# GameTechDev/Intel-Texture-Works-Plugin

Measured on AMD Instinct MI355X. Metric: Mpixels/s encode (BC1/BC3/BC7/BC6H) at 4k x 4k; bit-exact vs the oracle under the pinned ISPC sse/avx-target arithmetic model (no ispc binary exists here; sensitivity of that model: profiles/arith_sensitivity.txt), higher is better.
Workload: dtype f32; 1 GPU; bc7_slow: BC7 GetProfile_slow on ONE synthetic 4096x4096 RGBA8 surface, weak-sharded over 1 GPU(s) by block-row bands (4096 texel rows per rank), texels resident in HBM, device-pointer C ABI call; blocks_per_gpu=1048576, ranks_seen_by_rccl=1, device=gfx950:sramecc+:xnack- / AMD Radeon Graphics / 256 CUs / 2400 MHz, lib=itw-amd 0.1 gfx950 arith=x86-lut-nr contract=off

## Files before the change

include/itw_test_hooks.h:

```cpp
#ifndef ITW_TEST_HOOKS_H
#define ITW_TEST_HOOKS_H

#include "ispc_texcomp.h"

#ifdef __cplusplus
extern "C" {
#endif
#pragma GCC visibility push(default)

void itwTestRcp  (const float* d_in, float* d_out, int64_t n);
void itwTestRsqrt(const float* d_in, float* d_out, int64_t n);
void itwTestF2I  (const float* d_in, int32_t* d_out, int64_t n);

void itwTestBc7TwoSubsetBounds(const rgba_surface* d_src, float* d_out);

int itwTestBc45IndexTable(uint32_t* host_out);

int itwTestBc45ClosestS(uint8_t* host_out);

void itwMultiGpuTestInjectFailure(int rank, int stage, int stall_ms);

void itwTestCombinerHold(int requests, int timeout_ms);
void itwTestCombinerCounters(int64_t out[5]);

#pragma GCC visibility pop
#ifdef __cplusplus
}
#endif
#endif
```

intel-texture-works-plugin_amd/csrc/abi.hip:

```cpp
#include <hip/hip_runtime.h>
#include <cstdio>
#include <cstdlib>
#include <cstring>
#include "../../include/itw_amd.h"
#include "../../include/itw_bc45.h"
#include "../../include/itw_dispatch.h"
#ifdef ITW_TEST_HOOKS
#include "../../include/itw_test_hooks.h"
#endif
#include <algorithm>
#include <atomic>
#include <chrono>
#include <condition_variable>
#include <mutex>
#include <thread>
#include <vector>
#include "bcn_format.hpp"
#include "host_rt.hpp"
#include "kernels.hpp"
#include "x86_math.hpp"

namespace itw {

namespace {
// ... 1194 lines not shown
void CompressBlocksBC4(const rgba_surface* src, uint8_t* dst)
{
    itw::guarded([&] { Job j; j.kind = itw::BCN_BC4; compress(j, src, dst); });
}
void CompressBlocksBC5(const rgba_surface* src, uint8_t* dst)
{
    itw::guarded([&] { Job j; j.kind = itw::BCN_BC5; compress(j, src, dst); });
}
void CompressBlocksBC4S(const rgba_surface* src, uint8_t* dst)
{
    itw::guarded([&] { Job j; j.kind = itw::BCN_BC4S; compress(j, src, dst); });
}
void CompressBlocksBC5S(const rgba_surface* src, uint8_t* dst)
{
    itw::guarded([&] { Job j; j.kind = itw::BCN_BC5S; compress(j, src, dst); });
}

bool itwCompressImageSlicedEx(const rgba_surface* source, uint8_t* target, int64_t block_row_pitch, int dxgi_format, const void* settings,
                              int64_t slice_pixels, ItwProgressFunc* progress, void* user)
{
    bool done = false;
    itw::clear_failure();
    const bool ok = itw::guarded([&] {
        if (!source) itw::fail_msg("null surface");
        const Job j = job_of(dxgi_format, settings);
        const itw::SurfaceGeometry geo = itw::surface_geometry(j.kind, source->width, source->height);
        const int64_t tight = (int64_t)geo.bx * geo.bpb;
        if (block_row_pitch != tight) itw::fail_msg("itwCompressImageSlicedEx: block_row_pitch %lld != %lld (tight)", (long long)block_row_pitch, (long long)tight);
        done = compress_sliced(j, source, target, slices_of(source, slice_pixels), progress, user);
    });
    return ok && done;
}

bool itwCompressImageChainEx(const rgba_surface* images, int count, uint8_t* target, int dxgi_format, const void* settings,
                             ItwProgressFunc* progress, void* user)
{
    bool done = false;
    itw::clear_failure();
    const bool ok = itw::guarded([&] {
        const Job j = chain_job(images, count, target, dxgi_format, settings);
        done = compress_chain(j, images, count, target, progress, user);
    });
    return ok && done;
}

void itwSetSliceWindow(int slices) { g_slice_window.store(slices < 0 ? -1 : slices, std::memory_order_relaxed); }

int itwSliceWindow(int dxgi_format, int width, int height, int64_t slice_pixels) { return itwSliceWindowFor(dxgi_format, nullptr, width, height, slice_pixels); }

int itwSliceWindowFor(int dxgi_format, const void* settings, int width, int height, int64_t slice_pixels)
{
    if (slice_window_setting() < 0) return 0;
    const int kind = itw::format_kind(dxgi_format);
    const int64_t slices = std::min(itw::slice_count(width, height, slice_pixels), itw::kMaxSlices);
    const bool heavy = kind == itw::BCN_BC7 && settings && itw::bc7_scans_every_shape(*static_cast<const bc7_enc_settings*>(settings));
    return slice_window(kind, itw::surface_geometry(kind, width, height).blocks() / slices, (int)slices, heavy);
}

void  itwSetStream(void* s) { tls.user_stream = (hipStream_t)s; }
void* itwGetStream(void)    { return (void*)tls.user_stream; }

int itwAvailable(void)
{
    int n = 0;
    if (hipGetDeviceCount(&n) != hipSuccess || n < 1) { (void)hipGetLastError(); return 0; }
    int dev = 0;
    hipDeviceProp_t p;
    if (hipGetDevice(&dev) != hipSuccess || hipGetDeviceProperties(&p, dev) != hipSuccess) { (void)hipGetLastError(); return 0; }
    return std::strncmp(p.gcnArchName, "gfx950", 6) == 0 ? 1 : 0;
}

void itwSetErrorMode(int mode) { itw::g_error_mode.store(mode == ITW_ON_ERROR_RETURN ? 1 : 0); }
const char* itwLastError(void) { return itw::t_has_error ? itw::t_last_error : nullptr; }
void itwClearError(void) { itw::clear_failure(); }

const char* itwDeviceInfo(void)
{
    tls.info[0] = 0;
    itw::guarded([&] {
        int dev = 0;
        ITW_CHECK(hipGetDevice(&dev));
        hipDeviceProp_t p;
        ITW_CHECK(hipGetDeviceProperties(&p, dev));
        std::snprintf(tls.info, sizeof(tls.info), "%s / %s / %d CUs / %.0f MHz", p.gcnArchName, p.name,
                      p.multiProcessorCount, p.clockRate / 1000.0);
    });
    return tls.info;
}

void itwSetBc7Path(int path) { itw::set_bc7_path(path); itw::set_bc6h_path(path); }
void itwSetBc7Pilot(int percent) { itw::set_bc7_pilot(percent); }

const char* itwVersion(void) { return "itw-amd 0.1 gfx950 arith=x86-lut-nr contract=off"; }

int64_t itwBandForPart(int32_t width, int32_t height, int32_t bytes_per_block,
                       int32_t part, int32_t parts, int32_t* first_row, int32_t* row_count)
{
    const int64_t R = height / 4, bx = width / 4;
    if (parts <= 0 || part < 0 || part >= parts) { if (first_row) *first_row = 0; if (row_count) *row_count = 0; return -1; }
    const int64_t r0 = R * part / parts, r1 = R * (part + 1) / parts;
    if (first_row) *first_row = (int32_t)(r0 * 4);
    if (row_count) *row_count = (int32_t)((r1 - r0) * 4);
    return r0 * bx * bytes_per_block;
}

int64_t itwBandForPartEx(int32_t width, int32_t height, int32_t bytes_per_block, int32_t part, int32_t parts, int32_t keep_partial_blocks,
                         int32_t* first_row, int32_t* row_count)
{
    if (!keep_partial_blocks) return itwBandForPart(width, height, bytes_per_block, part, parts, first_row, row_count);
    const int64_t R = ((int64_t)height + 3) / 4, bx = ((int64_t)width + 3) / 4;
    if (parts <= 0 || part < 0 || part >= parts || height < 1 || width < 1) { if (first_row) *first_row = 0; if (row_count) *row_count = 0; return -1; }
    const int64_t r0 = R * part / parts, r1 = R * (part + 1) / parts;
    const int64_t y0 = r0 * 4, y1 = (r1 * 4 < height) ? r1 * 4 : height;
    if (first_row) *first_row = (int32_t)y0;
    if (row_count) *row_count = (int32_t)(y1 > y0 ? y1 - y0 : 0);
    return r0 * bx * bytes_per_block;
}

void itwWarmupBC45(void)
{
    itwClearError();
    itw::guarded([&] { bind_thread_to_current_device(); itw::warmup_bc45(); });
}

void itwWarmupBC45S(void)
{
    itwClearError();
    itw::guarded([&] { bind_thread_to_current_device(); itw::warmup_bc45s(); });
}

#ifdef ITW_TEST_HOOKS
int itwTestBc45IndexTable(uint32_t* host_out)
{
    itwClearError();
    return itw::guarded([&] { if (!host_out) itw::fail_msg("null pointer"); itw::copy_bc45_index_table(host_out, tls.user_stream); }) ? 0 : -1;
}

int itwTestBc45ClosestS(uint8_t* host_out)
{
    itwClearError();
    return itw::guarded([&] { if (!host_out) itw::fail_msg("null pointer"); itw::copy_bc45_closest_snorm(host_out, tls.user_stream); }) ? 0 : -1;
}

void itwTestBc7TwoSubsetBounds(const rgba_surface* d_src, float* d_out)
{
    itwClearError();
    itw::guarded([&] {
        if (!d_src || !d_src->ptr || !d_out) itw::fail_msg("null pointer");
        itw::launch_bc7_test_bounds(d_src->ptr, d_src->stride, d_src->width, d_src->height, d_out, tls.user_stream);
        ITW_CHECK(hipGetLastError());
    });
}

void itwTestRcp(const float* in, float* out, int64_t n)
{
    if (n <= 0) return;
    hipLaunchKernelGGL(k_test_rcp, dim3((unsigned)((n + 255) / 256)), dim3(256), 0, tls.user_stream, in, out, n);
    itw::guarded([&] { ITW_CHECK(hipGetLastError()); });
}
void itwTestRsqrt(const float* in, float* out, int64_t n)
{
    if (n <= 0) return;
    hipLaunchKernelGGL(k_test_rsqrt, dim3((unsigned)((n + 255) / 256)), dim3(256), 0, tls.user_stream, in, out, n);
    itw::guarded([&] { ITW_CHECK(hipGetLastError()); });
}
void itwTestF2I(const float* in, int32_t* out, int64_t n)
{
    if (n <= 0) return;
    hipLaunchKernelGGL(k_test_f2i, dim3((unsigned)((n + 255) / 256)), dim3(256), 0, tls.user_stream, in, out, n);
    itw::guarded([&] { ITW_CHECK(hipGetLastError()); });
}

void itwTestCombinerHold(int requests, int timeout_ms)
{
    int dev = 0;
    if (hipGetDevice(&dev) != hipSuccess) { (void)hipGetLastError(); return; }
    if (dev < 0 || dev >= kMaxDevices) return;
    Combiner& c = g_combiner[dev];
    std::lock_guard<std::mutex> lk(c.m);
    c.hold_requests = requests > 0 ? requests : 0;
    c.hold_timeout_ms = timeout_ms > 0 ? timeout_ms : 0;
}

void itwTestCombinerCounters(int64_t out[5])
{
    if (!out) return;
    out[0] = g_cstats.bursts.load(); out[1] = g_cstats.batches.load(); out[2] = g_cstats.requests.load(); out[3] = g_cstats.calls.load();
    out[4] = g_hold_timeouts.load();
}
#endif

}
```

intel-texture-works-plugin_amd/csrc/bc7.hip:

```cpp
#include <atomic>
#include <cstdlib>
#include <cstring>
#include <type_traits>
#include "bc7_exact.hpp"
#include "kernels.hpp"
#include "host_rt.hpp"

namespace itw {

#define BCN_TABLE_QUAL __device__ const
#include "bc7_f02_schedule.h"
#undef BCN_TABLE_QUAL

#ifndef ITW_BC7_LANE_PAL
#define ITW_BC7_LANE_PAL 1
#endif
constexpr int LANE_PAL_LEVELS = 24;
constexpr int TPB = 256;
constexpr float INV255 = 1.0f / 255.0f;
constexpr int32_t ERR_MAX = 0x7fffffff;
enum Family { F_MODES02 = 0, F_MODES13 = 1, F_MODE7 = 2, F_MODES456 = 3 };

struct ModeTraits { int pairs, bits, ch; };
__device__ __forceinline__ constexpr ModeTraits traits(int mode)
// ... 1007 lines not shown

template <int FAMILY, int RANKED, bool VEC16>
__global__ void __launch_bounds__(TPB) __attribute__((amdgpu_waves_per_eu(search_waves(FAMILY, RANKED), search_waves(FAMILY, RANKED))))
bc7_search_kernel(const uint8_t* __restrict__ src, int64_t stride, int32_t blocks_x, int32_t nblocks,
                  uint4* __restrict__ wins, const bc7_enc_settings S)
{
    __shared__ unsigned short s_seed16[2048];
    __shared__ uint32_t s_seed32[2048];
    extern __shared__ int32_t s_keys[];
    __shared__ uint2 s_pal[RANKED == 0 ? 12 * TPB : (RANKED == 2 && ITW_BC7_LANE_PAL) ? 16 * TPB : 1];
    Lane ln;
    ln.T = stage_seed_tables_fast(s_seed16, s_seed32, threadIdx.x, TPB);
    __syncthreads();
    const int32_t gid = blockIdx.x * TPB + threadIdx.x;
    const bool live = gid < nblocks;
    const int32_t b = live ? gid : nblocks - 1;
    ln.keys = s_keys + threadIdx.x;
    ln.pal = s_pal + ((RANKED == 0 || (RANKED == 2 && ITW_BC7_LANE_PAL)) ? threadIdx.x : 0);
    load_block<VEC16>(ln.tx, src, stride, blocks_x, b);

    Win wa, wb;
    if (FAMILY == F_MODES02) search_02(ln, S, wa, wb);
    if (FAMILY == F_MODES13) search_two_subset<false, 3, RANKED>(ln, S, wa, wb);
    if (FAMILY == F_MODE7) {
        if (S.channels == 4) search_two_subset<true, 4, RANKED>(ln, S, wa, wb); else search_two_subset<true, 3, RANKED>(ln, S, wa, wb);
    }
    if (live) {
        store_win(wins, nblocks, 0, b, wa);
        if (FAMILY != F_MODE7) store_win(wins, nblocks, 1, b, wb);
    }
}

template <int FAMILY, bool VEC16>
__global__ void __launch_bounds__(TPB) __attribute__((amdgpu_waves_per_eu(finish_waves(FAMILY), finish_waves(FAMILY))))
bc7_finish_kernel(const uint8_t* __restrict__ src, int64_t stride, int32_t blocks_x, int32_t nblocks,
                  uint8_t* __restrict__ dst, int32_t* __restrict__ err_ws, const uint4* __restrict__ wins,
                  const bc7_enc_settings S, const int first)
{
    __shared__ unsigned short s_seed16[2048];
    __shared__ uint32_t s_seed32[2048];
    __shared__ uint2 s_pal[FAMILY == F_MODES456 ? (ITW_BC7_LANE_PAL ? 16 : 8) * TPB : (ITW_BC7_LANE_PAL ? (FAMILY == F_MODES02 ? 24 : 16) * TPB : 1)];
    Lane ln;
    ln.T = stage_seed_tables_fast(s_seed16, s_seed32, threadIdx.x, TPB);
    __syncthreads();
    const int32_t gid = blockIdx.x * TPB + threadIdx.x;
    const bool live = gid < nblocks;
    const int32_t b = live ? gid : nblocks - 1;
    ln.keys = nullptr;
    ln.pal = s_pal + ((FAMILY == F_MODES456 || ITW_BC7_LANE_PAL) ? threadIdx.x : 0);
    load_block<VEC16>(ln.tx, src, stride, blocks_x, b);

    ln.best_err = first ? ERR_MAX : err_ws[b];
    ln.best[0] = ln.best[1] = ln.best[2] = ln.best[3] = 0u;
    ln.improved = (first != 0);
    ln.opaque_err = 0;
    if (S.channels == 4) {
        uint32_t e = 0;
#pragma unroll
        for (int d = 0; d < 4; d++) { const uint32_t x = ~ln.tx.pl[3][d]; e = udot4(x, x, e); }
        ln.opaque_err = (int32_t)e;
    }

    if (FAMILY == F_MODES02) {
        Win w;
        load_win(w, wins, nblocks, 0, b);
        refine_and_commit<0>(ln, w, S.refineIterations[0], S.channels);
        if (!S.skip_mode2) { load_win(w, wins, nblocks, 1, b); refine_and_commit<2>(ln, w, S.refineIterations[2], S.channels); }
    }
    if (FAMILY == F_MODES13) {
        Win w;
        if (S.fastSkipTreshold_mode1 > 0) { load_win(w, wins, nblocks, 0, b); refine_and_commit<1>(ln, w, S.refineIterations[1], S.channels); }
        if (S.fastSkipTreshold_mode3 > 0) { load_win(w, wins, nblocks, 1, b); refine_and_commit<3>(ln, w, S.refineIterations[3], S.channels); }
    }
    if (FAMILY == F_MODE7) {
        Win w;
        load_win(w, wins, nblocks, 0, b);
        refine_and_commit<7>(ln, w, S.refineIterations[7], S.channels);
    }
    if (FAMILY == F_MODES456) {
        if (S.mode_selection[2]) modes_45(ln, S);
        if (S.mode_selection[3]) { if (S.channels == 4) mode_6<4>(ln, S); else mode_6<3>(ln, S); }
    }

    if (live && ln.improved) {
        uint32_t* d = reinterpret_cast<uint32_t*>(dst + (int64_t)b * 16);
        if (VEC16) *reinterpret_cast<uint4*>(d) = make_uint4(ln.best[0], ln.best[1], ln.best[2], ln.best[3]);
        else { d[0] = ln.best[0]; d[1] = ln.best[1]; d[2] = ln.best[2]; d[3] = ln.best[3]; }
        err_ws[b] = ln.best_err;
    }
}

enum WideKind { WK_SCAN02 = 0, WK_SCAN13 = 1, WK_SCAN7 = 2 };
__host__ __device__ constexpr int wide_win_slot(int mode) { return mode == 0 ? 0 : mode == 2 ? 1 : mode == 1 ? 2 : mode == 3 ? 3 : 4; }

template <int FIT_CH, int RANK_CH>
__device__ __forceinline__ void whole_block_rank_stats(Stats<RANK_CH>& rfull, const Tex& tx)
{
    IStats<FIT_CH> full;
    stats_int<FIT_CH>(full, tx.pl, whole_block());
    IStats<RANK_CH> t;
    #pragma unroll
    for (int i = 0; i < 10; i++) t.m[i] = full.m[i];
    #pragma unroll
    for (int i = 0; i < 4; i++) t.s[i] = full.s[i];
    t.n = 16;
    stats_float<RANK_CH>(rfull, t);
}

template <int FIT_CH, int RANK_CH>
__device__ __forceinline__ int32_t merge_key(const Win& w, const Tex& tx, const SeedTables& T)
{
    if (w.key >= 0) return w.key;
    Stats<RANK_CH> rfull;
    whole_block_rank_stats<FIT_CH, RANK_CH>(rfull, tx);
    return rank_key<RANK_CH>(w.shape, tx, rfull, T);
}

__device__ __forceinline__ uint32_t pack_win(const Win& w) { return w.err == ERR_MAX ? 0xffffffffu : (((uint32_t)w.err << 7) | ((uint32_t)w.shape & 127u)); }
__device__ __forceinline__ void unpack_win(Win& w, uint32_t v)
{
    if (v == 0xffffffffu) { w.err = ERR_MAX; w.shape = 0; } else { w.err = (int32_t)(v >> 7); w.shape = (int32_t)(v & 127u); }
    w.key = -1;
}

#ifndef LIST_SCAN_MAX_PARTS
#define LIST_SCAN_MAX_PARTS 8
#endif
__device__ __forceinline__ int32_t list_scan_parts(int32_t count, int32_t nblocks)
{
    const int32_t chunks = ((count + TPB - 1) / TPB + 7) & ~7;
    if (chunks <= 0) return 1;
    const int32_t p = nblocks / (chunks * TPB);
    return p < 1 ? 1 : (p > LIST_SCAN_MAX_PARTS ? LIST_SCAN_MAX_PARTS : p);
}
template <int FIT_CH, int RANK_CH>
__device__ __forceinline__ void merge_packed_parts(Win& w, Lane& ln, const uint32_t* __restrict__ row, int32_t count, int parts, int32_t slot)
{
    unpack_win(w, row[slot]);
    for (int p = 1; p < parts; p++) {
        Win x;
        unpack_win(x, row[(int64_t)p * count + slot]);
        if (x.err < w.err) { w = x; continue; }
        if (x.err != w.err || x.err == ERR_MAX) continue;
        w.key = merge_key<FIT_CH, RANK_CH>(w, ln.tx, ln.T); x.key = merge_key<FIT_CH, RANK_CH>(x, ln.tx, ln.T);
        if (x.key < w.key) w = x;
    }
}

struct PairRegion { uint64_t* words; int32_t* buckets; int32_t* ctr; int32_t cap; };
constexpr int PAIR_CTR_OVERFLOW = 64, PAIR_CTR_REDO = 65, PAIR_CTR_LIST = 66, PAIR_CTR_TARGET = 68, PAIR_CTR_WORDS = 80;
struct PairTarget { PairRegion P; int32_t* redo; };
static_assert(sizeof(PairTarget) <= (PAIR_CTR_WORDS - PAIR_CTR_TARGET) * sizeof(int32_t) && PAIR_CTR_TARGET % 2 == 0 && PAIR_CTR_WORDS % 4 == 0, "PairTarget behind the counters");
constexpr int PAIR_MAX_PER_BLOCK = 32;
constexpr unsigned long long PAIR_WORD_HEAVY = ~0ull - 1ull;

struct ScanTasks { int n; int kind[3]; };

struct ChunkSel { int32_t kind, stripe, band; const int32_t* gate; int32_t want; };
__device__ __forceinline__ int32_t sel_chunk(const ChunkSel& s, int32_t i)
{
    if (s.kind == 0) return i;
    if (s.kind == 2) return i * 8 + 3;
    const int32_t q = i / s.stripe;
    return (2 * q + s.band) * s.stripe + (i - q * s.stripe);
}

__host__ __device__ constexpr int scan_all_waves(bool ranked, bool fam7) { return fam7 ? (ranked ? SWR27 : SW7) : (ranked ? SWR2 : SWALL); }
template <bool VEC16, bool RANKED_LISTS, bool FAM7>
__global__ void __launch_bounds__(TPB) __attribute__((amdgpu_waves_per_eu(scan_all_waves(RANKED_LISTS, FAM7), scan_all_waves(RANKED_LISTS, FAM7))))
bc7_scan_all(const uint8_t* __restrict__ src, int64_t stride, int32_t blocks_x, int32_t nblocks, uint32_t* __restrict__ wins4,
             const bc7_enc_settings S, const ScanTasks tasks, const int ranked13, const int ranked7, const int32_t nchunks, const int32_t grain,
             const int32_t* __restrict__ rgb_list, const int32_t* __restrict__ rgb_count, const int32_t split, const ChunkSel sel,
             const uint4* __restrict__ compact)
{
    __shared__ unsigned short s_seed16[2048];
    __shared__ uint32_t s_seed32[2048];
    __shared__ uint2 s_pal[((RANKED_LISTS && ITW_BC7_LANE_PAL) ? 16 : 12) * TPB];
    if (sel.gate && *sel.gate != sel.want) return;
    if (!RANKED_LISTS && split) {
        const int32_t count = *rgb_count;
        const int32_t parts = list_scan_parts(count, nblocks);
        const uint32_t wg = blockIdx.x;
        const int32_t chunk = (int32_t)((wg / (8u * (uint32_t)parts)) * 8u + (wg & 7u)), part = (int32_t)((wg >> 3) % (uint32_t)parts);
        if (chunk * TPB >= count) return;
        Lane ln;
        ln.T = stage_seed_tables_fast(s_seed16, s_seed32, threadIdx.x, TPB);
        __syncthreads();
        const int32_t gid = chunk * TPB + threadIdx.x;
        const bool live = gid < count;
        const int32_t slot = live ? gid : count - 1;
        ln.keys = nullptr;
        ln.pal = s_pal + threadIdx.x;
        if (compact) load_block_compact(ln.tx, compact, slot); else load_block<VEC16>(ln.tx, src, stride, blocks_x, rgb_list[slot]);
        Win wa, wb;
        if (FAM7) {
            search_two_subset<true, 4, 0>(ln, S, wa, wb, part, parts);
            if (live) wins4[(int64_t)wide_win_slot(7) * nblocks + (int64_t)part * count + slot] = pack_win(wa);
        } else {
            search_two_subset<false, 3, 0>(ln, S, wa, wb, part, parts);
            if (live) {
                wins4[(int64_t)wide_win_slot(1) * nblocks + (int64_t)part * count + slot] = pack_win(wa);
                wins4[(int64_t)wide_win_slot(3) * nblocks + (int64_t)part * count + slot] = pack_win(wb);
            }
        }
        return;
    }
    const uint32_t w = blockIdx.x, per = (uint32_t)grain * (uint32_t)tasks.n, group = w / per, r = w % per;
    const int t = (int)(r / (uint32_t)grain);
    const int32_t chunk_i = (int32_t)(group * (uint32_t)grain + r % (uint32_t)grain);
    if (chunk_i >= nchunks) return;
    const int32_t chunk = sel_chunk(sel, chunk_i);
    const int32_t nact = (!FAM7 && rgb_list) ? *rgb_count : nblocks;
    if (chunk * TPB >= nact) return;
    Lane ln;
    ln.T = stage_seed_tables_fast(s_seed16, s_seed32, threadIdx.x, TPB);
    __syncthreads();
    const int32_t gid = chunk * TPB + threadIdx.x;
    const bool live = gid < nact;
    const int32_t slot = live ? gid : nact - 1;
    const int32_t b = (!FAM7 && rgb_list) ? rgb_list[slot] : slot;
    ln.keys = nullptr;
    ln.pal = s_pal + threadIdx.x;
    load_block<VEC16>(ln.tx, src, stride, blocks_x, b);
    const int kind = tasks.kind[t];
    Win wa, wb;
    if (!FAM7 && kind == WK_SCAN02) {
        search_02(ln, S, wa, wb);
        if (live) { wins4[(int64_t)wide_win_slot(0) * nblocks + b] = pack_win(wa); if (!S.skip_mode2) wins4[(int64_t)wide_win_slot(2) * nblocks + b] = pack_win(wb); }
    } else if (!FAM7) {
        if (RANKED_LISTS && ranked13) search_two_subset<false, 3, 2>(ln, S, wa, wb); else search_two_subset<false, 3, 0>(ln, S, wa, wb);
        if (live) { wins4[(int64_t)wide_win_slot(1) * nblocks + b] = pack_win(wa); wins4[(int64_t)wide_win_slot(3) * nblocks + b] = pack_win(wb); }
    } else {
        if (S.channels == 4) { if (RANKED_LISTS && ranked7) search_two_subset<true, 4, 2>(ln, S, wa, wb); else search_two_subset<true, 4, 0>(ln, S, wa, wb); }
        else                 { if (RANKED_LISTS && ranked7) search_two_subset<true, 3, 2>(ln, S, wa, wb); else search_two_subset<true, 3, 0>(ln, S, wa, wb); }
        if (live) wins4[(int64_t)wide_win_slot(7) * nblocks + b] = pack_win(wa);
    }
}

__device__ __forceinline__ int32_t append_to_list(int32_t* __restrict__ list, int32_t* __restrict__ count, bool need, int32_t b)
{
    const unsigned long long m = __ballot(need);
    int32_t pos = -1;
    if (m) {
        const int lane = (int)(threadIdx.x & 63u);
        int32_t base = 0;
        if (lane == 0) base = atomicAdd(count, (int32_t)__popcll(m));
        base = __shfl(base, 0);
        if (need) { pos = base + (int32_t)__popcll(m & ((1ull << lane) - 1ull)); list[pos] = b; }
    }
    return pos;
}

__device__ __forceinline__ bool mode6_cannot_win(Lane& ln)
{
    if (__all(ln.best_err == 0)) return true;
    IStats<3> full;
    stats_int<3>(full, ln.tx.pl, whole_block());
    const float d = __builtin_amdgcn_sqrtf(subset_residual_bound(full) * rcp_of_count(16)) * 0.999999f - BOUND_SLACK3[16];
    const float e = fmaxf(d, 0.0f);
    const float lb = e * e * 0.999999f;
    return __all(lb >= (float)ln.best_err);
}

#ifndef FINISH_ALL_WAVES
#define FINISH_ALL_WAVES 2
#endif
#ifndef BOUND_BAIL_AFTER
#define BOUND_BAIL_AFTER 4
#endif
#ifndef BOUND_BAIL_LANES
#define BOUND_BAIL_LANES 40
#endif
template <bool VEC16, int PHASE>
__global__ void __launch_bounds__(TPB) __attribute__((amdgpu_waves_per_eu(FINISH_ALL_WAVES, FINISH_ALL_WAVES)))
bc7_finish_all(const uint8_t* __restrict__ src, int64_t stride, int32_t blocks_x, int32_t nblocks, uint8_t* __restrict__ dst,
               const uint32_t* __restrict__ wins4, const bc7_enc_settings S, int32_t* __restrict__ inc_err,
               const int32_t* __restrict__ in_list, const int32_t* __restrict__ in_count, int32_t* __restrict__ out_list, int32_t* __restrict__ out_count,
               int32_t* __restrict__ out_list7, int32_t* __restrict__ out_count7, const ChunkSel sel,
               const uint4* __restrict__ in_compact, uint4* __restrict__ out_compact)
{
    constexpr bool LISTED = PHASE == 2 || PHASE == 4 || PHASE == 5 || PHASE == 7 || PHASE == 8;
    constexpr bool DO02 = PHASE == 0 || PHASE == 2 || PHASE == 3 || PHASE == 5;
    constexpr bool DO13 = PHASE == 0 || PHASE == 2 || PHASE == 4;
    constexpr bool DO7 = PHASE == 0 || PHASE == 1;
    constexpr bool DO456 = PHASE == 0 || PHASE == 1 || PHASE == 3 || PHASE == 6;
    __shared__ unsigned short s_seed16[2048];
    __shared__ uint32_t s_seed32[2048];
    __shared__ uint2 s_pal[(ITW_BC7_LANE_PAL ? LANE_PAL_LEVELS : 8) * TPB];
    __shared__ int32_t s_at[PHASE == 3 ? TPB / 64 : 1][64];
    if (sel.gate && *sel.gate != sel.want) return;
    const int32_t nact = LISTED ? *in_count : nblocks;
    const int32_t chunk = LISTED ? (int32_t)blockIdx.x : sel_chunk(sel, (int32_t)blockIdx.x);
    if (chunk * TPB >= nact) return;
    Lane ln;
    ln.T = stage_seed_tables_fast(s_seed16, s_seed32, threadIdx.x, TPB);
    __syncthreads();
    const int32_t gid = chunk * TPB + threadIdx.x;
    const bool live = gid < nact;
    const int32_t slot = live ? gid : nact - 1;
    const int32_t b = LISTED ? in_list[slot] : slot;
    ln.keys = nullptr;
    ln.pal = s_pal + threadIdx.x;
    if (LISTED && in_compact) load_block_compact(ln.tx, in_compact, slot); else load_block<VEC16>(ln.tx, src, stride, blocks_x, b);
    ln.best_err = ERR_MAX;
    ln.best[0] = ln.best[1] = ln.best[2] = ln.best[3] = 0u;
    ln.improved = false;
    ln.opaque_err = 0;
    if (S.channels == 4) {
        uint32_t e = 0;
#pragma unroll
        for (int d = 0; d < 4; d++) { const uint32_t x = ~ln.tx.pl[3][d]; e = udot4(x, x, e); }
        ln.opaque_err = (int32_t)e;
    }
    const bool on13 = S.mode_selection[1];
    int32_t e_alpha = ERR_MAX;
    if (PHASE == 2 || PHASE == 5) e_alpha = inc_err[b];
    if (PHASE == 4 || PHASE == 7 || PHASE == 8) ln.best_err = inc_err[b];
    Win w;
    if (DO02 && S.mode_selection[0]) {
        unpack_win(w, wins4[(int64_t)wide_win_slot(0) * nblocks + b]);
        refine_and_commit<0>(ln, w, S.refineIterations[0], S.channels);
        if (!S.skip_mode2) { ln.tx.fence(); unpack_win(w, wins4[(int64_t)wide_win_slot(2) * nblocks + b]); refine_and_commit<2>(ln, w, S.refineIterations[2], S.channels); }
    }
    const int32_t e02 = ln.best_err;
    if (DO13 && PHASE != 4) {
        if (on13 && S.fastSkipTreshold_mode1 > 0) { ln.tx.fence(); unpack_win(w, wins4[(int64_t)wide_win_slot(1) * nblocks + b]); refine_and_commit<1>(ln, w, S.refineIterations[1], S.channels); }
        if (on13 && S.fastSkipTreshold_mode3 > 0) { ln.tx.fence(); unpack_win(w, wins4[(int64_t)wide_win_slot(3) * nblocks + b]); refine_and_commit<3>(ln, w, S.refineIterations[3], S.channels); }
    }
    if (PHASE == 4) {
        const int parts = list_scan_parts(nact, nblocks);
        if (S.fastSkipTreshold_mode1 > 0) { ln.tx.fence(); merge_packed_parts<3, 3>(w, ln, wins4 + (int64_t)wide_win_slot(1) * nblocks, nact, parts, slot); refine_and_commit<1>(ln, w, S.refineIterations[1], S.channels); }
        if (S.fastSkipTreshold_mode3 > 0) { ln.tx.fence(); merge_packed_parts<3, 3>(w, ln, wins4 + (int64_t)wide_win_slot(3) * nblocks, nact, parts, slot); refine_and_commit<3>(ln, w, S.refineIterations[3], S.channels); }
    }
    bool redo = false;
    if (PHASE == 8) {
        const unsigned long long* pw = reinterpret_cast<const unsigned long long*>(wins4) + 2 * (int64_t)slot;
        const int32_t inc = ln.best_err;
        const bool heavy = pw[0] == PAIR_WORD_HEAVY;
        redo = !heavy && *out_count7 != 0;
        const bool use = !heavy && !redo;
        const unsigned long long v1 = (use && S.fastSkipTreshold_mode1 > 0) ? pw[0] : ~0ull, v3 = (use && S.fastSkipTreshold_mode3 > 0) ? pw[1] : ~0ull;
        if (v1 != ~0ull) {
            ln.tx.fence();
            w.err = (int32_t)(v1 >> 32); w.key = (int32_t)(uint32_t)v1; w.shape = w.key & 63;
            const bool open = w.err + ln.opaque_err >= inc;
            const int32_t before = ln.best_err;
            refine_and_commit<1>(ln, w, S.refineIterations[1], S.channels);
            redo = redo || (open && ln.best_err < before);
        }
        if (v3 != ~0ull) {
            ln.tx.fence();
            w.err = (int32_t)(v3 >> 32); w.key = (int32_t)(uint32_t)v3; w.shape = w.key & 63;
            const bool open = w.err + ln.opaque_err >= inc;
            const int32_t before = ln.best_err;
            refine_and_commit<3>(ln, w, S.refineIterations[3], S.channels);
            redo = redo || (open && ln.best_err < before);
        }
        append_to_list(out_list, out_count, live && redo, b);
    }
    if (PHASE == 7) {
        const int parts = list_scan_parts(nact, nblocks);
        ln.tx.fence();
        merge_packed_parts<4, 4>(w, ln, wins4 + (int64_t)wide_win_slot(7) * nblocks, nact, parts, slot);
        refine_and_commit<7>(ln, w, S.refineIterations[7], S.channels);
    }
    if (DO7 && on13 && S.fastSkipTreshold_mode7 > 0) { ln.tx.fence(); unpack_win(w, wins4[(int64_t)wide_win_slot(7) * nblocks + b]); refine_and_commit<7>(ln, w, S.refineIterations[7], S.channels); }
    if (DO456) {
        ln.tx.fence();
        if (S.mode_selection[2]) modes_45(ln, S);
        if (S.mode_selection[3]) {
            if (S.channels == 4) mode_6<4>(ln, S);
            else if (!mode6_cannot_win(ln)) mode_6<3>(ln, S);
        }
    }
    if (PHASE == 1) {
        if (live) inc_err[b] = ln.best_err;
        append_to_list(out_list, out_count, live && ln.opaque_err <= ln.best_err, b);
    }
    if (PHASE == 6) {
        const bool rgb = ln.opaque_err <= ln.best_err;
        if (live) inc_err[b] = rgb ? ln.best_err : ln.best_err + 1;
        append_to_list(out_list, out_count, live && rgb, b);
        append_to_list(out_list7, out_count7, live && !rgb, b);
    }
    if (PHASE == 3 || PHASE == 5) {
        int32_t inc;
        if (PHASE == 3) inc = ln.best_err + (ln.best_err < e02 ? 1 : 0);
        else            inc = (e02 <= e_alpha) ? e02 : e_alpha + 1;
        if (live) inc_err[b] = inc;
        ln.tx.fence();
        IStats<3> full;
        stats_int<3>(full, ln.tx.pl, whole_block());
        const float lim = (float)(inc - ln.opaque_err) - 0.5f;
        const float lim7 = (float)inc - 0.5f;
        const bool with7 = PHASE == 5 && out_list7 != nullptr;
        const PairTarget* target = nullptr;
        if (PHASE == 3) target = reinterpret_cast<const PairTarget*>(out_count + (PAIR_CTR_TARGET - PAIR_CTR_LIST));
        const bool pairs = PHASE == 3 && target->P.words != nullptr;
        bool need = !live, need7 = !live || !with7;
        unsigned long long mine = 0, any = 0;
#pragma unroll 1
        for (int shape = 0; shape < 64; shape++) {
            if (!pairs) {
                if (__all(need && need7)) break;
                if (shape == BOUND_BAIL_AFTER && __popcll(__ballot(need && need7)) >= BOUND_BAIL_LANES) { need = true; need7 = true; break; }
            }
            const float lb = two_subset_bound(shape, ln.tx.pl, full);
            const bool in = !(lb >= lim);
            need = need || in;
            need7 = need7 || !(lb >= lim7);
            if (pairs) {
                mine |= (live && in) ? (1ull << shape) : 0ull;
                any |= __ballot(live && in) ? (1ull << shape) : 0ull;
            }
        }
        const int32_t pos = append_to_list(out_list, out_count, live && need, b);
        if (out_compact && pos >= 0) {
            uint4* c = out_compact + (int64_t)pos * 4;
#pragma unroll
            for (int y = 0; y < 4; y++) c[y] = make_uint4(ln.tx.w[y * 4 + 0], ln.tx.w[y * 4 + 1], ln.tx.w[y * 4 + 2], ln.tx.w[y * 4 + 3]);
        }
        if (pairs) {
            const int lane = (int)__builtin_amdgcn_mbcnt_hi(~0u, __builtin_amdgcn_mbcnt_lo(~0u, 0u));
            const int wave = __builtin_amdgcn_readfirstlane((int)(threadIdx.x >> 6));
            const PairRegion P = target->P;
            int32_t* pair_redo = target->redo;
            const bool heavy = __popcll(mine) > PAIR_MAX_PER_BLOCK;
            if (pos >= 0) { P.words[2 * (int64_t)pos] = heavy ? PAIR_WORD_HEAVY : ~0ull; P.words[2 * (int64_t)pos + 1] = ~0ull; }
            if (heavy) mine = 0;
            append_to_list(pair_redo, P.ctr + PAIR_CTR_REDO, heavy, b);
            int32_t k = 0;
            for (unsigned long long rest = any; rest; rest &= rest - 1ull) {
                const int shape = __builtin_amdgcn_readfirstlane((int)__builtin_ctzll(rest));
                const int32_t c = (int32_t)__popcll(__ballot((mine >> shape) & 1ull));
                k = (lane == shape) ? c : k;
            }
            s_at[wave][lane] = k;
            __syncthreads();
            if (threadIdx.x < 64u) {
                int32_t t = 0;
#pragma unroll
                for (int w = 0; w < TPB / 64; w++) t += s_at[w][lane];
                int32_t base = t ? atomicAdd(P.ctr + lane, t) : 0;
                if (base + t > P.cap) { P.ctr[PAIR_CTR_OVERFLOW] = 1; base = -1; }
#pragma unroll
                for (int w = 0; w < TPB / 64; w++) { const int32_t c = s_at[w][lane]; s_at[w][lane] = base; base = base < 0 ? -1 : base + c; }
            }
            __syncthreads();
            const int32_t at = s_at[wave][lane];
            for (unsigned long long rest = any; rest; rest &= rest - 1ull) {
                const int shape = __builtin_amdgcn_readfirstlane((int)__builtin_ctzll(rest));
                const bool in = (mine >> shape) & 1ull;
                const unsigned long long m = __ballot(in);
                const int32_t base = __builtin_amdgcn_readlane(at, shape);
                if (in && base >= 0) P.buckets[(int64_t)shape * P.cap + base + (int32_t)__popcll(m & ((1ull << lane) - 1ull))] = pos;
            }
        }
        if (with7) append_to_list(out_list7, out_count7, live && need7, b);
    }
    bool store = live;
    if (PHASE == 2 || PHASE == 5) store = store && ln.best_err <= e_alpha;
    if (PHASE == 4 || PHASE == 7) store = store && ln.improved;
    if (PHASE == 8) store = store && ln.improved && !redo;
    if ((PHASE == 4 || PHASE == 8) && store) inc_err[b] = ln.best_err;
    if (store) {
        uint32_t* d = reinterpret_cast<uint32_t*>(dst + (int64_t)b * 16);
        if (VEC16) *reinterpret_cast<uint4*>(d) = make_uint4(ln.best[0], ln.best[1], ln.best[2], ln.best[3]);
        else { d[0] = ln.best[0]; d[1] = ln.best[1]; d[2] = ln.best[2]; d[3] = ln.best[3]; }
    }
}

template <bool VEC16>
__global__ void __launch_bounds__(TPB)
bc7_pilot_estimate(const uint8_t* __restrict__ src, int64_t stride, int32_t blocks_x, int32_t nblocks, const uint32_t* __restrict__ wins4,
                   const int skip_mode2, const ChunkSel sel, int32_t* __restrict__ counters , const int32_t thr256,
                   int32_t* __restrict__ flag, int32_t* __restrict__ host_counts )
{
    const int32_t chunk = sel_chunk(sel, (int32_t)blockIdx.x * 8 + 3);
    if (chunk * TPB < nblocks) {
        const int32_t gid = chunk * TPB + threadIdx.x;
        const bool live = gid < nblocks;
        const int32_t b = live ? gid : nblocks - 1;
        Tex tx;
        load_block<VEC16>(tx, src, stride, blocks_x, b);
        Win w0, w2;
        unpack_win(w0, wins4[(int64_t)wide_win_slot(0) * nblocks + b]);
        unpack_win(w2, skip_mode2 ? 0xffffffffu : wins4[(int64_t)wide_win_slot(2) * nblocks + b]);
        const int32_t e = min(w0.err, w2.err);
        IStats<3> full;
        stats_int<3>(full, tx.pl, whole_block());
        const float lim = (float)e - 0.5f;
        bool need = !live;
#pragma unroll 1
        for (int shape = 0; shape < 64; shape++) {
            if (__all(need)) break;
            if (shape == BOUND_BAIL_AFTER && __popcll(__ballot(need)) >= BOUND_BAIL_LANES) { need = true; break; }
            need = need || !(two_subset_bound(shape, tx.pl, full) >= lim);
        }
        const unsigned long long ml = __ballot(live && need), mt = __ballot(live);
        if ((threadIdx.x & 63u) == 0u) { atomicAdd(counters + 0, (int32_t)__popcll(ml)); atomicAdd(counters + 1, (int32_t)__popcll(mt)); }
    }
    __syncthreads();
    if (threadIdx.x == 0) {
        __threadfence();
        if (atomicAdd(counters + 2, 1) == (int32_t)gridDim.x - 1) {
            __threadfence();
            const int64_t listed = atomicAdd(counters + 0, 0), sampled = atomicAdd(counters + 1, 0);
            *flag = (listed * 256 <= (int64_t)thr256 * sampled) ? 1 : 0;
            if (host_counts) { host_counts[0] = (int32_t)listed; host_counts[1] = (int32_t)sampled; __threadfence_system(); }
        }
    }
}

__global__ void __launch_bounds__(TPB) bc7_bounded_setup(int32_t* __restrict__ counters, const PairTarget t0, const PairTarget t1)
{
    for (int i = (int)threadIdx.x; i < 16 + 2 * PAIR_CTR_WORDS; i += TPB) {
        const int j = i < 16 ? 0 : (i - 16) % PAIR_CTR_WORDS;
        if (i < 16 || j < PAIR_CTR_TARGET) counters[i] = 0;
    }
    if (threadIdx.x == 0) {
        *reinterpret_cast<PairTarget*>(counters + 16 + PAIR_CTR_TARGET) = t0;
        *reinterpret_cast<PairTarget*>(counters + 16 + PAIR_CTR_WORDS + PAIR_CTR_TARGET) = t1;
    }
}


__global__ void __launch_bounds__(TPB) __attribute__((amdgpu_waves_per_eu(4, 4)))
bc7_pair_scan(const uint8_t* __restrict__ src, int64_t stride, int32_t blocks_x, const int32_t* __restrict__ list, const uint4* __restrict__ compact,
              const bc7_enc_settings S, const PairRegion P)
{
    __shared__ unsigned short s_seed16[2048];
    __shared__ uint32_t s_seed32[2048];
    __shared__ uint2 s_pal[12 * TPB];
    __shared__ int32_t s_first[65];
    if (P.ctr[PAIR_CTR_OVERFLOW]) return;
    if (threadIdx.x == 0) {
        int32_t t = 0;
        for (int s = 0; s < 64; s++) { s_first[s] = t; t += (P.ctr[s] + 63) >> 6; }
        s_first[64] = t;
    }
    __syncthreads();
    const int32_t total = s_first[64];
    const int32_t wpb = TPB / 64;
    if ((int32_t)blockIdx.x * wpb >= total) return;
    Lane ln;
    ln.T = stage_seed_tables_fast(s_seed16, s_seed32, threadIdx.x, TPB);
    __syncthreads();
    ln.keys = nullptr;
    ln.pal = s_pal + threadIdx.x;
    const int lane = (int)(threadIdx.x & 63u);
    const bool on_a = S.fastSkipTreshold_mode1 > 0, on_b = S.fastSkipTreshold_mode3 > 0;
    int shape = 0;
#pragma unroll 1
    for (int32_t tile = (int32_t)blockIdx.x * wpb + (int32_t)(threadIdx.x >> 6); tile < total; tile += (int32_t)gridDim.x * wpb) {
        while (s_first[shape + 1] <= tile) shape++;
        shape = __builtin_amdgcn_readfirstlane(shape);
        const int32_t len = P.ctr[shape];
        const int32_t at = (tile - s_first[shape]) * 64 + lane;
        const bool live = at < len;
        const int32_t slot = P.buckets[(int64_t)shape * P.cap + (live ? at : len - 1)];
        if (compact) load_block_compact(ln.tx, compact, slot); else load_block<false>(ln.tx, src, stride, blocks_x, list[slot]);
        Win wa, wb;
        search_two_subset<false, 3, 0>(ln, S, wa, wb, shape, 64);
        const int32_t ea = wa.err, ec = wb.err;
        ln.tx.fence();
        Stats<3> rfull;
        whole_block_rank_stats<3, 3>(rfull, ln.tx);
        const uint32_t key = (uint32_t)rank_key<3>(shape, ln.tx, rfull, ln.T);
        if (live && on_a) atomicMin(reinterpret_cast<unsigned long long*>(P.words + 2 * (int64_t)slot),     ((unsigned long long)(uint32_t)ea << 32) | key);
        if (live && on_b) atomicMin(reinterpret_cast<unsigned long long*>(P.words + 2 * (int64_t)slot + 1), ((unsigned long long)(uint32_t)ec << 32) | key);
    }
}

constexpr int WIDE_SLOTS = 18;
constexpr int WIDE_SLOT_M4 = 5, WIDE_SLOT_M5 = 13, WIDE_SLOT_M6 = 17;
constexpr int WIDE_MAX_TASKS = 56;
constexpr int WIDE_MAX_PARTS = 16;
struct WideTasks { int n; uint8_t kind[WIDE_MAX_TASKS]; uint8_t part[WIDE_MAX_TASKS]; uint8_t parts[WIDE_MAX_TASKS]; };
struct WideModes { int n; uint8_t mode[20]; uint8_t parts[20]; };


struct WideDims { int32_t nblocks; int32_t pstride; };
__device__ __forceinline__ void store_win_wide(uint4* __restrict__ wins, WideDims d, int slot, int part, int32_t b, const Win& w)
{
    wins[((int64_t)slot * d.pstride + part) * d.nblocks + b] = make_uint4((uint32_t)w.err, (uint32_t)w.shape, (uint32_t)w.key, 0u);
}
__device__ __forceinline__ void load_win_wide(Win& w, const uint4* __restrict__ wins, WideDims d, int slot, int part, int32_t b)
{
    const uint4 v = wins[((int64_t)slot * d.pstride + part) * d.nblocks + b];
    w.err = (int32_t)v.x; w.shape = (int32_t)v.y; w.key = (int32_t)v.z;
}
__device__ __forceinline__ void store_candidate(int32_t* __restrict__ cerr, uint4* __restrict__ cblk, int32_t nblocks, int slot, int32_t b,
                                                int32_t err, const uint32_t (&blk)[4])
{
    cerr[(int64_t)slot * nblocks + b] = err;
    cblk[(int64_t)slot * nblocks + b] = make_uint4(blk[0], blk[1], blk[2], blk[3]);
}

template <int MODE>
__device__ __forceinline__ void merge_parts(Win& w, Lane& ln, const uint4* __restrict__ wins, WideDims dims, int parts, int32_t b, int channels)
{
    load_win_wide(w, wins, dims, wide_win_slot(MODE), 0, b);
    for (int p = 1; p < parts; p++) {
        Win x;
        load_win_wide(x, wins, dims, wide_win_slot(MODE), p, b);
        if (x.err < w.err) { w = x; continue; }
        if (x.err != w.err || x.err == ERR_MAX) continue;
        if (MODE == 0 || MODE == 2) {
            if (x.shape < w.shape) w = x;
        } else {
            if (MODE == 7) {
                if (channels == 4) { w.key = merge_key<4, 4>(w, ln.tx, ln.T); x.key = merge_key<4, 4>(x, ln.tx, ln.T); }
                else               { w.key = merge_key<4, 3>(w, ln.tx, ln.T); x.key = merge_key<4, 3>(x, ln.tx, ln.T); }
            } else { w.key = merge_key<3, 3>(w, ln.tx, ln.T); x.key = merge_key<3, 3>(x, ln.tx, ln.T); }
            if (x.key < w.key) w = x;
        }
    }
}

#ifndef WIDE_SCAN_WAVES
#define WIDE_SCAN_WAVES 4
#endif
#ifndef WIDE_FILL_DIVISOR
#define WIDE_FILL_DIVISOR 2
#endif
template <bool VEC16, bool RANKED_LISTS>
__global__ void __launch_bounds__(TPB) __attribute__((amdgpu_waves_per_eu(RANKED_LISTS ? 3 : WIDE_SCAN_WAVES, RANKED_LISTS ? 3 : WIDE_SCAN_WAVES)))
bc7_wide_phase1(const uint8_t* __restrict__ src, int64_t stride, int32_t blocks_x, int32_t nblocks, uint4* __restrict__ wins,
                int32_t* __restrict__ cerr, uint4* __restrict__ cblk, const bc7_enc_settings S, const WideTasks tasks, const int ranked13, const int ranked7,
                const int pstride)
{
    const WideDims dims{nblocks, pstride};
    __shared__ unsigned short s_seed16[2048];
    __shared__ uint32_t s_seed32[2048];
    __shared__ uint2 s_pal[((RANKED_LISTS && ITW_BC7_LANE_PAL) ? 16 : 12) * TPB];
    Lane ln;
    ln.T = stage_seed_tables_fast(s_seed16, s_seed32, threadIdx.x, TPB);
    __syncthreads();
    const int32_t gid = blockIdx.x * TPB + threadIdx.x;
    const bool live = gid < nblocks;
    const int32_t b = live ? gid : nblocks - 1;
    ln.keys = nullptr;
    ln.pal = s_pal + threadIdx.x;
    load_block<VEC16>(ln.tx, src, stride, blocks_x, b);
    ln.best_err = ERR_MAX; ln.opaque_err = 0; ln.improved = false;
    ln.best[0] = ln.best[1] = ln.best[2] = ln.best[3] = 0u;

    const int kind = tasks.kind[blockIdx.y], part = tasks.part[blockIdx.y], parts = tasks.parts[blockIdx.y];
    if (kind == WK_SCAN02) {
        Win w0, w2;
        search_02(ln, S, w0, w2, part, parts);
        if (live) { store_win_wide(wins, dims, wide_win_slot(0), part, b, w0); if (!S.skip_mode2) store_win_wide(wins, dims, wide_win_slot(2), part, b, w2); }
    } else if (kind == WK_SCAN13) {
        Win w1, w3;
        if (RANKED_LISTS && ranked13) search_two_subset<false, 3, 2>(ln, S, w1, w3, part, parts); else search_two_subset<false, 3, 0>(ln, S, w1, w3, part, parts);
        if (live) { store_win_wide(wins, dims, wide_win_slot(1), part, b, w1); store_win_wide(wins, dims, wide_win_slot(3), part, b, w3); }
    } else {
        Win w7, unused;
        if (S.channels == 4) { if (RANKED_LISTS && ranked7) search_two_subset<true, 4, 2>(ln, S, w7, unused, part, parts); else search_two_subset<true, 4, 0>(ln, S, w7, unused, part, parts); }
        else                 { if (RANKED_LISTS && ranked7) search_two_subset<true, 3, 2>(ln, S, w7, unused, part, parts); else search_two_subset<true, 3, 0>(ln, S, w7, unused, part, parts); }
        if (live) store_win_wide(wins, dims, wide_win_slot(7), part, b, w7);
    }
}

template <bool VEC16, bool SINGLES>
#ifndef WIDE_SINGLES_WAVES
#define WIDE_SINGLES_WAVES 3
#endif
__global__ void __launch_bounds__(TPB) __attribute__((amdgpu_waves_per_eu(SINGLES ? WIDE_SINGLES_WAVES : 2, SINGLES ? WIDE_SINGLES_WAVES : 2)))
bc7_wide_phase2(const uint8_t* __restrict__ src, int64_t stride, int32_t blocks_x, int32_t nblocks, const uint4* __restrict__ wins,
                int32_t* __restrict__ cerr, uint4* __restrict__ cblk, const bc7_enc_settings S, const WideModes modes, const int pstride)
{
    const WideDims dims{nblocks, pstride};
    __shared__ unsigned short s_seed16[2048];
    __shared__ uint32_t s_seed32[2048];
    __shared__ uint2 s_pal[SINGLES ? (ITW_BC7_LANE_PAL ? 16 : 8) * TPB : (ITW_BC7_LANE_PAL ? LANE_PAL_LEVELS * TPB : 1)];
    Lane ln;
    ln.T = stage_seed_tables_fast(s_seed16, s_seed32, threadIdx.x, TPB);
    __syncthreads();
    const int32_t gid = blockIdx.x * TPB + threadIdx.x;
    const bool live = gid < nblocks;
    const int32_t b = live ? gid : nblocks - 1;
    ln.keys = nullptr;
    ln.pal = s_pal + ((SINGLES || ITW_BC7_LANE_PAL) ? threadIdx.x : 0);
    load_block<VEC16>(ln.tx, src, stride, blocks_x, b);
    ln.best_err = ERR_MAX; ln.improved = false;
    ln.best[0] = ln.best[1] = ln.best[2] = ln.best[3] = 0u;
    ln.opaque_err = 0;
    if (S.channels == 4) {
        uint32_t e = 0;
#pragma unroll
        for (int d = 0; d < 4; d++) { const uint32_t x = ~ln.tx.pl[3][d]; e = udot4(x, x, e); }
        ln.opaque_err = (int32_t)e;
    }
    const int mode = modes.mode[blockIdx.y], parts = modes.parts[blockIdx.y];
    if (SINGLES && mode >= 100) {
        const int r = (mode - 100) >> 2, c = (mode - 100) & 3;
        Dual best4, best5;
        clear(best4); clear(best5);
        int32_t err4 = ERR_MAX, err5 = ERR_MAX;
        modes_45_scan(ln, S, r, r + 1, best4, err4, best5, err5, c == 3 ? 7 : 1 << c);
        uint32_t blk[4] = {0u, 0u, 0u, 0u};
        if (c != 2) {
            if (err4 < ERR_MAX) emit_dual<4>(blk, best4);
            if (live) store_candidate(cerr, cblk, nblocks, WIDE_SLOT_M4 + 2 * r + (c == 1 ? 1 : 0), b, err4, blk);
        }
        if (c >= 2) {
            blk[0] = blk[1] = blk[2] = blk[3] = 0u;
            if (err5 < ERR_MAX) emit_dual<5>(blk, best5);
            if (live) store_candidate(cerr, cblk, nblocks, WIDE_SLOT_M5 + r, b, err5, blk);
        }
        return;
    }
    if (SINGLES) {
        if (S.channels == 4) mode_6<4>(ln, S); else mode_6<3>(ln, S);
        if (live) store_candidate(cerr, cblk, nblocks, WIDE_SLOT_M6, b, ln.best_err, ln.best);
        return;
    }
    Win w;
    int slot = 0;
    if (mode == 0)      { merge_parts<0>(w, ln, wins, dims, parts, b, S.channels); refine_and_commit<0>(ln, w, S.refineIterations[0], S.channels); slot = 0; }
    else if (mode == 2) { merge_parts<2>(w, ln, wins, dims, parts, b, S.channels); refine_and_commit<2>(ln, w, S.refineIterations[2], S.channels); slot = 1; }
    else if (mode == 1) { merge_parts<1>(w, ln, wins, dims, parts, b, S.channels); refine_and_commit<1>(ln, w, S.refineIterations[1], S.channels); slot = 2; }
    else if (mode == 3) { merge_parts<3>(w, ln, wins, dims, parts, b, S.channels); refine_and_commit<3>(ln, w, S.refineIterations[3], S.channels); slot = 3; }
    else                { merge_parts<7>(w, ln, wins, dims, parts, b, S.channels); refine_and_commit<7>(ln, w, S.refineIterations[7], S.channels); slot = 4; }
    if (live) store_candidate(cerr, cblk, nblocks, slot, b, ln.best_err, ln.best);
}

__global__ void __launch_bounds__(TPB)
bc7_wide_commit(const int32_t* __restrict__ cerr, const uint4* __restrict__ cblk, int32_t nblocks, uint32_t active_slots, uint4* __restrict__ dst, int vec16)
{
    const int32_t b = blockIdx.x * TPB + threadIdx.x;
    if (b >= nblocks) return;
    int32_t best = ERR_MAX;
    uint4 blk = make_uint4(0u, 0u, 0u, 0u);
    for (int slot = 0; slot < WIDE_SLOTS; slot++) {
        if (!((active_slots >> slot) & 1u)) continue;
        const int32_t e = cerr[(int64_t)slot * nblocks + b];
        if (e < best) { best = e; blk = cblk[(int64_t)slot * nblocks + b]; }
    }
    if (vec16) dst[b] = blk;
    else { uint32_t* d = reinterpret_cast<uint32_t*>(dst) + (int64_t)b * 4; d[0] = blk.x; d[1] = blk.y; d[2] = blk.z; d[3] = blk.w; }
}

struct Bc7Launch {
    bool vec; dim3 grid; hipStream_t st; const uint8_t* src; int64_t stride; int bx; int32_t n;
    uint8_t* dst; int32_t* err; uint4* wins; bc7_enc_settings S; int first;
};

template <int FAMILY, int RANKED>
static void launch_search(const Bc7Launch& L)
{
    const size_t lds = RANKED == 1 ? (size_t)64 * TPB * sizeof(int32_t) : 0;
    if (L.vec) hipLaunchKernelGGL((bc7_search_kernel<FAMILY, RANKED, true>),  L.grid, dim3(TPB), lds, L.st, L.src, L.stride, L.bx, L.n, L.wins, L.S);
    else       hipLaunchKernelGGL((bc7_search_kernel<FAMILY, RANKED, false>), L.grid, dim3(TPB), lds, L.st, L.src, L.stride, L.bx, L.n, L.wins, L.S);
}
template <int FAMILY>
static void launch_finish(Bc7Launch& L)
{
    if (L.vec) hipLaunchKernelGGL((bc7_finish_kernel<FAMILY, true>),  L.grid, dim3(TPB), 0, L.st, L.src, L.stride, L.bx, L.n, L.dst, L.err, L.wins, L.S, L.first);
    else       hipLaunchKernelGGL((bc7_finish_kernel<FAMILY, false>), L.grid, dim3(TPB), 0, L.st, L.src, L.stride, L.bx, L.n, L.dst, L.err, L.wins, L.S, L.first);
    L.first = 0;
}

#ifndef ITW_BC7_WIDE_MAX_BLOCKS
#define ITW_BC7_WIDE_MAX_BLOCKS 262144
#endif

#ifdef ITW_TEST_HOOKS
template <bool VEC16>
__global__ void __launch_bounds__(TPB) bc7_test_bounds(const uint8_t* __restrict__ src, int64_t stride, int32_t blocks_x, int32_t nblocks, float* __restrict__ out)
{
    const int32_t gid = blockIdx.x * TPB + threadIdx.x;
    const int32_t b = gid < nblocks ? gid : nblocks - 1;
    Tex tx;
    load_block<VEC16>(tx, src, stride, blocks_x, b);
    IStats<3> full;
    stats_int<3>(full, tx.pl, whole_block());
#pragma unroll 1
    for (int shape = 0; shape < 64; shape++) {
        const float lb = two_subset_bound(shape, tx.pl, full);
        if (gid < nblocks) out[(int64_t)b * 64 + shape] = lb;
    }
}
void launch_bc7_test_bounds(const uint8_t* src, int64_t stride, int width, int height, float* out, hipStream_t st)
{
    const int bx = width / 4;
    const int64_t n = (int64_t)bx * (height / 4);
    if (n <= 0) return;
    const bool vec = ((reinterpret_cast<uintptr_t>(src) | (uintptr_t)stride) & 15) == 0;
    const dim3 grid((unsigned)((n + TPB - 1) / TPB));
    if (vec) hipLaunchKernelGGL((bc7_test_bounds<true>),  grid, dim3(TPB), 0, st, src, stride, bx, (int32_t)n, out);
    else     hipLaunchKernelGGL((bc7_test_bounds<false>), grid, dim3(TPB), 0, st, src, stride, bx, (int32_t)n, out);
}
#endif

static std::atomic<int> g_bc7_path{-1};
static int bc7_path_override()
{
    int v = g_bc7_path.load(std::memory_order_relaxed);
    if (v < 0) {
        const char* e = std::getenv("ITW_BC7_PATH");
        v = !e ? 0 : !std::strcmp(e, "deep") ? 1 : !std::strcmp(e, "wide") ? 2 : 0;
        g_bc7_path.store(v, std::memory_order_relaxed);
    }
    return v;
}
void set_bc7_path(int v) { g_bc7_path.store(v == 1 || v == 2 ? v : 0, std::memory_order_relaxed); }
bool bc7_staged_bands_ok()
{
    static const bool on = [] { const char* e = std::getenv("ITW_STAGED_BANDS"); return !(e && e[0] == '0'); }();
    return on && bc7_path_override() != 2;
}

static bool bc7_bounded_order()
{
    static const bool on = [] { const char* e = std::getenv("ITW_BC7_BOUND"); return !(e && e[0] == '0'); }();
    return on;
}
#ifndef ITW_BC7_PILOT_THR_DEFAULT
#define ITW_BC7_PILOT_THR_DEFAULT 90
#endif
static std::atomic<int> g_bc7_pilot{-2};
static int bc7_pilot_threshold()
{
    int pct = g_bc7_pilot.load(std::memory_order_relaxed);
    if (pct == -2) {
        const char* e = std::getenv("ITW_BC7_PILOT_THR");
        pct = e ? std::atoi(e) : ITW_BC7_PILOT_THR_DEFAULT;
        pct = pct < 0 ? -1 : (pct > 100 ? 100 : pct);
        g_bc7_pilot.store(pct, std::memory_order_relaxed);
    }
    return pct < 0 ? -1 : pct * 256 / 100;
}
void set_bc7_pilot(int percent) { g_bc7_pilot.store(percent < -1 ? -2 : (percent > 100 ? 100 : percent), std::memory_order_relaxed); }
static bool bc7_pilot_debug()
{
    static const bool on = [] { const char* e = std::getenv("ITW_BC7_PILOT_DEBUG"); return e && e[0] == '1'; }();
    return on;
}
static int bc7_bands()
{
    static const int k = [] { const char* e = std::getenv("ITW_BC7_BANDS"); const int v = e ? std::atoi(e) : 2; return v < 2 ? 1 : 2; }();
    return k;
}
static bool bc7_compact_lists()
{
    static const bool on = [] { const char* e = std::getenv("ITW_BC7_COMPACT"); return !(e && e[0] == '0'); }();
    return on;
}
static bool bc7_pairs_on()
{
    const char* e = std::getenv("ITW_BC7_PAIRS");
    return !(e && e[0] == '0');
}
static int32_t bc7_pair_cap(int32_t layout_cap)
{
    const char* e = std::getenv("ITW_BC7_PAIR_CAP");
    const long v = e ? std::atol(e) : 0;
    return (v > 0 && v < layout_cap) ? (int32_t)v : layout_cap;
}
static bool bc7_fused_on()
{
    static const bool on = [] { const char* e = std::getenv("ITW_BC7_FUSED"); return !(e && e[0] == '0'); }();
    return on;
}
static bool bc7_alpha_first(const bc7_enc_settings& S)
{
    static const bool on = [] { const char* e = std::getenv("ITW_BC7_ALPHA_PRUNE"); return !(e && e[0] == '0'); }();
    const bool on02 = S.mode_selection[0];
    const bool on13 = S.mode_selection[1] && (S.fastSkipTreshold_mode1 > 0 || S.fastSkipTreshold_mode3 > 0);
    const bool on7 = S.mode_selection[1] && S.fastSkipTreshold_mode7 > 0;
    return on && S.channels == 4 && (on02 || on13) && (on7 || S.mode_selection[2] || S.mode_selection[3]);
}
#define ITW_BC7_WIDE_MAX_BLOCKS_ALPHA_FIRST 131072

static bool bc7_use_wide(int64_t n, const bc7_enc_settings& S, int64_t wide_max)
{
    auto long_ranked = [](int t) { return t > 16 && t < 64; };
    if (S.mode_selection[1] && (long_ranked(S.fastSkipTreshold_mode1) || long_ranked(S.fastSkipTreshold_mode3) || long_ranked(S.fastSkipTreshold_mode7))) return false;
    auto ranked = [](int t) { return t > 0 && t < 64; };
    if (S.mode_selection[1]) {
        const int a = S.fastSkipTreshold_mode1, c = S.fastSkipTreshold_mode3;
        if ((ranked(a) || ranked(c)) && (a > 16 || c > 16)) return false;
    }
    if (S.mode45_channel0 < 0 || S.mode45_channel0 > 3) return false;
    const int o = bc7_path_override();
    if (o == 1) return false;
    const int64_t hard_cap = (int64_t)1 << 20;
    if (o == 2) return n <= hard_cap;
    if (n >= ITW_BC7_WIDE_MAX_BLOCKS_ALPHA_FIRST && bc7_alpha_first(S)) return false;
    return n <= (wide_max > 0 ? (wide_max < hard_cap ? wide_max : hard_cap) : ITW_BC7_WIDE_MAX_BLOCKS);
}

static size_t wide_win_entries(size_t n) { return n > 262144 ? n : 262144; }
static size_t wide_workspace_bytes(size_t n)
{
    return (size_t)5 * wide_win_entries(n) * sizeof(uint4) + (((size_t)WIDE_SLOTS * n * sizeof(int32_t) + 15) & ~(size_t)15) + (size_t)WIDE_SLOTS * n * sizeof(uint4);
}
struct ListRegion { size_t list, wins, compact, cap, pair_words, pair_redo, pair_buckets, pair_ctr, pair_cap; };
struct FusedLayout { size_t inc, list0, list1, list2, counts, words; ListRegion band[2]; };
struct FusedNeeds { bool lists, bands, compact, pairs; };
static FusedNeeds fused_needs(const bc7_enc_settings* s)
{
    if (!s) return FusedNeeds{true, true, true, true};
    bc7_enc_settings S = *s;
    S.channels = (s->channels == 4) ? 4 : 3;
    auto ranked = [](int t) { return t > 0 && t < 64; };
    const bool on02 = S.mode_selection[0];
    const bool on13 = S.mode_selection[1] && (S.fastSkipTreshold_mode1 > 0 || S.fastSkipTreshold_mode3 > 0);
    const bool r13 = on13 && (ranked(S.fastSkipTreshold_mode1) || ranked(S.fastSkipTreshold_mode3));
    const bool bounded = bc7_bounded_order() && on02 && on13 && !r13;
    const bool alpha = bc7_alpha_first(S);
    const bool on7 = S.mode_selection[1] && S.fastSkipTreshold_mode7 > 0;
    return FusedNeeds{alpha || bounded, bounded, bounded && !alpha && bc7_compact_lists(), bounded && !alpha && !on7};
}
static FusedLayout fused_layout(size_t n, const FusedNeeds& need)
{
    auto up4 = [](size_t w) { return (w + 3) & ~(size_t)3; };
    const size_t nchunks = (n + TPB - 1) / TPB;
    FusedLayout W;
    size_t o = up4(5 * n);
    W.inc = o;      o = up4(o + n);
    const size_t lcap = need.lists ? 2 * (nchunks / 2 + 65) * TPB : 0;
    W.list0 = o;    o = up4(o + lcap);
    W.list1 = o;    o = up4(o + lcap);
    W.list2 = o;    o = up4(o + lcap);
    W.counts = o;   o += 16;
    for (int k = 0; k < 2; k++) { W.band[k].pair_ctr = o; o += PAIR_CTR_WORDS; }
    for (int k = 0; k < 2; k++) {
        ListRegion& r = W.band[k];
        r.cap = (nchunks / 2 + 65) * TPB;
        r.list = o;    o = up4(o + (need.bands ? r.cap : 0));
        r.wins = o;    o = up4(o + (need.bands ? 5 * r.cap : 0));
    }
    W.band[0].compact = o; o += need.compact ? 16 * W.band[0].cap : 0;
    W.band[1].compact = o; o += need.compact ? 16 * W.band[1].cap : 0;
    for (int k = 0; k < 2; k++) { W.band[k].pair_words = o; o += need.pairs ? 4 * W.band[k].cap : 0; }
    for (int k = 0; k < 2; k++) { W.band[k].pair_redo = o; o += need.pairs ? W.band[k].cap : 0; }
    for (int k = 0; k < 2; k++) { W.band[k].pair_cap = W.band[k].cap / 8; W.band[k].pair_buckets = o; o += need.pairs ? 64 * W.band[k].pair_cap : 0; }
    W.words = o;
    return W;
}
bool bc7_scans_every_shape(const bc7_enc_settings& s) { return fused_needs(&s).bands; }

size_t bc7_workspace_bytes(int width, int height, int64_t wide_max_blocks, const bc7_enc_settings* settings)
{
    const size_t n = (size_t)(width / 4) * (size_t)(height / 4);
    size_t deep = ((n * sizeof(int32_t) + 15) & ~(size_t)15) + 2 * n * sizeof(uint4);
    const size_t fused = fused_layout(n, fused_needs(settings)).words * sizeof(uint32_t);
    if (fused > deep) deep = fused;
    const size_t limit = bc7_path_override() == 2 ? ((size_t)1 << 20) : (wide_max_blocks > 0 ? (size_t)wide_max_blocks : (size_t)ITW_BC7_WIDE_MAX_BLOCKS);
    const bool may_wide = bc7_path_override() != 1 && n <= limit && n <= ((size_t)1 << 20);
    const size_t wide = may_wide ? wide_workspace_bytes(n) : 0;
    return deep > wide ? deep : wide;
}

static void launch_bc7_wide(const uint8_t* src, int64_t stride, int bx, int64_t n, uint8_t* dst, const bc7_enc_settings& S, float* workspace,
                            hipStream_t st, const Bc7Aux* aux)
{
    uint4* wins = reinterpret_cast<uint4*>(workspace);
    int32_t* cerr = reinterpret_cast<int32_t*>(wins + (size_t)5 * wide_win_entries((size_t)n));
    uint4* cblk = reinterpret_cast<uint4*>(reinterpret_cast<uint8_t*>(cerr) + (((size_t)WIDE_SLOTS * n * sizeof(int32_t) + 15) & ~(size_t)15));
    const bool vec = ((reinterpret_cast<uintptr_t>(src) | (uintptr_t)stride | reinterpret_cast<uintptr_t>(dst)) & 15) == 0;
    auto ranked = [](int t) { return t > 0 && t < 64; };

    const bool on02 = S.mode_selection[0];
    const bool on13 = S.mode_selection[1] && (S.fastSkipTreshold_mode1 > 0 || S.fastSkipTreshold_mode3 > 0);
    const bool on7  = S.mode_selection[1] && S.fastSkipTreshold_mode7 > 0;
    const bool on45 = S.mode_selection[2], on6 = S.mode_selection[3];
    const int ranked13 = on13 && (ranked(S.fastSkipTreshold_mode1) || ranked(S.fastSkipTreshold_mode3));
    const int ranked7 = on7 && ranked(S.fastSkipTreshold_mode7);
    const bool any_ranked = ranked13 || ranked7;

    const int64_t waves = (n + 63) / 64;
    const int families = (on02 ? 1 : 0) + (on13 ? 1 : 0) + (on7 ? 1 : 0);
    const int resident = 1024 * (any_ranked ? 3 : WIDE_SCAN_WAVES);
    int want = 1;
    while (want < WIDE_MAX_PARTS && waves * families * want * WIDE_FILL_DIVISOR <= resident) want *= 2;
    auto cap = [&](int limit) { int p = want; while (p > limit) p /= 2; return p < 1 ? 1 : p; };
    const int p02 = cap(16);
    const int list13 = ranked13 ? (S.fastSkipTreshold_mode1 > S.fastSkipTreshold_mode3 ? S.fastSkipTreshold_mode1 : S.fastSkipTreshold_mode3) : 64;
    const int p13 = cap(ranked13 ? (list13 >= 8 ? 4 : list13 >= 2 ? 2 : 1) : 16);
    const int list7 = ranked7 ? S.fastSkipTreshold_mode7 : 64;
    const int p7 = cap(ranked7 ? (list7 >= 8 ? 4 : list7 >= 2 ? 2 : 1) : 16);
    int pstride = 1;
    if (on02 && p02 > pstride) pstride = p02;
    if (on13 && p13 > pstride) pstride = p13;
    if (on7 && p7 > pstride) pstride = p7;

    WideTasks T;
    std::memset(&T, 0, sizeof T);
    auto add = [&](int kind, int part, int parts) { T.kind[T.n] = (uint8_t)kind; T.part[T.n] = (uint8_t)part; T.parts[T.n] = (uint8_t)parts; T.n++; };
    WideModes R, G;
    std::memset(&R, 0, sizeof R);
    std::memset(&G, 0, sizeof G);
    uint32_t active = 0;
    auto add_refine = [&](int mode, int parts) { R.mode[R.n] = (uint8_t)mode; R.parts[R.n] = (uint8_t)parts; R.n++; active |= 1u << wide_win_slot(mode); };
    auto add_single = [&](int code) { G.mode[G.n] = (uint8_t)code; G.parts[G.n] = 1; G.n++; };
    if (on13) { for (int p = 0; p < p13; p++) add(WK_SCAN13, p, p13); if (S.fastSkipTreshold_mode1 > 0) add_refine(1, p13); if (S.fastSkipTreshold_mode3 > 0) add_refine(3, p13); }
    if (on02) { for (int p = 0; p < p02; p++) add(WK_SCAN02, p, p02); add_refine(0, p02); if (!S.skip_mode2) add_refine(2, p02); }
    if (on7)  { for (int p = 0; p < p7; p++) add(WK_SCAN7, p, p7); add_refine(7, p7); }
    if (on45) {
        const int rots = (S.channels == 4 ? 4 : 3) - S.mode45_channel0;
        const bool split = waves * (3 * rots + (on6 ? 1 : 0) + (aux ? 0 : R.n)) <= 2048;
        for (int r = S.mode45_channel0; r < (S.channels == 4 ? 4 : 3); r++) {
            if (split) { for (int c = 0; c < 3; c++) add_single(100 + 4 * r + c); active |= 3u << (WIDE_SLOT_M4 + 2 * r); }
            else       { add_single(100 + 4 * r + 3); active |= 1u << (WIDE_SLOT_M4 + 2 * r); }
            active |= 1u << (WIDE_SLOT_M5 + r);
        }
    }
    if (on6)  { add_single(6); active |= 1u << WIDE_SLOT_M6; }

    const unsigned gx = (unsigned)((n + TPB - 1) / TPB);
    const dim3 blk(TPB);
    hipStream_t gs = st;
    if (aux && G.n > 0 && T.n > 0) {
        (void)hipEventRecord(aux->fork, st);
        (void)hipStreamWaitEvent(aux->stream, aux->fork, 0);
        gs = aux->stream;
    }
    if (G.n > 0) {
        if (vec) hipLaunchKernelGGL((bc7_wide_phase2<true, true>),  dim3(gx, (unsigned)G.n), blk, 0, gs, src, stride, bx, (int32_t)n, wins, cerr, cblk, S, G, pstride);
        else     hipLaunchKernelGGL((bc7_wide_phase2<false, true>), dim3(gx, (unsigned)G.n), blk, 0, gs, src, stride, bx, (int32_t)n, wins, cerr, cblk, S, G, pstride);
        if (gs != st) (void)hipEventRecord(aux->join, gs);
    }
    if (T.n > 0) {
        const dim3 grid(gx, (unsigned)T.n);
        if (any_ranked) {
            if (vec) hipLaunchKernelGGL((bc7_wide_phase1<true, true>),  grid, blk, 0, st, src, stride, bx, (int32_t)n, wins, cerr, cblk, S, T, ranked13, ranked7, pstride);
            else     hipLaunchKernelGGL((bc7_wide_phase1<false, true>), grid, blk, 0, st, src, stride, bx, (int32_t)n, wins, cerr, cblk, S, T, ranked13, ranked7, pstride);
        } else {
            if (vec) hipLaunchKernelGGL((bc7_wide_phase1<true, false>),  grid, blk, 0, st, src, stride, bx, (int32_t)n, wins, cerr, cblk, S, T, ranked13, ranked7, pstride);
            else     hipLaunchKernelGGL((bc7_wide_phase1<false, false>), grid, blk, 0, st, src, stride, bx, (int32_t)n, wins, cerr, cblk, S, T, ranked13, ranked7, pstride);
        }
    }
    if (R.n > 0) {
        if (vec) hipLaunchKernelGGL((bc7_wide_phase2<true, false>),  dim3(gx, (unsigned)R.n), blk, 0, st, src, stride, bx, (int32_t)n, wins, cerr, cblk, S, R, pstride);
        else     hipLaunchKernelGGL((bc7_wide_phase2<false, false>), dim3(gx, (unsigned)R.n), blk, 0, st, src, stride, bx, (int32_t)n, wins, cerr, cblk, S, R, pstride);
    }
    if (gs != st) (void)hipStreamWaitEvent(st, aux->join, 0);
    hipLaunchKernelGGL(bc7_wide_commit, dim3(gx), blk, 0, st, cerr, cblk, (int32_t)n, active, reinterpret_cast<uint4*>(dst), vec ? 1 : 0);
}

bool bc7_has_order_verdict(const bc7_enc_settings& s)
{
    bc7_enc_settings S = s;
    S.channels = (s.channels == 4) ? 4 : 3;
    auto ranked = [](int t) { return t > 0 && t < 64; };
    const bool on13 = S.mode_selection[1] && (S.fastSkipTreshold_mode1 > 0 || S.fastSkipTreshold_mode3 > 0);
    return bc7_fused_on() && bc7_bounded_order() && S.mode_selection[0] && on13 && !ranked(S.fastSkipTreshold_mode1) && !ranked(S.fastSkipTreshold_mode3) &&
           !(S.mode_selection[1] && S.fastSkipTreshold_mode7 > 0) && !bc7_alpha_first(S);
}

void launch_bc7(const uint8_t* src, int64_t stride, int width, int height, uint8_t* dst,
                const bc7_enc_settings& s, float* workspace, hipStream_t st, const Bc7Aux* aux)
{
    const int bx = width / 4, by = height / 4;
    const int64_t n = (int64_t)bx * by;
    if (n <= 0) return;
    Bc7Launch L;
    L.S = s;
    L.S.channels = (s.channels == 4) ? 4 : 3;
    const bool single = aux && aux->single;
    if (aux && aux->probe && !bc7_has_order_verdict(L.S)) return;
    if (!single && bc7_use_wide(n, L.S, aux ? aux->wide_max_blocks : 0)) { launch_bc7_wide(src, stride, bx, n, dst, L.S, workspace, st, aux); return; }
    L.err = reinterpret_cast<int32_t*>(workspace);
    L.wins = reinterpret_cast<uint4*>(reinterpret_cast<uint8_t*>(workspace) + (((size_t)n * sizeof(int32_t) + 15) & ~(size_t)15));
    L.vec = ((reinterpret_cast<uintptr_t>(src) | (uintptr_t)stride | reinterpret_cast<uintptr_t>(dst)) & 15) == 0;
    L.grid = dim3((unsigned)((n + TPB - 1) / TPB));
    L.st = st; L.src = src; L.stride = stride; L.bx = bx; L.n = (int32_t)n; L.dst = dst; L.first = 1;
    const bc7_enc_settings& S = L.S;
    auto ranked = [](int t) { return t > 0 && t < 64; };
    auto small = [](int t) { return t <= 16; };
    {
        const bool fused_on = bc7_fused_on();
        const bool on02 = S.mode_selection[0];
        const bool on13 = S.mode_selection[1] && (S.fastSkipTreshold_mode1 > 0 || S.fastSkipTreshold_mode3 > 0);
        const bool on7 = S.mode_selection[1] && S.fastSkipTreshold_mode7 > 0;
        const bool r13 = on13 && (ranked(S.fastSkipTreshold_mode1) || ranked(S.fastSkipTreshold_mode3));
        const bool r7 = on7 && ranked(S.fastSkipTreshold_mode7);
        const bool long13 = r13 && !(small(S.fastSkipTreshold_mode1) && small(S.fastSkipTreshold_mode3));
        const bool long7 = r7 && !small(S.fastSkipTreshold_mode7);
        const bool any_mode = on02 || on13 || on7 || S.mode_selection[2] || S.mode_selection[3];
        if (fused_on && !long13 && !long7 && any_mode) {
            uint32_t* wins4 = reinterpret_cast<uint32_t*>(workspace);
            const int32_t nchunks = (int32_t)((n + TPB - 1) / TPB);
            const int a13 = r13 ? 1 : 0, a7 = r7 ? 1 : 0;
            const FusedLayout W = fused_layout((size_t)n, fused_needs(&S));
            int32_t* alpha_err = reinterpret_cast<int32_t*>(wins4 + W.inc);
            int32_t* rgb_list = reinterpret_cast<int32_t*>(wins4 + W.list0);
            int32_t* list13 = reinterpret_cast<int32_t*>(wins4 + W.list1);
            int32_t* list7 = reinterpret_cast<int32_t*>(wins4 + W.list2);
            int32_t* rgb_count = reinterpret_cast<int32_t*>(wins4 + W.counts);
            int32_t* count13 = rgb_count + 1;
            int32_t* pilot_flag = rgb_count + 6;
            int32_t* pilot_ctr = rgb_count + 8;
            const bool compact_on = bc7_compact_lists();
            const dim3 blk(TPB);
            const ChunkSel ALL{0, 1, 0, nullptr, 0};
            auto scan_rgb = [&](const int32_t* list, const int32_t* count, bool do13, bool do02, int32_t split = 0, ChunkSel sel = ChunkSel{0, 1, 0, nullptr, 0},
                                int32_t cnt = -1, hipStream_t s = nullptr, uint32_t* wins = nullptr, int32_t rows = 0, const uint4* compact = nullptr) {
                ScanTasks T;
                T.n = 0;
                if (on13 && do13) T.kind[T.n++] = WK_SCAN13;
                if (on02 && do02) T.kind[T.n++] = WK_SCAN02;
                if (T.n == 0) return;
                if (cnt < 0) cnt = nchunks;
                if (!s) s = st;
                if (!wins) { wins = wins4; rows = (int32_t)n; }
                const int32_t c8 = ((cnt + 7) / 8) * 8;
                int32_t grain = 256;
                if (grain > c8) grain = c8;
                const int32_t groups = (c8 + grain - 1) / grain;
                const dim3 grid((unsigned)(groups * grain * T.n));
                if (r13) {
                    if (L.vec) hipLaunchKernelGGL((bc7_scan_all<true, true, false>),  grid, blk, 0, s, src, stride, bx, rows, wins, S, T, a13, a7, cnt, grain, list, count, split, sel, compact);
                    else       hipLaunchKernelGGL((bc7_scan_all<false, true, false>), grid, blk, 0, s, src, stride, bx, rows, wins, S, T, a13, a7, cnt, grain, list, count, split, sel, compact);
                } else {
                    if (L.vec) hipLaunchKernelGGL((bc7_scan_all<true, false, false>),  grid, blk, 0, s, src, stride, bx, rows, wins, S, T, a13, a7, cnt, grain, list, count, split, sel, compact);
                    else       hipLaunchKernelGGL((bc7_scan_all<false, false, false>), grid, blk, 0, s, src, stride, bx, rows, wins, S, T, a13, a7, cnt, grain, list, count, split, sel, compact);
                }
            };
            auto scan_7 = [&](const int32_t* list = nullptr, const int32_t* count = nullptr, int32_t split = 0, int32_t cnt = -1, hipStream_t s = nullptr,
                              uint32_t* wins = nullptr, int32_t rows = 0) {
                if (!on7) return;
                ScanTasks T7;
                T7.n = 1; T7.kind[0] = WK_SCAN7;
                if (cnt < 0) cnt = nchunks;
                if (!s) s = st;
                if (!wins) { wins = wins4; rows = (int32_t)n; }
                const int32_t chunks8 = ((cnt + 7) / 8) * 8;
                const dim3 grid((unsigned)chunks8);
                if (r7) {
                    if (L.vec) hipLaunchKernelGGL((bc7_scan_all<true, true, true>),  grid, blk, 0, s, src, stride, bx, rows, wins, S, T7, a13, a7, cnt, chunks8, list, count, split, ALL, (const uint4*)nullptr);
                    else       hipLaunchKernelGGL((bc7_scan_all<false, true, true>), grid, blk, 0, s, src, stride, bx, rows, wins, S, T7, a13, a7, cnt, chunks8, list, count, split, ALL, (const uint4*)nullptr);
                } else {
                    if (L.vec) hipLaunchKernelGGL((bc7_scan_all<true, false, true>),  grid, blk, 0, s, src, stride, bx, rows, wins, S, T7, a13, a7, cnt, chunks8, list, count, split, ALL, (const uint4*)nullptr);
                    else       hipLaunchKernelGGL((bc7_scan_all<false, false, true>), grid, blk, 0, s, src, stride, bx, rows, wins, S, T7, a13, a7, cnt, chunks8, list, count, split, ALL, (const uint4*)nullptr);
                }
            };
            auto finish = [&](auto phase, const int32_t* in_list, const int32_t* in_count, int32_t* out_list, int32_t* out_count,
                              int32_t* out_list7 = nullptr, int32_t* out_count7 = nullptr, ChunkSel sel = ChunkSel{0, 1, 0, nullptr, 0}, int32_t cnt = -1,
                              hipStream_t s = nullptr, const uint32_t* wins = nullptr, int32_t rows = 0, const uint4* in_compact = nullptr, uint4* out_compact = nullptr) {
                constexpr int PH = decltype(phase)::value;
                if (PH == 3 && out_count != rgb_count + 16 + PAIR_CTR_LIST && out_count != rgb_count + 16 + PAIR_CTR_WORDS + PAIR_CTR_LIST)
                    fail_msg("bc7_finish_all<3>: the list length must be word %d of a band's counter block", PAIR_CTR_LIST);
                if (cnt < 0) cnt = nchunks;
                if (!s) s = st;
                if (!wins) { wins = wins4; rows = (int32_t)n; }
                const dim3 grid((unsigned)cnt);
                if (L.vec) hipLaunchKernelGGL((bc7_finish_all<true, PH>),  grid, blk, 0, s, src, stride, bx, rows, dst, wins, S, alpha_err, in_list, in_count, out_list, out_count, out_list7, out_count7, sel, in_compact, out_compact);
                else       hipLaunchKernelGGL((bc7_finish_all<false, PH>), grid, blk, 0, s, src, stride, bx, rows, dst, wins, S, alpha_err, in_list, in_count, out_list, out_count, out_list7, out_count7, sel, in_compact, out_compact);
            };
            const bool bounded = bc7_bounded_order() && on02 && on13 && !r13;
            if (bc7_alpha_first(S)) {
                ITW_CHECK(hipMemsetAsync(rgb_count, 0, 16 * sizeof(int32_t), st));
                if (bounded && on7 && !r7 && (S.mode_selection[2] || S.mode_selection[3])) {
                    const bool two = bc7_bands() > 1 && aux && !aux->single && aux->stream && nchunks >= 32;
                    int32_t stripe = nchunks / 16;
                    stripe = stripe < 1 ? 1 : (stripe > 64 ? 64 : stripe);
                    const int32_t stripes = (nchunks + stripe - 1) / stripe;
                    auto chain = [&](int k, hipStream_t s) {
                        const ChunkSel sel{two ? 1 : 0, stripe, k, nullptr, 0};
                        const int32_t cnt = two ? ((stripes + 1 - k) / 2) * stripe : nchunks;
                        const size_t cap = W.band[0].cap;
                        int32_t* lrgb = rgb_list + (two ? k * cap : 0); int32_t* l13 = list13 + (two ? k * cap : 0); int32_t* l7 = list7 + (two ? k * cap : 0);
                        int32_t* crgb = rgb_count + (k ? 11 : 0); int32_t* c13 = rgb_count + (k ? 12 : 1); int32_t* c7 = rgb_count + (k ? 13 : 2);
                        uint32_t* wins = two ? wins4 + W.band[k].wins : wins4;
                        const int32_t rows = two ? cnt * TPB : (int32_t)n;
                        finish(std::integral_constant<int, 6>{}, nullptr, nullptr, lrgb, crgb, l7, c7, sel, cnt, s);
                        scan_rgb(lrgb, crgb, false, true, 0, ALL, cnt, s);
                        finish(std::integral_constant<int, 5>{}, lrgb, crgb, l13, c13, l7, c7, ALL, cnt, s);
                        scan_rgb(l13, c13, true, false, 1, ALL, cnt, s, wins, rows);
                        finish(std::integral_constant<int, 4>{}, l13, c13, nullptr, nullptr, nullptr, nullptr, ALL, cnt, s, wins, rows);
                        scan_7(l7, c7, 1, cnt, s, wins, rows);
                        finish(std::integral_constant<int, 7>{}, l7, c7, nullptr, nullptr, nullptr, nullptr, ALL, cnt, s, wins, rows);
                    };
                    if (!two) chain(0, st);
                    else {
                        ITW_CHECK(hipEventRecord(aux->fork, st));
                        ITW_CHECK(hipStreamWaitEvent(aux->stream, aux->fork, 0));
                        chain(1, aux->stream);
                        chain(0, st);
                        ITW_CHECK(hipEventRecord(aux->join, aux->stream));
                        ITW_CHECK(hipStreamWaitEvent(st, aux->join, 0));
                    }
                } else {
                    scan_7();
                    finish(std::integral_constant<int, 1>{}, nullptr, nullptr, rgb_list, rgb_count);
                    if (bounded) {
                        scan_rgb(rgb_list, rgb_count, false, true);
                        finish(std::integral_constant<int, 5>{}, rgb_list, rgb_count, list13, count13);
                        scan_rgb(list13, count13, true, false, 1);
                        finish(std::integral_constant<int, 4>{}, list13, count13, nullptr, nullptr);
                    } else {
                        scan_rgb(rgb_list, rgb_count, true, true);
                        finish(std::integral_constant<int, 2>{}, rgb_list, rgb_count, nullptr, nullptr);
                    }
                }
            } else if (bounded && !on7) {
                const bool two = bc7_bands() > 1 && aux && !aux->single && aux->stream && nchunks >= 32;
                const bool pairs = bc7_pairs_on();
                const bool pilot = two && bc7_pilot_threshold() >= 0 && aux->mid;
                int32_t stripe = nchunks / 16;
                stripe = stripe < 1 ? 1 : (stripe > 64 ? 64 : stripe);
                const int32_t stripes = (nchunks + stripe - 1) / stripe;
                struct Band { ChunkSel sel; int32_t cnt; hipStream_t s; int32_t* list; int32_t* count; uint32_t* wins; int32_t rows; uint4* compact; PairRegion P; int32_t* redo; };
                auto band = [&](int k, hipStream_t s) {
                    const ListRegion& r = W.band[k];
                    Band B{ChunkSel{two ? 1 : 0, stripe, k, nullptr, 0}, two ? ((stripes + 1 - k) / 2) * stripe : nchunks, s,
                           reinterpret_cast<int32_t*>(wins4 + r.list), nullptr, wins4 + r.wins, 0, compact_on ? reinterpret_cast<uint4*>(wins4 + r.compact) : nullptr,
                           PairRegion{reinterpret_cast<uint64_t*>(wins4 + r.pair_words), reinterpret_cast<int32_t*>(wins4 + r.pair_buckets), reinterpret_cast<int32_t*>(wins4 + r.pair_ctr),
                                      bc7_pair_cap((int32_t)(two ? r.pair_cap : 2 * r.pair_cap))}, reinterpret_cast<int32_t*>(wins4 + r.pair_redo)};
                    B.count = B.P.ctr + PAIR_CTR_LIST;
                    B.rows = B.cnt * TPB;
                    if (!two) { B.list = list13; B.wins = wins4; B.rows = (int32_t)n; }
                    return B;
                };
                auto gated = [&](const Band& B, int32_t want) { ChunkSel g = B.sel; if (pilot) { g.gate = pilot_flag; g.want = want; } return g; };
                auto head = [&](const Band& B) { scan_rgb(nullptr, nullptr, false, true, 0, B.sel, B.cnt, B.s); };
                auto tail = [&](const Band& B) {
                    finish(std::integral_constant<int, 3>{}, nullptr, nullptr, B.list, B.count, nullptr, nullptr, gated(B, 1), B.cnt, B.s, nullptr, 0, nullptr, B.compact);
                    if (pairs) {
                        int32_t* redo_count = B.P.ctr + PAIR_CTR_REDO;
                        hipLaunchKernelGGL(bc7_pair_scan, dim3((unsigned)((B.cnt + 1) / 2)), blk, 0, B.s, src, stride, bx, B.list, B.compact, S, B.P);
                        finish(std::integral_constant<int, 8>{}, B.list, B.count, B.redo, redo_count, nullptr, B.P.ctr + PAIR_CTR_OVERFLOW, ALL, B.cnt, B.s,
                               reinterpret_cast<const uint32_t*>(B.P.words), B.rows, B.compact);
                        scan_rgb(B.redo, redo_count, true, false, 1, ALL, B.cnt, B.s, B.wins, B.rows);
                        finish(std::integral_constant<int, 4>{}, B.redo, redo_count, nullptr, nullptr, nullptr, nullptr, ALL, B.cnt, B.s, B.wins, B.rows);
                    } else {
                        scan_rgb(B.list, B.count, true, false, 1, ALL, B.cnt, B.s, B.wins, B.rows, B.compact);
                        finish(std::integral_constant<int, 4>{}, B.list, B.count, nullptr, nullptr, nullptr, nullptr, ALL, B.cnt, B.s, B.wins, B.rows, B.compact);
                    }
                    if (pilot) {
                        scan_rgb(nullptr, nullptr, true, false, 0, gated(B, 0), B.cnt, B.s);
                        finish(std::integral_constant<int, 0>{}, nullptr, nullptr, nullptr, nullptr, nullptr, nullptr, gated(B, 0), B.cnt, B.s);
                    }
                };
                auto setup = [&](const Band& A, const Band& Bb) {
                    const PairTarget off{PairRegion{nullptr, nullptr, nullptr, 0}, nullptr};
                    hipLaunchKernelGGL(bc7_bounded_setup, dim3(1), blk, 0, st, rgb_count, pairs ? PairTarget{A.P, A.redo} : off, pairs ? PairTarget{Bb.P, Bb.redo} : off);
                };
                if (!two) {
                    const Band B = band(0, st);
                    setup(B, B);
                    const bool probe = aux && aux->probe && aux->verdict && aux->verdict->event;
                    if (probe) scan_rgb(nullptr, nullptr, false, true, 0, ChunkSel{2, 1, 0, nullptr, 0}, (nchunks + 7) / 8, st);
                    else head(B);
                    if (aux && aux->verdict && aux->verdict->event) {
                        const dim3 grid((unsigned)((B.cnt + 7) / 8));
                        if (L.vec) hipLaunchKernelGGL((bc7_pilot_estimate<true>),  grid, blk, 0, st, src, stride, bx, (int32_t)n, wins4, S.skip_mode2 ? 1 : 0, B.sel, pilot_ctr, 256, pilot_flag, aux->verdict->host_counts_dev);
                        else       hipLaunchKernelGGL((bc7_pilot_estimate<false>), grid, blk, 0, st, src, stride, bx, (int32_t)n, wins4, S.skip_mode2 ? 1 : 0, B.sel, pilot_ctr, 256, pilot_flag, aux->verdict->host_counts_dev);
                        ITW_CHECK(hipEventRecord(aux->verdict->event, st));
                        aux->verdict->valid = true;
                    }
                    if (probe) return;
                    tail(B);
                } else {
                    hipStream_t s2 = aux->stream;
                    const Band A = band(0, st), Bb = band(1, s2);
                    setup(A, Bb);
                    ITW_CHECK(hipEventRecord(aux->fork, st));
                    ITW_CHECK(hipStreamWaitEvent(s2, aux->fork, 0));
                    head(Bb); head(A);
                    if (pilot) {
                        const dim3 grid((unsigned)((A.cnt + 7) / 8));
                        if (L.vec) hipLaunchKernelGGL((bc7_pilot_estimate<true>),  grid, blk, 0, st, src, stride, bx, (int32_t)n, wins4, S.skip_mode2 ? 1 : 0, A.sel, pilot_ctr, bc7_pilot_threshold(), pilot_flag, (int32_t*)nullptr);
                        else       hipLaunchKernelGGL((bc7_pilot_estimate<false>), grid, blk, 0, st, src, stride, bx, (int32_t)n, wins4, S.skip_mode2 ? 1 : 0, A.sel, pilot_ctr, bc7_pilot_threshold(), pilot_flag, (int32_t*)nullptr);
                        ITW_CHECK(hipEventRecord(aux->mid, st));
                        ITW_CHECK(hipStreamWaitEvent(s2, aux->mid, 0));
                    }
                    tail(Bb); tail(A);
                    ITW_CHECK(hipEventRecord(aux->join, s2));
                    ITW_CHECK(hipStreamWaitEvent(st, aux->join, 0));
                    if (bc7_pilot_debug()) {
                        int32_t h[16 + 2 * PAIR_CTR_WORDS];
                        ITW_CHECK(hipStreamSynchronize(st));
                        ITW_CHECK(hipMemcpy(h, rgb_count, sizeof h, hipMemcpyDeviceToHost));
                        std::fprintf(stderr, "bc7 pilot: estimate %d of %d sampled blocks listed -> %s; lists %d + %d of %lld blocks\n", h[8], h[9], h[6] ? "bounded" : "reference order",
                                     h[16 + PAIR_CTR_LIST], h[16 + PAIR_CTR_WORDS + PAIR_CTR_LIST], (long long)n);
                        for (int k = 0; k < 2 && pairs; k++) {
                            int32_t c[PAIR_CTR_WORDS];
                            ITW_CHECK(hipMemcpy(c, (k ? Bb : A).P.ctr, sizeof c, hipMemcpyDeviceToHost));
                            long long sum = 0; int32_t top = 0;
                            for (int i = 0; i < 64; i++) { sum += c[i]; top = c[i] > top ? c[i] : top; }
                            std::fprintf(stderr, "bc7 pairs: band %d: %lld pairs, fullest bucket %d of %d, overflow %d, deferred to the full scan %d\n", k, sum, top, (k ? Bb : A).P.cap,
                                         c[PAIR_CTR_OVERFLOW], c[PAIR_CTR_REDO]);
                        }
                    }
                }
            } else {
                scan_rgb(nullptr, nullptr, true, true);
                scan_7();
                finish(std::integral_constant<int, 0>{}, nullptr, nullptr, nullptr, nullptr);
            }
            return;
        }
    }
    if (S.mode_selection[0]) { launch_search<F_MODES02, 0>(L); launch_finish<F_MODES02>(L); }
    if (S.mode_selection[1] && (S.fastSkipTreshold_mode1 > 0 || S.fastSkipTreshold_mode3 > 0)) {
        if (ranked(S.fastSkipTreshold_mode1) || ranked(S.fastSkipTreshold_mode3)) {
            if (small(S.fastSkipTreshold_mode1) && small(S.fastSkipTreshold_mode3)) launch_search<F_MODES13, 2>(L);
            else launch_search<F_MODES13, 1>(L);
        } else launch_search<F_MODES13, 0>(L);
        launch_finish<F_MODES13>(L);
    }
    if (S.mode_selection[1] && S.fastSkipTreshold_mode7 > 0) {
        if (ranked(S.fastSkipTreshold_mode7)) {
            if (small(S.fastSkipTreshold_mode7)) launch_search<F_MODE7, 2>(L); else launch_search<F_MODE7, 1>(L);
        } else launch_search<F_MODE7, 0>(L);
        launch_finish<F_MODE7>(L);
    }
    if (S.mode_selection[2] || S.mode_selection[3]) launch_finish<F_MODES456>(L);
    if (L.first) ITW_CHECK(hipMemsetAsync(dst, 0, (size_t)n * 16, st));
}

}
```

intel-texture-works-plugin_amd/csrc/bc7_exact.hpp:

```cpp
#pragma once
#include "bcn_core.hpp"

namespace itw {

#define BCN_TABLE_QUAL __device__ const
#include "bc7_bytemasks.h"
#undef BCN_TABLE_QUAL

typedef short s16x2 __attribute__((ext_vector_type(2)));
__device__ __forceinline__ s16x2 as_s16x2(uint32_t v) { return __builtin_bit_cast(s16x2, v); }
__device__ __forceinline__ uint32_t as_u32(s16x2 v) { return __builtin_bit_cast(uint32_t, v); }
__device__ __forceinline__ uint32_t pk_sub(uint32_t a, uint32_t b) { return as_u32(as_s16x2(a) - as_s16x2(b)); }
__device__ __forceinline__ uint32_t pk_add(uint32_t a, uint32_t b) { return as_u32(as_s16x2(a) + as_s16x2(b)); }
__device__ __forceinline__ int32_t dot2(uint32_t a, uint32_t b, int32_t c)
{
    return __builtin_amdgcn_sdot2(as_s16x2(a), as_s16x2(b), c, false);
}
__device__ __forceinline__ uint32_t udot4(uint32_t a, uint32_t b, uint32_t c) { return __builtin_amdgcn_udot4(a, b, c, false); }
__device__ __forceinline__ uint32_t mul_lo_u16(uint32_t a, uint32_t b) { uint32_t d; asm("v_mul_lo_u16 %0, %1, %2" : "=v"(d) : "v"(a), "v"(b)); return d; }
__device__ __forceinline__ uint32_t add_u16(uint32_t a, uint32_t b) { uint32_t d; asm("v_add_u16 %0, %1, %2" : "=v"(d) : "v"(a), "v"(b)); return d; }
__device__ __forceinline__ uint32_t add32_u16(uint32_t a) { uint32_t d; asm("v_add_u16 %0, 32, %1" : "=v"(d) : "v"(a)); return d; }
__device__ __forceinline__ uint32_t ashr6_i16(uint32_t a) { uint32_t d; asm("v_ashrrev_i16 %0, 6, %1" : "=v"(d) : "v"(a)); return d; }
__device__ __forceinline__ uint32_t pack16(int32_t lo, int32_t hi) { return (uint32_t)lo | ((uint32_t)hi << 16); }
__device__ __forceinline__ int32_t imed3(int32_t v, int32_t lo, int32_t hi) { return min(max(v, lo), hi); }
// ... 6 lines not shown
struct Tex {
    uint32_t w[16];
    uint32_t pl[4][4];
    __device__ __forceinline__ float get(int p, int k) const { return (float)((w[k] >> (8 * p)) & 255u); }
    __device__ __forceinline__ uint32_t pair01(int k) const { return __builtin_amdgcn_perm(0u, w[k], 0x0c010c00u); }
    template <bool ALPHA>
    __device__ __forceinline__ uint32_t pair23(int k) const
    {
        return ALPHA ? __builtin_amdgcn_perm(0u, w[k], 0x0c030c02u) : ((w[k] >> 16) & 255u);
    }
    __device__ __forceinline__ void make_planar()
    {
        const int grp[4][4] = {{0, 2, 4, 6}, {1, 3, 5, 7}, {8, 10, 12, 14}, {9, 11, 13, 15}};
#pragma unroll
        for (int d = 0; d < 4; d++) {
            const uint32_t a = w[grp[d][0]], b = w[grp[d][1]], c = w[grp[d][2]], e = w[grp[d][3]];
            const uint32_t t0 = __builtin_amdgcn_perm(b, a, 0x05010400u);
            const uint32_t t1 = __builtin_amdgcn_perm(b, a, 0x07030602u);
            const uint32_t u0 = __builtin_amdgcn_perm(e, c, 0x05010400u);
            const uint32_t u1 = __builtin_amdgcn_perm(e, c, 0x07030602u);
            pl[0][d] = __builtin_amdgcn_perm(u0, t0, 0x05040100u);
            pl[1][d] = __builtin_amdgcn_perm(u0, t0, 0x07060302u);
            pl[2][d] = __builtin_amdgcn_perm(u1, t1, 0x05040100u);
            pl[3][d] = __builtin_amdgcn_perm(u1, t1, 0x07060302u);
        }
    }
    __device__ __forceinline__ void fence()
    {
#pragma unroll
        for (int k = 0; k < 16; k++) asm volatile("" : "+v"(w[k]));
#pragma unroll
        for (int c = 0; c < 4; c++)
#pragma unroll
            for (int d = 0; d < 4; d++) asm volatile("" : "+v"(pl[c][d]));
    }
};

struct SubsetMask {
    uint32_t bits;
    uint32_t bm[4];
    int32_t n;
};

__device__ __forceinline__ SubsetMask subset_of(int shape, int j)
{
    const uint32_t masks = BCN_SUBSET_MASKS[shape];
    const uint32_t m0 = masks & 0xffffu, m1 = masks >> 16;
    const uint32_t* t = BCN_BYTEMASK + shape * 8;
    SubsetMask s;
    if (j == 0)      { s.bits = m0; for (int d = 0; d < 4; d++) s.bm[d] = t[d]; }
    else if (j == 1) { s.bits = m1; for (int d = 0; d < 4; d++) s.bm[d] = t[4 + d]; }
    else             { s.bits = ~(m0 | m1) & 0xffffu; for (int d = 0; d < 4; d++) s.bm[d] = ~(t[d] | t[4 + d]); }
    s.n = __builtin_popcount(s.bits);
    return s;
}

__device__ __forceinline__ SubsetMask whole_block()
{
    return SubsetMask{0xffffu, {0xffffffffu, 0xffffffffu, 0xffffffffu, 0xffffffffu}, 16};
}

template <int CH>
struct IStats {
    int32_t m[10];
    int32_t s[4];
    int32_t n;
};

template <int CH>
__device__ __forceinline__ void stats_int(IStats<CH>& st, const uint32_t (&pl)[4][4], const SubsetMask& sm)
{
    uint32_t r[4], g[4], b[4], a[4];
#pragma unroll
    for (int d = 0; d < 4; d++) {
        r[d] = pl[0][d] & sm.bm[d]; g[d] = pl[1][d] & sm.bm[d]; b[d] = pl[2][d] & sm.bm[d];
        a[d] = (CH == 4) ? (pl[3][d] & sm.bm[d]) : 0u;
    }
    uint32_t m[10] = {0, 0, 0, 0, 0, 0, 0, 0, 0, 0}, s[4] = {0, 0, 0, 0};
#pragma unroll
    for (int d = 0; d < 4; d++) {
        m[0] = udot4(r[d], pl[0][d], m[0]); m[1] = udot4(r[d], pl[1][d], m[1]); m[2] = udot4(r[d], pl[2][d], m[2]);
        m[4] = udot4(g[d], pl[1][d], m[4]); m[5] = udot4(g[d], pl[2][d], m[5]);
        m[7] = udot4(b[d], pl[2][d], m[7]);
        s[0] = udot4(r[d], 0x01010101u, s[0]); s[1] = udot4(g[d], 0x01010101u, s[1]); s[2] = udot4(b[d], 0x01010101u, s[2]);
        if (CH == 4) {
            m[3] = udot4(r[d], pl[3][d], m[3]); m[6] = udot4(g[d], pl[3][d], m[6]); m[8] = udot4(b[d], pl[3][d], m[8]);
            m[9] = udot4(a[d], pl[3][d], m[9]);
            s[3] = udot4(a[d], 0x01010101u, s[3]);
        }
    }
#pragma unroll
    for (int i = 0; i < 10; i++) st.m[i] = (int32_t)m[i];
#pragma unroll
    for (int i = 0; i < 4; i++) st.s[i] = (int32_t)s[i];
    st.n = sm.n;
}

template <int CH>
__device__ __forceinline__ void stats_sub(IStats<CH>& a, const IStats<CH>& b)
{
#pragma unroll
    for (int i = 0; i < 10; i++) a.m[i] -= b.m[i];
#pragma unroll
    for (int i = 0; i < 4; i++) a.s[i] -= b.s[i];
    a.n -= b.n;
}

#ifndef ITW_BOUND_SQUARINGS
#define ITW_BOUND_SQUARINGS 1
#endif
__device__ const float BOUND_SLACK3[17] = {
    0.f, 0.866026282f, 1.22474611f, 1.50000155f, 1.73205256f, 1.93649364f, 2.12132239f, 2.29129004f, 2.44949222f, 2.59807873f,
    2.73861551f, 2.87228417f, 3.0000031f, 3.12250209f, 3.24037361f, 3.35410523f, 3.46410513f};

__device__ __forceinline__ float subset_residual_bound(const IStats<3>& st)
{
    const int32_t n = st.n;
    const int32_t c00 = n * st.m[0] - st.s[0] * st.s[0], c01 = n * st.m[1] - st.s[0] * st.s[1], c02 = n * st.m[2] - st.s[0] * st.s[2];
    const int32_t c11 = n * st.m[4] - st.s[1] * st.s[1], c12 = n * st.m[5] - st.s[1] * st.s[2], c22 = n * st.m[7] - st.s[2] * st.s[2];
    const float t = (float)(c00 + c11 + c22);
    const float inv = __builtin_amdgcn_rcpf(fmaxf(t, 1.0f));
    const float a = (float)c00 * inv, b = (float)c01 * inv, c = (float)c02 * inv, d = (float)c11 * inv, e = (float)c12 * inv, f = (float)c22 * inv;
    const float bb = b * b, cc = c * c, ee = e * e;
    const float A = a * a + bb + cc, B = a * b + b * d + c * e, C = a * c + b * e + c * f;
    const float D = bb + d * d + ee, E = b * c + d * e + e * f, F = cc + ee + f * f;
#if ITW_BOUND_SQUARINGS == 1
    const float off1 = B * B + C * C + E * E;
    const float fro1 = (A * A + D * D + F * F) + (off1 + off1);
    const float lam = __builtin_amdgcn_sqrtf(__builtin_amdgcn_sqrtf(fro1));
#else
    const float BB = B * B, CC = C * C, EE = E * E;
    const float A2 = A * A + BB + CC, B2 = A * B + B * D + C * E, C2 = A * C + B * E + C * F;
    const float D2 = BB + D * D + EE, E2 = B * C + D * E + E * F, F2 = CC + EE + F * F;
    const float off = B2 * B2 + C2 * C2 + E2 * E2;
    const float fro2 = (A2 * A2 + D2 * D2 + F2 * F2) + (off + off);
    const float lam = __builtin_amdgcn_sqrtf(__builtin_amdgcn_sqrtf(__builtin_amdgcn_sqrtf(fro2)));
#endif
    const float r = ((a + d + f) - lam) - 1e-5f;
    return fmaxf(r, 0.0f) * t;
}

__device__ __forceinline__ float two_subset_bound(int shape, const uint32_t (&pl)[4][4], const IStats<3>& full)
{
    const SubsetMask sm = subset_of(shape, 0);
    IStats<3> s0, s1 = full;
    stats_int<3>(s0, pl, sm);
    stats_sub<3>(s1, s0);
    const float d0 = __builtin_amdgcn_sqrtf(subset_residual_bound(s0) * rcp_of_count(s0.n)) * 0.999999f - BOUND_SLACK3[s0.n];
    const float d1 = __builtin_amdgcn_sqrtf(subset_residual_bound(s1) * rcp_of_count(s1.n)) * 0.999999f - BOUND_SLACK3[s1.n];
    const float e0 = fmaxf(d0, 0.0f), e1 = fmaxf(d1, 0.0f);
    return (e0 * e0 + e1 * e1) * 0.999999f;
}

template <int CH>
__device__ __forceinline__ void stats_float(Stats<CH>& f, const IStats<CH>& st)
{
#pragma unroll
    for (int i = 0; i < 10; i++) f.m[i] = (float)st.m[i];
#pragma unroll
    for (int i = 0; i < 4; i++) f.s[i] = (float)st.s[i];
    f.n = (float)st.n;
}

template <int CH>
__device__ __forceinline__ void fit_line(float (&ep)[2][4], const Tex& tx, uint32_t mask, const IStats<CH>& ist, float rn, const SeedTables& T)
{
    Stats<CH> st;
    stats_float<CH>(st, ist);
    float cv[10];
    covariance_of<CH>(cv, st, rn);
    float dc[4];
#pragma unroll
    for (int p = 0; p < CH; p++) dc[p] = st.s[p] * rn;

    const float inv_var = 1.0f / 65536.0f;
#pragma unroll
    for (int i = 0; i < 10; i++) cv[i] *= inv_var;
    const float eps = 0.001f * 0.001f;
    cv[0] += eps; cv[4] += eps; cv[7] += eps; cv[9] += eps;

    float axis[4];
    principal_axis<CH, 8, true>(axis, cv, T);

    float lo = __builtin_inff(), hi = -__builtin_inff();
    float probe = axis[0];
#pragma unroll
    for (int p = 1; p < CH; p++) probe += axis[p];
    probe *= 0.0f;
    if (__builtin_expect(probe != probe, 0)) {
#pragma unroll
        for (int k = 0; k < 16; k++) {
            if ((mask >> k) & 1u) {
                float dot = axis[0] * (tx.get(0, k) - dc[0]);
#pragma unroll
                for (int p = 1; p < CH; p++) dot += axis[p] * (tx.get(p, k) - dc[p]);
                lo = fmin_x86(lo, dot);
                hi = fmax_x86(hi, dot);
            }
        }
    } else {
#pragma unroll
        for (int k = 0; k < 16; k++) {
            if ((mask >> k) & 1u) {
                float dot = axis[0] * (tx.get(0, k) - dc[0]);
#pragma unroll
                for (int p = 1; p < CH; p++) dot += axis[p] * (tx.get(p, k) - dc[p]);
                lo = vmin_raw(lo, dot);
                hi = vmax_raw(hi, dot);
            }
        }
    }
    if (hi - lo < 1.0f) { lo -= 0.5f; hi += 0.5f; }
#pragma unroll
    for (int p = 0; p < CH; p++) {
        ep[0][p] = fclamp_num(lo * axis[p] + dc[p], 0.f, 255.f);
        ep[1][p] = fclamp_num(hi * axis[p] + dc[p], 0.f, 255.f);
    }
}

struct Segment {
    uint32_t a01, ba01;
    uint32_t a23, ba23;
    float k0, k1;
};

template <int BITS, int CH>
__device__ __forceinline__ Segment make_segment(const int32_t (&d)[2][4])
{
    Segment s;
    s.a01 = pack16(d[0][0], d[0][1]);
    s.ba01 = pk_sub(pack16(d[1][0], d[1][1]), s.a01);
    int32_t dd;
    if (CH == 4) {
        s.a23 = pack16(d[0][2], d[0][3]);
        s.ba23 = pk_sub(pack16(d[1][2], d[1][3]), s.a23);
        dd = dot2(s.ba01, s.ba01, dot2(s.ba23, s.ba23, 0));
    } else {
        const int32_t ba2 = d[1][2] - d[0][2];
        s.a23 = (uint32_t)d[0][2];
        s.ba23 = (uint32_t)ba2;
        dd = dot2(s.ba01, s.ba01, ba2 * ba2);
    }
    const float dn = -(float)dd;
    const float r = (dd == 0) ? 0.0f : 1.0f / dn;
    if (BITS <= 3) {
        s.k0 = (float)(1 << BITS) * r;
        s.k1 = 0.5f - 0.25f * r;
    } else {
        s.k0 = dn;
        s.k1 = r;
    }
    return s;
}

template <int BITS>
__device__ __forceinline__ uint32_t weight_selector(int32_t q) { return (uint32_t)q * 0x00010001u + 0x0c000c00u; }
template <int BITS>
__device__ __forceinline__ uint32_t weight_from_selector(uint32_t sel)
{
    if (BITS == 2) return __builtin_amdgcn_perm(0u, 0x402b1500u, sel);
    return __builtin_amdgcn_perm(0x40372e25u, 0x1b120900u, sel);
}
__device__ __forceinline__ uint32_t weight_pair4(int32_t q) { return (((uint32_t)q * 68u + 8u) >> 4) * 0x00010001u; }

template <int BITS, int CH>
__device__ __forceinline__ void select_texel(int32_t& q_out, int32_t& e_out, const Segment& sg, uint32_t t01, uint32_t t23)
{
    constexpr int LEVELS = 1 << BITS;
    const uint32_t at01 = pk_sub(sg.a01, t01);
    uint32_t at23;
    int32_t m;
    if (CH == 4) {
        at23 = pk_sub(sg.a23, t23);
        m = dot2(at01, sg.ba01, dot2(at23, sg.ba23, 0));
    } else {
        at23 = sg.a23 - t23;
        m = dot2(at01, sg.ba01, (int32_t)at23 * (int32_t)sg.ba23);
    }
    const float mf = (float)m;
    float x;
    if (BITS <= 3) {
        x = __builtin_fmaf(mf, sg.k0, sg.k1);
    } else {
        float q = mf * sg.k1;
        const float rem = __builtin_fmaf(-q, sg.k0, mf);
        q = __builtin_fmaf(rem, sg.k1, q);
        x = __builtin_fmaf(q, (float)LEVELS, 0.5f);
    }
    const int32_t q1 = imed3((int32_t)x, 1, LEVELS - 1);

    uint32_t w0, w1;
    if (BITS <= 3) {
        const uint32_t sel = weight_selector<BITS>(q1);
        w1 = weight_from_selector<BITS>(sel);
        w0 = weight_from_selector<BITS>(sel - 0x00010001u);
    } else {
        w1 = weight_pair4(q1); w0 = weight_pair4(q1 - 1);
    }
    const s16x2 k32 = {32, 32}, six = {6, 6};
    const uint32_t x0_01 = pk_add(as_u32((as_s16x2(w0) * as_s16x2(sg.ba01) + k32) >> six), at01);
    const uint32_t x1_01 = pk_add(as_u32((as_s16x2(w1) * as_s16x2(sg.ba01) + k32) >> six), at01);
    int32_t e0, e1;
    if (CH == 4) {
        const uint32_t x0_23 = pk_add(as_u32((as_s16x2(w0) * as_s16x2(sg.ba23) + k32) >> six), at23);
        const uint32_t x1_23 = pk_add(as_u32((as_s16x2(w1) * as_s16x2(sg.ba23) + k32) >> six), at23);
        e0 = dot2(x0_01, x0_01, dot2(x0_23, x0_23, 0));
// ... 337 lines not shown
```

intel-texture-works-plugin_amd/csrc/kernels.hpp:

```cpp
#pragma once
#include <hip/hip_runtime.h>
#include <stdint.h>
#include "../../include/ispc_texcomp.h"

namespace itw {

void launch_bc1 (const uint8_t* src, int64_t stride, int width, int height, uint8_t* dst, hipStream_t st);
void launch_bc3 (const uint8_t* src, int64_t stride, int width, int height, uint8_t* dst, hipStream_t st);
void launch_etc1(const uint8_t* src, int64_t stride, int width, int height, uint8_t* dst, int threshold, hipStream_t st);
void launch_bc4 (const uint8_t* src, int64_t stride, int width, int height, uint8_t* dst, hipStream_t st);
void launch_bc5 (const uint8_t* src, int64_t stride, int width, int height, uint8_t* dst, hipStream_t st);
void launch_bc4s(const uint8_t* src, int64_t stride, int width, int height, uint8_t* dst, hipStream_t st);
void launch_bc5s(const uint8_t* src, int64_t stride, int width, int height, uint8_t* dst, hipStream_t st);
void warmup_bc45s();
void copy_bc45_closest_snorm(uint8_t* host_out, hipStream_t st);
void warmup_bc45();
void copy_bc45_index_table(uint32_t* host_out, hipStream_t st);
size_t bc7_workspace_bytes(int width, int height, int64_t wide_max_blocks = 0, const bc7_enc_settings* settings = nullptr);
void set_bc7_path(int path);
bool bc7_scans_every_shape(const bc7_enc_settings& s);
bool bc7_has_order_verdict(const bc7_enc_settings& s);
bool bc7_staged_bands_ok();
void set_bc7_pilot(int percent);
struct Bc7Verdict { hipEvent_t event; volatile int32_t* host_counts; bool valid; int32_t* host_counts_dev; };
struct Bc7Aux { hipStream_t stream; hipEvent_t fork, join; int64_t wide_max_blocks; hipEvent_t mid; bool single; Bc7Verdict* verdict; bool probe; };
void launch_bc7 (const uint8_t* src, int64_t stride, int width, int height, uint8_t* dst,
                 const bc7_enc_settings& s, float* workspace, hipStream_t st, const Bc7Aux* aux = nullptr);
void launch_bc7_test_bounds(const uint8_t* src, int64_t stride, int width, int height, float* out, hipStream_t st);
size_t bc6h_workspace_bytes(int width, int height, const bc6h_enc_settings& s);
void launch_bc6h(const uint8_t* src, int64_t stride, int width, int height, uint8_t* dst,
                 const bc6h_enc_settings& s, hipStream_t st, void* workspace = nullptr);
void set_bc6h_path(int path);

__device__ __forceinline__ int bc45_fill_index(int i, int valid)
{
    const int s = i < valid ? i : (i == 3 ? 1 : 0);
    return s < valid ? s : 0;
}

struct ChainImage { const uint8_t* ptr; int64_t stride; int32_t width, height; int64_t first_block; };
void launch_chain_gather(const ChainImage* images, int nimg, int64_t nblocks, int packed_bx, int packed_by, int texel_bytes, bool fill45,
                         uint8_t* dst, int64_t dst_pitch, hipStream_t st, uint8_t* extents = nullptr);

}
```

intel-texture-works-plugin_amd/itw_amd/__init__.py:

```python
from .abi import (
    lib, test_lib, TEST_HOOK_SYMBOLS, lib_path, RgbaSurface, Bc7Settings, Bc6hSettings, EtcSettings, BC7_PROFILES, BC6H_PROFILES,
    bc7_profile, bc6h_profile, etc_profile, compress, compress_numpy, band_for_part, version, device_info,
    BYTES_PER_BLOCK, EXPORTED_SYMBOLS, DXGI_FORMAT, DdsDesc, image_func, compress_image, PROGRESS_FUNC, pad_to_multiple_of_4, dds_file, decode, block_count, KEEPS_PARTIAL_BLOCKS, SIGNED_FORMATS,
    available, set_error_mode, last_error, ON_ERROR_ABORT, ON_ERROR_RETURN, set_bc7_path, set_bc7_pilot, compress_image_multigpu, multigpu_sub_bands, MultiGpuStats, source_sha256, bc7_two_subset_bounds,
    chain_bytes, compress_chain, mip_chain, decode_chain, decode_image, load_dds, dds_images,
    KtxDesc, ktx_file, ktx_images, load_ktx,
    ErrorStats, OWN_CHANNELS, measure, measure_async, measure_chain, stats_from_tensor,
    RefineStats, compress_refined, RefinePolicy, RefineTargetStats, compress_refined_to, psnr_to_total_sse,
    compress_chain_refined, compress_chain_refined_to, chain_psnr_to_total_sse,
)
```

intel-texture-works-plugin_amd/itw_amd/abi.py:

```python
import ctypes as C
import os

_PKG = os.path.dirname(os.path.abspath(__file__))
_LIB = os.path.normpath(os.path.join(_PKG, "..", "lib", "libispc_texcomp.so"))
_TEST_LIB = os.path.normpath(os.path.join(_PKG, "..", "lib", "libispc_texcomp_test.so"))

BYTES_PER_BLOCK = {"bc1": 8, "bc3": 16, "bc7": 16, "bc6h": 16, "bc4": 8, "bc5": 16, "bc4_snorm": 8, "bc5_snorm": 16, "etc1": 8}
KEEPS_PARTIAL_BLOCKS = ("bc4", "bc5", "bc4_snorm", "bc5_snorm")
SIGNED_FORMATS = ("bc4_snorm", "bc5_snorm")
BC7_PROFILES = ("ultrafast", "veryfast", "fast", "basic", "slow",
                "alpha_ultrafast", "alpha_veryfast", "alpha_fast", "alpha_basic", "alpha_slow")
BC6H_PROFILES = ("veryfast", "fast", "basic", "slow", "veryslow")

EXPORTED_SYMBOLS = tuple(
    ["CompressBlocksBC1", "CompressBlocksBC3", "CompressBlocksBC6H", "CompressBlocksBC7"]
    + ["GetProfile_" + p for p in BC7_PROFILES] + ["GetProfile_bc6h_" + p for p in BC6H_PROFILES]
    + ["itwSetStream", "itwGetStream", "itwAvailable", "itwSetErrorMode", "itwLastError", "itwClearError", "itwSetBc7Path", "itwSetBc7Pilot",
       "itwDeviceInfo", "itwVersion", "itwBandForPart", "itwBandForPartEx", "itwGetProfile_etc_slow", "itwCompressBlocksETC1"]
    + ["GetProcessorCount", "InitWin32Threads", "DestroyThreads", "GetBytesPerBlock", "CompressImageMT", "CompressImageST",
       "CompressImageBC1", "CompressImageBC3", "CompressImageBC4", "CompressImageBC5", "CompressImageBC4S", "CompressImageBC5S"]
    + ["CompressImageBC7_" + p for p in BC7_PROFILES] + ["CompressImageBC6H_" + p for p in BC6H_PROFILES]
    + ["itwCompressImageSliced", "itwCompressImageSlicedEx", "itwChainBytes", "itwCompressImageChain", "itwCompressImageChainEx", "itwCompressImageRefined", "itwCompressImageRefinedTo", "itwPsnrToTotalSse", "itwCompressImageChainRefined", "itwCompressImageChainRefinedTo", "itwChainPsnrToTotalSse", "itwSetSliceWindow", "itwSliceWindow", "itwSliceWindowFor", "itwPadToMultipleOf4", "itwFreeSurface", "itwPadToMultipleOf4Device",
       "itwConvertToRGBA8Device", "itwConvertToRGBA16FDevice"]
    + ["itwMultiGpuRanks", "itwMultiGpuTransport", "itwMultiGpuPeerLinks", "itwCompressImageMultiGPU", "itwCompressImageMultiGPUEx", "itwCompressImageMultiGPUBands",
       "itwMultiGpuSetInterleave", "itwMultiGpuPieces"]
    + ["CompressBlocksBC4", "CompressBlocksBC5", "itwWarmupBC45", "CompressBlocksBC4S", "CompressBlocksBC5S", "itwWarmupBC45S"]
    + ["itwDecodeBlocks", "itwDecodeChain", "itwDecodeImage", "itwMeasureBlocks", "itwMeasureChain", "itwStatsPsnr"]
    + ["itwDdsLevelBytes", "itwDdsHeaderBytes", "itwDdsFileBytes", "itwDdsWriteHeader", "itwDdsReadHeader", "itwDdsWriteFile", "itwDdsImage"]
    + ["itwKtxHeaderBytes", "itwKtxFileBytes", "itwKtxWriteHeader", "itwKtxReadHeader", "itwKtxWriteFile", "itwKtxImage"])
TEST_HOOK_SYMBOLS = ("itwTestRcp", "itwTestRsqrt", "itwTestF2I", "itwTestBc7TwoSubsetBounds", "itwTestBc45IndexTable", "itwTestBc45ClosestS",
                     "itwMultiGpuTestInjectFailure", "itwTestCombinerHold", "itwTestCombinerCounters")




class RgbaSurface(C.Structure):
    _fields_ = [("ptr", C.c_void_p), ("width", C.c_int32), ("height", C.c_int32), ("stride", C.c_int32)]


class Bc7Settings(C.Structure):
    _fields_ = [("mode_selection", C.c_bool * 4), ("refineIterations", C.c_int * 8),
                ("skip_mode2", C.c_bool), ("fastSkipTreshold_mode1", C.c_int),
                ("fastSkipTreshold_mode3", C.c_int), ("fastSkipTreshold_mode7", C.c_int),
                ("mode45_channel0", C.c_int), ("refineIterations_channel", C.c_int),
                ("channels", C.c_int)]


class Bc6hSettings(C.Structure):
    _fields_ = [("slow_mode", C.c_bool), ("fast_mode", C.c_bool), ("refineIterations_1p", C.c_int),
                ("refineIterations_2p", C.c_int), ("fastSkipTreshold", C.c_int)]


class EtcSettings(C.Structure):
    _fields_ = [("fastSkipTreshold", C.c_int)]


assert C.sizeof(RgbaSurface) == 24 and C.sizeof(Bc7Settings) == 64 and C.sizeof(Bc6hSettings) == 16 and C.sizeof(EtcSettings) == 4

DXGI_FORMAT = {"etc1": 0x8D64, "bc1": 71, "bc1_srgb": 72, "bc3": 77, "bc3_srgb": 78, "bc4": 80, "bc4_snorm": 81, "bc5": 83, "bc5_snorm": 84, "bc6h": 95, "bc6h_sf16": 96, "bc7": 98, "bc7_srgb": 99}


class DdsDesc(C.Structure):
    _fields_ = [("width", C.c_uint32), ("height", C.c_uint32), ("mip_levels", C.c_uint32), ("dxgi_format", C.c_uint32),
                ("is_cubemap", C.c_uint32), ("array_size", C.c_uint32)]


class KtxDesc(C.Structure):
    _fields_ = [("width", C.c_uint32), ("height", C.c_uint32), ("mip_levels", C.c_uint32), ("gl_internal_format", C.c_uint32),
                ("is_cubemap", C.c_uint32), ("key_value_bytes", C.c_uint32)]


class MultiGpuRankStats(C.Structure):
    _fields_ = [("rank", C.c_int32), ("device", C.c_int32), ("block_row0", C.c_int32), ("block_rows", C.c_int32),
                ("upload_ms", C.c_float), ("encode_ms", C.c_float), ("gather_ms", C.c_float), ("span_ms", C.c_float)]


class MultiGpuStats(C.Structure):
    _fields_ = [("ranks", C.c_int32), ("devices", C.c_int32), ("peer_links", C.c_int32), ("rccl_ranks", C.c_int32),
                ("watchdog_fired", C.c_int32), ("resident_bands", C.c_int32), ("wall_ms", C.c_float), ("posted_ms", C.c_float),
                ("transport", C.c_char * 8), ("transport_note", C.c_char * 96), ("rank", MultiGpuRankStats * 64),
                ("interleave", C.c_int32)]

    def as_dict(self):
        n = max(0, min(int(self.ranks), 64))
        return {"ranks": int(self.ranks), "devices": int(self.devices), "peer_links": int(self.peer_links), "rccl_ranks": int(self.rccl_ranks),
                "watchdog_fired": bool(self.watchdog_fired), "resident_bands": bool(self.resident_bands), "interleave": int(self.interleave),
                "wall_ms": round(float(self.wall_ms), 4), "posted_ms": round(float(self.posted_ms), 4),
                "transport": self.transport.decode(), "transport_note": self.transport_note.decode(),
                "per_rank": [{"rank": int(r.rank), "device": int(r.device), "block_row0": int(r.block_row0), "block_rows": int(r.block_rows),
                              "upload_ms": round(float(r.upload_ms), 4), "encode_ms": round(float(r.encode_ms), 4),
                              "gather_ms": round(float(r.gather_ms), 4), "span_ms": round(float(r.span_ms), 4)} for r in self.rank[:n]]}


OWN_CHANNELS = {"bc1": "rgb", "bc3": "rgba", "bc4": "r", "bc5": "rg", "bc4_snorm": "r", "bc5_snorm": "rg", "bc6h": "rgb", "bc7": "rgba", "etc1": "rgb"}
_DXGI_BASE = {71: "bc1", 72: "bc1", 77: "bc3", 78: "bc3", 80: "bc4", 81: "bc4_snorm", 83: "bc5", 84: "bc5_snorm", 95: "bc6h", 96: "bc6h",
              98: "bc7", 99: "bc7", 0x8D64: "etc1"}


def _base(fmt):
    return fmt if fmt in SIGNED_FORMATS else fmt.split("_")[0]


def _check_texel_type(fmt, img):
    if fmt in SIGNED_FORMATS and not str(img.dtype).endswith(".int8") and str(img.dtype) != "int8":
        raise TypeError(f"{fmt} encodes RGBA8_SNORM: pass an int8 array / tensor, not {img.dtype} "
                        "(view uint8 bytes as int8 if they are two's complement codes)")


def _channel_mask(channels):
    mask = 0
    for c in channels:
        mask |= 1 << ("rgba".index(c.lower()) if isinstance(c, str) else int(c))
    assert 0 <= mask < 16
    return mask


class ErrorStats(C.Structure):
    _fields_ = [("dxgi_format", C.c_int32), ("width", C.c_int32), ("height", C.c_int32), ("reserved_blocks", C.c_uint32),
                ("blocks", C.c_uint64), ("sse", C.c_uint64 * 4), ("max_abs", C.c_uint32 * 4), ("worst_block_sse", C.c_uint64),
                ("worst_block", C.c_uint32), ("_pad", C.c_uint32), ("mode_hist", C.c_uint64 * 16)]

    def _mask(self, channels):
        return _channel_mask(OWN_CHANNELS[_DXGI_BASE[int(self.dxgi_format)]] if channels is None else channels)

    def mse(self, channels=None):
        mask = self._mask(channels)
        picked = [c for c in range(4) if mask >> c & 1]
        return sum(int(self.sse[c]) for c in picked) / float(int(self.width) * int(self.height) * len(picked))

    def psnr(self, channels=None):
        if _DXGI_BASE.get(int(self.dxgi_format)) == "bc6h":
            raise ValueError("PSNR is not defined for BC6H code differences; use sse / max_abs")
        return float(lib().itwStatsPsnr(C.byref(self), self._mask(channels)))

    def as_dict(self):
        return {"dxgi_format": int(self.dxgi_format), "width": int(self.width), "height": int(self.height),
                "reserved_blocks": int(self.reserved_blocks), "blocks": int(self.blocks), "sse": [int(v) for v in self.sse],
                "max_abs": [int(v) for v in self.max_abs], "worst_block_sse": int(self.worst_block_sse), "worst_block": int(self.worst_block),
                "mode_hist": [int(v) for v in self.mode_hist]}

    def __eq__(self, other):
        return isinstance(other, ErrorStats) and bytes(self) == bytes(other)

    __hash__ = None


assert C.sizeof(ErrorStats) == 216


class RefineStats(C.Structure):
    _fields_ = [("blocks", C.c_uint64), ("listed", C.c_uint64), ("replaced", C.c_uint64), ("sse_first", C.c_uint64), ("sse_final", C.c_uint64),
                ("worst_first", C.c_uint64), ("worst_final", C.c_uint64)]

    def as_dict(self):
        return {name: int(getattr(self, name)) for name, _ in self._fields_}


assert C.sizeof(RefineStats) == 56


class RefinePolicy(C.Structure):
    _fields_ = [("max_listed", C.c_uint64), ("target_total_sse", C.c_uint64)]


class RefineTargetStats(C.Structure):
    _fields_ = [("total", RefineStats), ("rounds", C.c_uint32), ("target_met", C.c_uint32), ("budget", C.c_uint64 * 5), ("listed", C.c_uint64 * 5)]

    def as_dict(self):
        d = self.total.as_dict()
        d.update(rounds=int(self.rounds), target_met=int(self.target_met), budget=[int(v) for v in self.budget],
                 listed_per_round=[int(v) for v in self.listed])
        return d


assert C.sizeof(RefinePolicy) == 16 and C.sizeof(RefineTargetStats) == 144
UINT64_MAX = 2 ** 64 - 1

COMPRESSION_FUNC = C.CFUNCTYPE(None, C.POINTER(RgbaSurface), C.c_void_p)
PROGRESS_FUNC = C.CFUNCTYPE(C.c_bool, C.c_int, C.c_int, C.c_void_p)

_lib = None
_test_lib = None


def lib_path():
    return _LIB


def lib():
    global _lib
    if _lib is None:
        _lib = _load(_LIB, hooks=False)
    return _lib


def test_lib():
    global _test_lib
    if _test_lib is None:
        _test_lib = _load(_TEST_LIB, hooks=True)
    return _test_lib


def _load(path, hooks):
    if True:
        if not os.path.exists(path):
            raise RuntimeError(
                f"{path} is missing: build it with `python -c 'import __graft_entry__ as g; g.build()'` "
                "or `make -C intel-texture-works-plugin_amd/csrc`.  There is no CPU fallback.")
        L = C.CDLL(path, mode=C.RTLD_LOCAL if hooks else C.RTLD_GLOBAL)
        L.CompressBlocksBC1.argtypes = [C.POINTER(RgbaSurface), C.c_void_p]
        L.CompressBlocksBC4.argtypes = [C.POINTER(RgbaSurface), C.c_void_p]
        L.CompressBlocksBC5.argtypes = [C.POINTER(RgbaSurface), C.c_void_p]
        L.CompressBlocksBC4.restype = None
        L.itwWarmupBC45.restype = None
        for n in ("CompressBlocksBC4S", "CompressBlocksBC5S", "CompressImageBC4S", "CompressImageBC5S"):
            getattr(L, n).argtypes = [C.POINTER(RgbaSurface), C.c_void_p]
            getattr(L, n).restype = None
        L.itwWarmupBC45S.restype = None
        L.CompressBlocksBC5.restype = None
        L.CompressBlocksBC3.argtypes = [C.POINTER(RgbaSurface), C.c_void_p]
        L.CompressBlocksBC7.argtypes = [C.POINTER(RgbaSurface), C.c_void_p, C.POINTER(Bc7Settings)]
        L.CompressBlocksBC6H.argtypes = [C.POINTER(RgbaSurface), C.c_void_p, C.POINTER(Bc6hSettings)]
        for n in ("CompressBlocksBC1", "CompressBlocksBC3", "CompressBlocksBC7", "CompressBlocksBC6H"):
            getattr(L, n).restype = None
        L.itwGetProfile_etc_slow.argtypes = [C.POINTER(EtcSettings)]
        L.itwGetProfile_etc_slow.restype = None
        L.itwCompressBlocksETC1.argtypes = [C.POINTER(RgbaSurface), C.c_void_p, C.POINTER(EtcSettings)]
        L.itwCompressBlocksETC1.restype = None
        L.itwSetStream.argtypes = [C.c_void_p]
        L.itwSetStream.restype = None
        L.itwGetStream.restype = C.c_void_p
        L.itwDeviceInfo.restype = C.c_char_p
        L.itwAvailable.restype = C.c_int
        L.itwSetErrorMode.argtypes = [C.c_int]
        L.itwSetErrorMode.restype = None
        L.itwLastError.restype = C.c_char_p
        L.itwClearError.restype = None
        L.itwSetBc7Path.argtypes = [C.c_int]
        L.itwSetBc7Path.restype = None
        L.itwSetBc7Pilot.argtypes = [C.c_int]
        L.itwSetBc7Pilot.restype = None
        L.itwVersion.restype = C.c_char_p
        L.itwBandForPart.argtypes = [C.c_int32] * 5 + [C.POINTER(C.c_int32)] * 2
        L.itwBandForPart.restype = C.c_int64
        L.itwBandForPartEx.argtypes = [C.c_int32] * 6 + [C.POINTER(C.c_int32)] * 2
        L.itwBandForPartEx.restype = C.c_int64
        if hooks:
            for n in ("itwTestRcp", "itwTestRsqrt", "itwTestF2I"):
                getattr(L, n).argtypes = [C.c_void_p, C.c_void_p, C.c_int64]
                getattr(L, n).restype = None
            L.itwTestBc7TwoSubsetBounds.argtypes = [C.POINTER(RgbaSurface), C.c_void_p]
            L.itwTestBc7TwoSubsetBounds.restype = None
            L.itwTestBc45IndexTable.argtypes = [C.c_void_p]
            L.itwTestBc45IndexTable.restype = C.c_int
            L.itwTestBc45ClosestS.argtypes = [C.c_void_p]
            L.itwTestBc45ClosestS.restype = C.c_int
            L.itwMultiGpuTestInjectFailure.argtypes = [C.c_int, C.c_int, C.c_int]
            L.itwMultiGpuTestInjectFailure.restype = None
            L.itwTestCombinerHold.argtypes = [C.c_int, C.c_int]
            L.itwTestCombinerHold.restype = None
            L.itwTestCombinerCounters.argtypes = [C.POINTER(C.c_int64)]
            L.itwTestCombinerCounters.restype = None
        L.GetProcessorCount.restype = C.c_int
        L.GetBytesPerBlock.argtypes = [C.c_int]
        L.GetBytesPerBlock.restype = C.c_int
        for n in ("CompressImageMT", "CompressImageST"):
            getattr(L, n).argtypes = [C.POINTER(RgbaSurface), C.c_void_p, C.c_void_p, C.c_int]
            getattr(L, n).restype = C.c_bool
        for n in ["CompressImageBC1", "CompressImageBC3"] + ["CompressImageBC7_" + p for p in BC7_PROFILES] \
                + ["CompressImageBC6H_" + p for p in BC6H_PROFILES]:
            getattr(L, n).argtypes = [C.POINTER(RgbaSurface), C.c_void_p]
            getattr(L, n).restype = None
        L.itwCompressImageSliced.argtypes = [C.POINTER(RgbaSurface), C.c_void_p, C.c_int64, C.c_void_p, C.c_int, C.c_bool,
                                             C.c_int64, C.c_void_p, C.c_void_p]
        L.itwCompressImageSliced.restype = C.c_bool
        L.itwCompressImageSlicedEx.argtypes = [C.POINTER(RgbaSurface), C.c_void_p, C.c_int64, C.c_int, C.c_void_p, C.c_int64, C.c_void_p, C.c_void_p]
        L.itwCompressImageSlicedEx.restype = C.c_bool
        L.itwChainBytes.argtypes = [C.c_void_p, C.c_int, C.c_int]
        L.itwChainBytes.restype = C.c_int64
        L.itwCompressImageChain.argtypes = [C.c_void_p, C.c_int, C.c_void_p, C.c_void_p, C.c_int, C.c_void_p, C.c_void_p]
        L.itwCompressImageChain.restype = C.c_bool
        L.itwCompressImageChainEx.argtypes = [C.c_void_p, C.c_int, C.c_void_p, C.c_int, C.c_void_p, C.c_void_p, C.c_void_p]
        L.itwCompressImageChainEx.restype = C.c_bool
        L.itwCompressImageRefined.argtypes = [C.POINTER(RgbaSurface), C.c_void_p, C.c_int, C.c_void_p, C.c_void_p, C.c_uint32, C.c_uint64,
                                              C.c_void_p, C.c_size_t, C.c_void_p, C.c_void_p]
        L.itwCompressImageRefined.restype = C.c_bool
        L.itwCompressImageRefinedTo.argtypes = [C.POINTER(RgbaSurface), C.c_void_p, C.c_int, C.c_void_p, C.c_void_p, C.c_uint32, C.c_void_p, C.c_size_t,
                                                C.c_void_p, C.c_size_t, C.c_void_p, C.c_void_p]
        L.itwCompressImageRefinedTo.restype = C.c_bool
        L.itwPsnrToTotalSse.argtypes = [C.c_int, C.c_int, C.c_int, C.c_uint32, C.c_double]
        L.itwPsnrToTotalSse.restype = C.c_uint64
        L.itwCompressImageChainRefined.argtypes = [C.c_void_p, C.c_int, C.c_void_p, C.c_int, C.c_void_p, C.c_void_p, C.c_uint32, C.c_uint64,
                                                   C.c_void_p, C.c_size_t, C.c_void_p, C.c_void_p, C.c_void_p]
        L.itwCompressImageChainRefined.restype = C.c_bool
        L.itwCompressImageChainRefinedTo.argtypes = [C.c_void_p, C.c_int, C.c_void_p, C.c_int, C.c_void_p, C.c_void_p, C.c_uint32, C.c_void_p, C.c_size_t,
                                                     C.c_void_p, C.c_size_t, C.c_void_p, C.c_void_p, C.c_void_p]
        L.itwCompressImageChainRefinedTo.restype = C.c_bool
        L.itwChainPsnrToTotalSse.argtypes = [C.c_void_p, C.c_int, C.c_int, C.c_uint32, C.c_double]
        L.itwChainPsnrToTotalSse.restype = C.c_uint64
        L.itwSetSliceWindow.argtypes = [C.c_int]
        L.itwSetSliceWindow.restype = None
        L.itwSliceWindow.argtypes = [C.c_int, C.c_int, C.c_int, C.c_int64]
        L.itwSliceWindow.restype = C.c_int
        L.itwSliceWindowFor.argtypes = [C.c_int, C.c_void_p, C.c_int, C.c_int, C.c_int64]
        L.itwSliceWindowFor.restype = C.c_int
        L.itwMultiGpuRanks.restype = C.c_int
        L.itwMultiGpuSetInterleave.argtypes = [C.c_int]
        L.itwMultiGpuSetInterleave.restype = None
        L.itwMultiGpuPieces.argtypes = [C.c_int32, C.c_int, C.c_int]
        L.itwMultiGpuPieces.restype = C.c_int
        L.itwMultiGpuTransport.restype = C.c_char_p
        L.itwMultiGpuPeerLinks.restype = C.c_int
        L.itwCompressImageMultiGPU.argtypes = [C.POINTER(RgbaSurface), C.c_void_p, C.c_void_p, C.c_int, C.c_int]
        L.itwCompressImageMultiGPU.restype = C.c_bool
        L.itwCompressImageMultiGPUEx.argtypes = [C.POINTER(RgbaSurface), C.c_void_p, C.c_void_p, C.c_int, C.c_int, C.POINTER(RgbaSurface),
                                                 C.POINTER(MultiGpuStats)]
        L.itwCompressImageMultiGPUEx.restype = C.c_bool
        L.itwCompressImageMultiGPUBands.argtypes = [C.POINTER(RgbaSurface), C.c_void_p, C.c_void_p, C.c_int, C.c_int, C.POINTER(RgbaSurface), C.c_int,
                                                    C.POINTER(MultiGpuStats)]
        L.itwCompressImageMultiGPUBands.restype = C.c_bool
        L.itwPadToMultipleOf4.argtypes = [C.POINTER(RgbaSurface), C.c_int]
        L.itwPadToMultipleOf4.restype = RgbaSurface
        L.itwFreeSurface.argtypes = [C.POINTER(RgbaSurface)]
        L.itwFreeSurface.restype = None
        L.itwPadToMultipleOf4Device.argtypes = [C.POINTER(RgbaSurface), C.c_int, C.c_void_p]
        L.itwPadToMultipleOf4Device.restype = None
        L.itwConvertToRGBA8Device.argtypes = [C.c_void_p, C.c_int, C.c_int, C.c_int, C.c_int, C.c_int, C.c_int, C.c_void_p]
        L.itwConvertToRGBA8Device.restype = C.c_int
        L.itwConvertToRGBA16FDevice.argtypes = [C.c_void_p, C.c_int, C.c_int, C.c_int, C.c_int, C.c_int, C.c_void_p]
        L.itwConvertToRGBA16FDevice.restype = C.c_int
        L.itwDecodeBlocks.argtypes = [C.c_int, C.c_void_p, C.c_int, C.c_int, C.c_void_p, C.c_int64, C.c_void_p]
        L.itwDecodeBlocks.restype = C.c_int
        L.itwDecodeChain.argtypes = [C.c_int, C.c_void_p, C.c_void_p, C.c_int, C.c_void_p, C.c_void_p]
        L.itwDecodeChain.restype = C.c_int
        L.itwDecodeImage.argtypes = [C.c_int, C.c_void_p, C.c_void_p, C.c_void_p, C.c_void_p]
        L.itwDecodeImage.restype = C.c_int
        L.itwMeasureBlocks.argtypes = [C.c_int, C.c_void_p, C.POINTER(RgbaSurface), C.c_void_p, C.c_size_t, C.c_void_p]
        L.itwMeasureBlocks.restype = C.c_int
        L.itwMeasureChain.argtypes = [C.c_void_p, C.c_int, C.c_void_p, C.c_int, C.c_void_p, C.c_size_t]
        L.itwMeasureChain.restype = C.c_int
        L.itwStatsPsnr.argtypes = [C.POINTER(ErrorStats), C.c_uint32]
        L.itwStatsPsnr.restype = C.c_double
        L.itwDdsLevelBytes.argtypes = [C.c_uint32, C.c_uint32, C.c_uint32]
        L.itwDdsLevelBytes.restype = C.c_size_t
        for n in ("itwDdsHeaderBytes", "itwDdsFileBytes"):
            getattr(L, n).argtypes = [C.POINTER(DdsDesc)]
            getattr(L, n).restype = C.c_size_t
        L.itwDdsWriteHeader.argtypes = [C.POINTER(DdsDesc), C.c_void_p, C.c_size_t]
        L.itwDdsWriteHeader.restype = C.c_size_t
        L.itwDdsReadHeader.argtypes = [C.c_void_p, C.c_size_t, C.POINTER(DdsDesc)]
        L.itwDdsReadHeader.restype = C.c_size_t
        L.itwDdsWriteFile.argtypes = [C.POINTER(DdsDesc), C.POINTER(C.c_void_p), C.c_size_t, C.c_void_p, C.c_size_t]
        L.itwDdsWriteFile.restype = C.c_size_t
        L.itwDdsImage.argtypes = [C.POINTER(DdsDesc), C.c_uint32, C.POINTER(C.c_uint32), C.POINTER(C.c_uint32), C.POINTER(C.c_size_t)]
        L.itwDdsImage.restype = C.c_size_t
        for n in ("itwKtxHeaderBytes", "itwKtxFileBytes"):
            getattr(L, n).argtypes = [C.POINTER(KtxDesc)]
            getattr(L, n).restype = C.c_size_t
        L.itwKtxWriteHeader.argtypes = [C.POINTER(KtxDesc), C.c_void_p, C.c_size_t]
        L.itwKtxWriteHeader.restype = C.c_size_t
        L.itwKtxReadHeader.argtypes = [C.c_void_p, C.c_size_t, C.POINTER(KtxDesc)]
        L.itwKtxReadHeader.restype = C.c_size_t
        L.itwKtxWriteFile.argtypes = [C.POINTER(KtxDesc), C.POINTER(C.c_void_p), C.c_size_t, C.c_void_p, C.c_size_t]
        L.itwKtxWriteFile.restype = C.c_size_t
        L.itwKtxImage.argtypes = [C.POINTER(KtxDesc), C.c_uint32, C.POINTER(C.c_uint32), C.POINTER(C.c_uint32), C.POINTER(C.c_size_t)]
        L.itwKtxImage.restype = C.c_size_t
    return L


def version():
    return lib().itwVersion().decode()


def source_sha256():
    import hashlib
    d = os.path.normpath(os.path.join(_PKG, "..", "csrc"))
    h = hashlib.sha256()
    for name in sorted(os.listdir(d)):
        if name.endswith((".hip", ".hpp", ".h")) or name == "Makefile":
            h.update(name.encode() + b"\0")
            with open(os.path.join(d, name), "rb") as f:
                h.update(f.read())
    return h.hexdigest()


ON_ERROR_ABORT, ON_ERROR_RETURN = 0, 1
BC7_PATH = {"auto": 0, "deep": 1, "wide": 2}


def set_bc7_pilot(percent):
    lib().itwSetBc7Pilot(-2 if percent is None else int(percent))


def set_bc7_path(name):
    lib().itwSetBc7Path(BC7_PATH[name])


def available():
    return bool(lib().itwAvailable())


def set_error_mode(mode):
    lib().itwSetErrorMode(mode)


def last_error():
    e = lib().itwLastError()
    return e.decode() if e else None


def device_info():
    return lib().itwDeviceInfo().decode()


def bc7_profile(name):
    if name not in BC7_PROFILES:
        raise KeyError(name)
    s = Bc7Settings()
    getattr(lib(), "GetProfile_" + name)(C.byref(s))
    return s


def bc6h_profile(name):
    if name not in BC6H_PROFILES:
        raise KeyError(name)
    s = Bc6hSettings()
    getattr(lib(), "GetProfile_bc6h_" + name)(C.byref(s))
    return s


def etc_profile(name="slow"):
    if name != "slow":
        raise KeyError(name)
    s = EtcSettings()
    lib().itwGetProfile_etc_slow(C.byref(s))
    return s


def band_for_part(width, height, fmt, part, parts):
    y0, n = C.c_int32(), C.c_int32()
    off = lib().itwBandForPartEx(width, height, BYTES_PER_BLOCK[fmt], part, parts, 1 if fmt in KEEPS_PARTIAL_BLOCKS else 0, C.byref(y0), C.byref(n))
    if off < 0:
        raise ValueError((part, parts))
    return y0.value, n.value, off


def _call(fmt, surf, dst_ptr, settings):
    L = lib()
    if fmt == "bc1":
        L.CompressBlocksBC1(C.byref(surf), dst_ptr)
    elif fmt == "bc3":
        L.CompressBlocksBC3(C.byref(surf), dst_ptr)
    elif fmt == "bc4":
        L.CompressBlocksBC4(C.byref(surf), dst_ptr)
    elif fmt == "bc5":
        L.CompressBlocksBC5(C.byref(surf), dst_ptr)
    elif fmt == "bc4_snorm":
        L.CompressBlocksBC4S(C.byref(surf), dst_ptr)
    elif fmt == "bc5_snorm":
        L.CompressBlocksBC5S(C.byref(surf), dst_ptr)
    elif fmt == "bc7":
        st = settings if isinstance(settings, Bc7Settings) else bc7_profile(settings or "slow")
        L.CompressBlocksBC7(C.byref(surf), dst_ptr, C.byref(st))
    elif fmt == "bc6h":
        st = settings if isinstance(settings, Bc6hSettings) else bc6h_profile(settings or "slow")
        L.CompressBlocksBC6H(C.byref(surf), dst_ptr, C.byref(st))
    elif fmt == "etc1":
        st = settings if isinstance(settings, EtcSettings) else etc_profile(settings or "slow")
        L.itwCompressBlocksETC1(C.byref(surf), dst_ptr, C.byref(st))
    else:
        raise ValueError(fmt)


def block_count(fmt, width, height):
    if fmt in KEEPS_PARTIAL_BLOCKS:
        return ((width + 3) // 4) * ((height + 3) // 4)
    return (width // 4) * (height // 4)


def compress_numpy(fmt, img, settings=None):
    import numpy as np
    _check_texel_type(fmt, img)
    assert img.ndim == 3 and img.shape[2] == 4 and img.strides[2] == img.itemsize and img.strides[1] == 4 * img.itemsize
    assert img.dtype == (np.uint16 if fmt == "bc6h" else np.int8 if fmt in SIGNED_FORMATS else np.uint8)
    h, w = img.shape[:2]
    out = np.empty(block_count(fmt, w, h) * BYTES_PER_BLOCK[fmt], dtype=np.uint8)
    surf = RgbaSurface(img.ctypes.data, w, h, img.strides[0])
    _call(fmt, surf, out.ctypes.data, settings)
    return out


def compress(fmt, img, settings=None, out=None):
    import torch
    _check_texel_type(fmt, img)
    assert img.is_cuda and img.dim() == 3 and img.shape[2] == 4
    es = img.element_size()
    assert es == (2 if fmt == "bc6h" else 1), "texel type does not match the format"
    assert img.stride(2) == 1 and img.stride(1) == 4
    h, w = img.shape[:2]
    nbytes = block_count(fmt, w, h) * BYTES_PER_BLOCK[fmt]
    if out is None:
        out = torch.empty(nbytes, dtype=torch.uint8, device=img.device)
    assert out.is_cuda and out.numel() >= nbytes and out.is_contiguous()
    L = lib()
    with torch.cuda.device(img.device):
        L.itwSetStream(torch.cuda.current_stream(img.device).cuda_stream)
        surf = RgbaSurface(img.data_ptr(), w, h, img.stride(0) * es)
        _call(fmt, surf, out.data_ptr(), settings)
    return out


def bc7_two_subset_bounds(img):
    import torch
    assert img.is_cuda and img.dim() == 3 and img.shape[2] == 4 and img.element_size() == 1
    assert img.stride(2) == 1 and img.stride(1) == 4
    h, w = img.shape[:2]
    out = torch.empty(((h // 4) * (w // 4), 64), dtype=torch.float32, device=img.device)
    L = test_lib()
    with torch.cuda.device(img.device):
        L.itwSetStream(torch.cuda.current_stream(img.device).cuda_stream)
        surf = RgbaSurface(img.data_ptr(), w, h, img.stride(0))
        L.itwTestBc7TwoSubsetBounds(C.byref(surf), out.data_ptr())
    e = L.itwLastError()
    if e:
        raise RuntimeError(e.decode())
    return out


def image_func(fmt, profile=None, L=None):
    name = {"bc1": "CompressImageBC1", "bc3": "CompressImageBC3", "bc4": "CompressImageBC4", "bc5": "CompressImageBC5",
            "bc4_snorm": "CompressImageBC4S", "bc5_snorm": "CompressImageBC5S"}.get(fmt) or \
        ("CompressImageBC7_" if fmt == "bc7" else "CompressImageBC6H_") + (profile or "slow")
    return C.cast(getattr(L or lib(), name), C.c_void_p)


def compress_image(fmt, img, profile=None, multithreaded=True, slice_pixels=0, progress=None, out=None, settings=None):
    import numpy as np
    _check_texel_type(fmt, img)
    h, w = img.shape[:2]
    nbytes = block_count(fmt, w, h) * BYTES_PER_BLOCK[fmt]
    on_device = hasattr(img, "data_ptr")
    if on_device:
        import torch
        if out is None:
            out = torch.zeros(nbytes, dtype=torch.uint8, device=img.device)
        surf = RgbaSurface(img.data_ptr(), w, h, img.stride(0) * img.element_size())
        lib().itwSetStream(torch.cuda.current_stream(img.device).cuda_stream)
    else:
        if out is None:
            out = np.zeros(nbytes, dtype=np.uint8)
        surf = RgbaSurface(img.ctypes.data, w, h, img.strides[0])
    dst = out.data_ptr() if hasattr(out, "data_ptr") else out.ctypes.data
    cb = PROGRESS_FUNC(progress) if progress else None
    pitch = block_count(fmt, w, 4) * BYTES_PER_BLOCK[fmt]
    if fmt == "etc1" and settings is None:
        settings = etc_profile(profile or "slow")
    if settings is not None:
        ok = lib().itwCompressImageSlicedEx(C.byref(surf), dst, pitch, DXGI_FORMAT[fmt], C.cast(C.byref(settings), C.c_void_p), slice_pixels,
                                            C.cast(cb, C.c_void_p) if cb else None, None)
    else:
        ok = lib().itwCompressImageSliced(C.byref(surf), dst, pitch, image_func(fmt, profile),
                                          DXGI_FORMAT[fmt], multithreaded, slice_pixels, C.cast(cb, C.c_void_p) if cb else None, None)
    return bool(ok), out


def _surfaces(images):
    surfs = []
    for img in images:
        if hasattr(img, "data_ptr"):
            assert img.dim() == 3 and img.shape[2] == 4 and img.stride(2) == 1 and img.stride(1) == 4
            surfs.append(RgbaSurface(img.data_ptr(), img.shape[1], img.shape[0], img.stride(0) * img.element_size()))
        else:
            assert img.ndim == 3 and img.shape[2] == 4 and img.strides[2] == img.itemsize and img.strides[1] == 4 * img.itemsize
            surfs.append(RgbaSurface(img.ctypes.data, img.shape[1], img.shape[0], img.strides[0]))
    return (RgbaSurface * max(1, len(surfs)))(*surfs)


def chain_bytes(fmt, images):
    arr = (RgbaSurface * max(1, len(images)))(*[RgbaSurface(None, s[1], s[0], 0) if isinstance(s, tuple) else _surfaces([s])[0] for s in images])
    return int(lib().itwChainBytes(C.cast(arr, C.c_void_p), len(images), DXGI_FORMAT[fmt]))


def compress_chain(fmt, images, profile=None, settings=None, progress=None, out=None, cmp_func=None):
    import numpy as np
    fmt_key = fmt
    base = _base(fmt)
    for img in images:
        _check_texel_type(fmt, img)
    nbytes = sum(((img.shape[1] + 3) // 4) * ((img.shape[0] + 3) // 4) for img in images) * BYTES_PER_BLOCK[base]
    on_device = bool(images) and hasattr(images[0], "data_ptr")
    if out is None:
        if on_device:
            import torch
            out = torch.zeros(nbytes, dtype=torch.uint8, device=images[0].device)
        else:
            out = np.zeros(nbytes, dtype=np.uint8)
    if on_device or hasattr(out, "data_ptr"):
        import torch
        dev = images[0].device if on_device else out.device
        lib().itwSetStream(torch.cuda.current_stream(dev).cuda_stream)
    dst = out.data_ptr() if hasattr(out, "data_ptr") else out.ctypes.data
    arr = _surfaces(images)
    cb = PROGRESS_FUNC(progress) if progress else None
    cbp = C.cast(cb, C.c_void_p) if cb else None
    if cmp_func is not None:
        ok = lib().itwCompressImageChain(C.cast(arr, C.c_void_p), len(images), dst, cmp_func, DXGI_FORMAT[fmt_key], cbp, None)
    else:
        if settings is None and base == "bc7":
            settings = bc7_profile(profile or "slow")
        elif settings is None and base == "bc6h":
            settings = bc6h_profile(profile or "slow")
        elif settings is None and base == "etc1":
            settings = etc_profile(profile or "slow")
        sp = C.cast(C.byref(settings), C.c_void_p) if settings is not None else None
        ok = lib().itwCompressImageChainEx(C.cast(arr, C.c_void_p), len(images), dst, DXGI_FORMAT[fmt_key], sp, cbp, None)
    return bool(ok), out


def mip_chain(img):
    import numpy as np
    levels = [np.ascontiguousarray(img)]
    half = img.dtype == np.uint16
    while levels[-1].shape[0] > 1 or levels[-1].shape[1] > 1:
        a = levels[-1]
        f = a.view(np.float16).astype(np.float32) if half else a.astype(np.float32)
        h, w = a.shape[:2]
        nh, nw = max(1, h >> 1), max(1, w >> 1)
        f = np.pad(f, ((0, 2 * nh - h if 2 * nh > h else 0), (0, 2 * nw - w if 2 * nw > w else 0), (0, 0)), mode="edge")[:2 * nh, :2 * nw]
        m = 0.25 * (f[0::2, 0::2] + f[1::2, 0::2] + f[0::2, 1::2] + f[1::2, 1::2])
        levels.append(np.ascontiguousarray(m.astype(np.float16).view(np.uint16) if half else np.floor(m + 0.5).astype(np.uint8)))
    return levels


def multigpu_sub_bands(fmt, width, height, ranks, L=None):
    k = (L or lib()).itwMultiGpuPieces(height, ranks, 1 if fmt in KEEPS_PARTIAL_BLOCKS else 0)
    out = []
    for j in range(k * ranks):
        y0, rows, off = band_for_part(width, height, fmt, j, k * ranks)
        out.append((j, j % ranks, y0, rows, off))
    return out


def compress_image_multigpu(fmt, img, profile=None, ranks=0, out=None, bands=None, stats=None, L=None, interleave=None):
    import numpy as np
    L = L or lib()
    if interleave is not None:
        L.itwMultiGpuSetInterleave(int(interleave))
    if bands is not None:
        import torch
        h, w = (img if isinstance(img, tuple) else img.shape[:2])
        if not ranks:
            ranks = len(bands)
        assert len(bands) % ranks == 0, f"{len(bands)} resident surfaces for {ranks} ranks"
        for b in bands:
            assert b.is_cuda and b.dim() == 3 and b.shape[2] == 4 and b.stride(2) == 1 and b.stride(1) == 4 and b.shape[1] == w
            torch.cuda.synchronize(b.device)
        arr = (RgbaSurface * len(bands))(*[RgbaSurface(b.data_ptr(), w, b.shape[0], b.stride(0) * b.element_size()) for b in bands])
        on_gpu, src_ptr, stride = True, None, w * 4 * bands[0].element_size()
        first_dev = bands[0].device
    else:
        h, w = img.shape[:2]
        arr = None
        on_gpu = not isinstance(img, np.ndarray)
        src_ptr, stride = (img.data_ptr(), img.stride(0) * img.element_size()) if on_gpu else (img.ctypes.data, img.strides[0])
        first_dev = img.device if on_gpu else None
    nbytes = block_count(fmt, w, h) * BYTES_PER_BLOCK[fmt]
    if out is None:
        if on_gpu:
            import torch
            out = torch.empty(nbytes, dtype=torch.uint8, device=first_dev)
        else:
            out = np.empty(nbytes, dtype=np.uint8)
    dst_ptr = out.ctypes.data if isinstance(out, np.ndarray) else out.data_ptr()
    if on_gpu and bands is None:
        import torch
        torch.cuda.synchronize(img.device)
    surf = RgbaSurface(src_ptr, w, h, stride)
    if bands is None and stats is None:
        ok = L.itwCompressImageMultiGPU(C.byref(surf), dst_ptr, image_func(fmt, profile, L), DXGI_FORMAT[fmt], ranks)
    elif bands is not None and len(bands) != ranks:
        ok = L.itwCompressImageMultiGPUBands(C.byref(surf), dst_ptr, image_func(fmt, profile, L), DXGI_FORMAT[fmt], ranks, arr, len(bands),
# ... 499 lines not shown
```

Baseline: 3855 Mpixels/s.

## Split BC7 modes 4/5 rotation search into bounded per-rotation task lists

The single tail phase that ran modes 4/5/6 per block is split into three steps. First, a new phase computes a lower bound on the error for each rotation from the block's covariance and lists only the rotations that could beat the current best. Second, a dense task kernel runs the mode 4/5 scan on those lists and resolves the winner per block with an atomicMin on a packed word. Third, a final phase applies the winner and runs mode 6. The goal is to skip rotations that cannot win and to avoid wave divergence from mixed per-block work. In exchange it adds two kernel launches, extra workspace and atomics, and it relies on the bound being conservative to stay bit-exact.

```diff
diff --git a/include/itw_test_hooks.h b/include/itw_test_hooks.h
--- a/include/itw_test_hooks.h
+++ b/include/itw_test_hooks.h
@@ -14,6 +14,8 @@
 
 void itwTestBc7TwoSubsetBounds(const rgba_surface* d_src, float* d_out);
 
+void itwTestBc7RotationBounds(const rgba_surface* d_src, float* d_out);
+
 int itwTestBc45IndexTable(uint32_t* host_out);
 
 int itwTestBc45ClosestS(uint8_t* host_out);
diff --git a/intel-texture-works-plugin_amd/csrc/abi.hip b/intel-texture-works-plugin_amd/csrc/abi.hip
--- a/intel-texture-works-plugin_amd/csrc/abi.hip
+++ b/intel-texture-works-plugin_amd/csrc/abi.hip
@@ -1370,6 +1370,16 @@
     });
 }
 
+void itwTestBc7RotationBounds(const rgba_surface* d_src, float* d_out)
+{
+    itwClearError();
+    itw::guarded([&] {
+        if (!d_src || !d_src->ptr || !d_out) itw::fail_msg("null pointer");
+        itw::launch_bc7_test_rot_bounds(d_src->ptr, d_src->stride, d_src->width, d_src->height, d_out, tls.user_stream);
+        ITW_CHECK(hipGetLastError());
+    });
+}
+
 void itwTestRcp(const float* in, float* out, int64_t n)
 {
     if (n <= 0) return;
diff --git a/intel-texture-works-plugin_amd/csrc/bc7.hip b/intel-texture-works-plugin_amd/csrc/bc7.hip
--- a/intel-texture-works-plugin_amd/csrc/bc7.hip
+++ b/intel-texture-works-plugin_amd/csrc/bc7.hip
@@ -1183,6 +1183,9 @@
 struct PairTarget { PairRegion P; int32_t* redo; };
 static_assert(sizeof(PairTarget) <= (PAIR_CTR_WORDS - PAIR_CTR_TARGET) * sizeof(int32_t) && PAIR_CTR_TARGET % 2 == 0 && PAIR_CTR_WORDS % 4 == 0, "PairTarget behind the counters");
 constexpr int PAIR_MAX_PER_BLOCK = 32;
+struct RotRegion { int32_t* lists; int32_t* counts; unsigned long long* words; uint4* payload; int32_t cap; };
+constexpr int ROT_WORD_ROT_SHIFT = 29, ROT_WORD_MODE5_SHIFT = 31;
+constexpr unsigned long long ROT_WORD_POS_MASK = (1ull << ROT_WORD_ROT_SHIFT) - 1ull;
 constexpr unsigned long long PAIR_WORD_HEAVY = ~0ull - 1ull;
 
 struct ScanTasks { int n; int kind[3]; };
@@ -1308,17 +1311,18 @@
                const uint32_t* __restrict__ wins4, const bc7_enc_settings S, int32_t* __restrict__ inc_err,
                const int32_t* __restrict__ in_list, const int32_t* __restrict__ in_count, int32_t* __restrict__ out_list, int32_t* __restrict__ out_count,
                int32_t* __restrict__ out_list7, int32_t* __restrict__ out_count7, const ChunkSel sel,
-               const uint4* __restrict__ in_compact, uint4* __restrict__ out_compact)
+               const uint4* __restrict__ in_compact, uint4* __restrict__ out_compact, const RotRegion R)
 {
     constexpr bool LISTED = PHASE == 2 || PHASE == 4 || PHASE == 5 || PHASE == 7 || PHASE == 8;
-    constexpr bool DO02 = PHASE == 0 || PHASE == 2 || PHASE == 3 || PHASE == 5;
+    constexpr bool DO02 = PHASE == 0 || PHASE == 2 || PHASE == 3 || PHASE == 5 || PHASE == 9;
+    constexpr bool TAIL3 = PHASE == 3 || PHASE == 10;
     constexpr bool DO13 = PHASE == 0 || PHASE == 2 || PHASE == 4;
     constexpr bool DO7 = PHASE == 0 || PHASE == 1;
     constexpr bool DO456 = PHASE == 0 || PHASE == 1 || PHASE == 3 || PHASE == 6;
     __shared__ unsigned short s_seed16[2048];
     __shared__ uint32_t s_seed32[2048];
     __shared__ uint2 s_pal[(ITW_BC7_LANE_PAL ? LANE_PAL_LEVELS : 8) * TPB];
-    __shared__ int32_t s_at[PHASE == 3 ? TPB / 64 : 1][64];
+    __shared__ int32_t s_at[TAIL3 ? TPB / 64 : 1][64];
     if (sel.gate && *sel.gate != sel.want) return;
     const int32_t nact = LISTED ? *in_count : nblocks;
     const int32_t chunk = LISTED ? (int32_t)blockIdx.x : sel_chunk(sel, (int32_t)blockIdx.x);
@@ -1346,7 +1350,7 @@
     const bool on13 = S.mode_selection[1];
     int32_t e_alpha = ERR_MAX;
     if (PHASE == 2 || PHASE == 5) e_alpha = inc_err[b];
-    if (PHASE == 4 || PHASE == 7 || PHASE == 8) ln.best_err = inc_err[b];
+    if (PHASE == 4 || PHASE == 7 || PHASE == 8 || PHASE == 10) ln.best_err = inc_err[b];
     Win w;
     if (DO02 && S.mode_selection[0]) {
         unpack_win(w, wins4[(int64_t)wide_win_slot(0) * nblocks + b]);
@@ -1354,6 +1358,30 @@
         if (!S.skip_mode2) { ln.tx.fence(); unpack_win(w, wins4[(int64_t)wide_win_slot(2) * nblocks + b]); refine_and_commit<2>(ln, w, S.refineIterations[2], S.channels); }
     }
     const int32_t e02 = ln.best_err;
+    if (PHASE == 9) {
+        if (live) { inc_err[b] = e02; R.words[b] = ~0ull; }
+        ln.tx.fence();
+        IStats<3> full;
+        stats_int<3>(full, ln.tx.pl, whole_block());
+        const float lim = (float)e02 - 0.5f;
+        const bool on45 = live && S.mode_selection[2];
+#pragma unroll
+        for (int r = 0; r < 3; r++) {
+            const bool need = on45 && r >= S.mode45_channel0 && !(rotation_bound(r, full) >= lim);
+            append_to_list(R.lists + (int64_t)r * R.cap, R.counts + r, need, b);
+        }
+    }
+    if (PHASE == 10) {
+        const unsigned long long v = R.words[b];
+        const int32_t e = (int32_t)(v >> 32);
+        if (v != ~0ull && e < ln.best_err) {
+            const uint4 p = R.payload[(int64_t)((v >> ROT_WORD_ROT_SHIFT) & 3ull) * R.cap + (int64_t)(v & ROT_WORD_POS_MASK)];
+            ln.best_err = e; ln.improved = true;
+            ln.best[0] = p.x; ln.best[1] = p.y; ln.best[2] = p.z; ln.best[3] = p.w;
+        }
+        ln.tx.fence();
+        if (S.mode_selection[3] && !mode6_cannot_win(ln)) mode_6<3>(ln, S);
+    }
     if (DO13 && PHASE != 4) {
         if (on13 && S.fastSkipTreshold_mode1 > 0) { ln.tx.fence(); unpack_win(w, wins4[(int64_t)wide_win_slot(1) * nblocks + b]); refine_and_commit<1>(ln, w, S.refineIterations[1], S.channels); }
         if (on13 && S.fastSkipTreshold_mode3 > 0) { ln.tx.fence(); unpack_win(w, wins4[(int64_t)wide_win_slot(3) * nblocks + b]); refine_and_commit<3>(ln, w, S.refineIterations[3], S.channels); }
@@ -1414,9 +1442,9 @@
         append_to_list(out_list, out_count, live && rgb, b);
         append_to_list(out_list7, out_count7, live && !rgb, b);
     }
-    if (PHASE == 3 || PHASE == 5) {
+    if (TAIL3 || PHASE == 5) {
         int32_t inc;
-        if (PHASE == 3) inc = ln.best_err + (ln.best_err < e02 ? 1 : 0);
+        if (TAIL3) inc = ln.best_err + (ln.best_err < e02 ? 1 : 0);
         else            inc = (e02 <= e_alpha) ? e02 : e_alpha + 1;
         if (live) inc_err[b] = inc;
         ln.tx.fence();
@@ -1426,8 +1454,8 @@
         const float lim7 = (float)inc - 0.5f;
         const bool with7 = PHASE == 5 && out_list7 != nullptr;
         const PairTarget* target = nullptr;
-        if (PHASE == 3) target = reinterpret_cast<const PairTarget*>(out_count + (PAIR_CTR_TARGET - PAIR_CTR_LIST));
-        const bool pairs = PHASE == 3 && target->P.words != nullptr;
+        if (TAIL3) target = reinterpret_cast<const PairTarget*>(out_count + (PAIR_CTR_TARGET - PAIR_CTR_LIST));
+        const bool pairs = TAIL3 && target->P.words != nullptr;
         bool need = !live, need7 = !live || !with7;
         unsigned long long mine = 0, any = 0;
 #pragma unroll 1
@@ -1491,7 +1519,7 @@
     }
     bool store = live;
     if (PHASE == 2 || PHASE == 5) store = store && ln.best_err <= e_alpha;
-    if (PHASE == 4 || PHASE == 7) store = store && ln.improved;
+    if (PHASE == 4 || PHASE == 7 || PHASE == 10) store = store && ln.improved;
     if (PHASE == 8) store = store && ln.improved && !redo;
     if ((PHASE == 4 || PHASE == 8) && store) inc_err[b] = ln.best_err;
     if (store) {
@@ -1603,6 +1631,64 @@
     }
 }
 
+#ifndef ROT_TASK_WAVES
+#define ROT_TASK_WAVES 2
+#endif
+template <bool VEC16>
+__global__ void __launch_bounds__(TPB) __attribute__((amdgpu_waves_per_eu(ROT_TASK_WAVES, ROT_TASK_WAVES)))
+bc7_rot_tasks(const uint8_t* __restrict__ src, int64_t stride, int32_t blocks_x, const bc7_enc_settings S, const int32_t* __restrict__ inc_err, const RotRegion R)
+{
+    __shared__ unsigned short s_seed16[2048];
+    __shared__ uint32_t s_seed32[2048];
+    __shared__ uint2 s_pal[8 * TPB];
+    __shared__ int32_t s_first[4];
+    if (threadIdx.x == 0) {
+        int32_t t = 0;
+        for (int r = 0; r < 3; r++) { s_first[r] = t; t += (R.counts[r] + 63) >> 6; }
+        s_first[3] = t;
+    }
+    __syncthreads();
+    const int32_t total = s_first[3];
+    const int32_t wpb = TPB / 64;
+    if ((int32_t)blockIdx.x * wpb >= total) return;
+    Lane ln;
+    ln.T = stage_seed_tables_fast(s_seed16, s_seed32, threadIdx.x, TPB);
+    __syncthreads();
+    ln.keys = nullptr;
+    ln.pal = s_pal + threadIdx.x;
+    ln.best_err = ERR_MAX; ln.improved = false; ln.opaque_err = 0;
+    ln.best[0] = ln.best[1] = ln.best[2] = ln.best[3] = 0u;
+    const int lane = (int)(threadIdx.x & 63u);
+    const int32_t first1 = s_first[1], first2 = s_first[2];
+#pragma unroll 1
+    for (int32_t tile = (int32_t)blockIdx.x * wpb + (int32_t)(threadIdx.x >> 6); tile < total; tile += (int32_t)gridDim.x * wpb) {
+        const int r = __builtin_amdgcn_readfirstlane((tile >= first1 ? 1 : 0) + (tile >= first2 ? 1 : 0));
+        const int32_t len = R.counts[r];
+        const int32_t at = (tile - s_first[r]) * 64 + lane;
+        const bool live = at < len;
+        const int32_t pos = live ? at : len - 1;
+        const int32_t b = R.lists[(int64_t)r * R.cap + pos];
+        load_block<VEC16>(ln.tx, src, stride, blocks_x, b);
+        const int32_t inc = inc_err[b];
+        Dual best4, best5;
+        clear(best4); clear(best5);
+        int32_t err4 = inc, err5 = ERR_MAX;
+        modes_45_scan(ln, S, r, r + 1, best4, err4, best5, err5);
+        const bool five = err5 < err4;
+        if (five || err4 < inc) {
+            uint32_t blk[4] = {0u, 0u, 0u, 0u};
+            if (five) emit_dual<5>(blk, best5); else emit_dual<4>(blk, best4);
+            if (live) {
+                R.payload[(int64_t)r * R.cap + pos] = make_uint4(blk[0], blk[1], blk[2], blk[3]);
+                const unsigned long long word = ((unsigned long long)(uint32_t)(five ? err5 : err4) << 32) | ((five ? 1ull : 0ull) << ROT_WORD_MODE5_SHIFT) |
+                                                ((unsigned long long)r << ROT_WORD_ROT_SHIFT) | (unsigned long long)pos;
+                atomicMin(R.words + b, word);
+            }
+        }
+        ln.tx.fence();
+    }
+}
+
 constexpr int WIDE_SLOTS = 18;
 constexpr int WIDE_SLOT_M4 = 5, WIDE_SLOT_M5 = 13, WIDE_SLOT_M6 = 17;
 constexpr int WIDE_MAX_TASKS = 56;
@@ -1824,6 +1910,31 @@
     if (vec) hipLaunchKernelGGL((bc7_test_bounds<true>),  grid, dim3(TPB), 0, st, src, stride, bx, (int32_t)n, out);
     else     hipLaunchKernelGGL((bc7_test_bounds<false>), grid, dim3(TPB), 0, st, src, stride, bx, (int32_t)n, out);
 }
+template <bool VEC16>
+__global__ void __launch_bounds__(TPB) bc7_test_rot_bounds(const uint8_t* __restrict__ src, int64_t stride, int32_t blocks_x, int32_t nblocks, float* __restrict__ out)
+{
+    const int32_t gid = blockIdx.x * TPB + threadIdx.x;
+    const int32_t b = gid < nblocks ? gid : nblocks - 1;
+    Tex tx;
+    load_block<VEC16>(tx, src, stride, blocks_x, b);
+    IStats<3> full;
+    stats_int<3>(full, tx.pl, whole_block());
+#pragma unroll
+    for (int r = 0; r < 3; r++) {
+        const float lb = rotation_bound(r, full);
+        if (gid < nblocks) out[(int64_t)b * 3 + r] = lb;
+    }
+}
+void launch_bc7_test_rot_bounds(const uint8_t* src, int64_t stride, int width, int height, float* out, hipStream_t st)
+{
+    const int bx = width / 4;
+    const int64_t n = (int64_t)bx * (height / 4);
+    if (n <= 0) return;
+    const bool vec = ((reinterpret_cast<uintptr_t>(src) | (uintptr_t)stride) & 15) == 0;
+    const dim3 grid((unsigned)((n + TPB - 1) / TPB));
+    if (vec) hipLaunchKernelGGL((bc7_test_rot_bounds<true>),  grid, dim3(TPB), 0, st, src, stride, bx, (int32_t)n, out);
+    else     hipLaunchKernelGGL((bc7_test_rot_bounds<false>), grid, dim3(TPB), 0, st, src, stride, bx, (int32_t)n, out);
+}
 #endif
 
 static std::atomic<int> g_bc7_path{-1};
@@ -1883,6 +1994,11 @@
 static bool bc7_pairs_on()
 {
     const char* e = std::getenv("ITW_BC7_PAIRS");
+    return !(e && e[0] == '0');
+}
+static bool bc7_rot_tasks_on()
+{
+    const char* e = std::getenv("ITW_BC7_ROT_TASKS");
     return !(e && e[0] == '0');
 }
 static int32_t bc7_pair_cap(int32_t layout_cap)
@@ -1929,12 +2045,12 @@
 {
     return (size_t)5 * wide_win_entries(n) * sizeof(uint4) + (((size_t)WIDE_SLOTS * n * sizeof(int32_t) + 15) & ~(size_t)15) + (size_t)WIDE_SLOTS * n * sizeof(uint4);
 }
-struct ListRegion { size_t list, wins, compact, cap, pair_words, pair_redo, pair_buckets, pair_ctr, pair_cap; };
-struct FusedLayout { size_t inc, list0, list1, list2, counts, words; ListRegion band[2]; };
-struct FusedNeeds { bool lists, bands, compact, pairs; };
+struct ListRegion { size_t list, wins, compact, cap, pair_words, pair_redo, pair_buckets, pair_ctr, pair_cap, rot_lists, rot_payload; };
+struct FusedLayout { size_t inc, list0, list1, list2, counts, words, rot_words; ListRegion band[2]; };
+struct FusedNeeds { bool lists, bands, compact, pairs, rot; };
 static FusedNeeds fused_needs(const bc7_enc_settings* s)
 {
-    if (!s) return FusedNeeds{true, true, true, true};
+    if (!s) return FusedNeeds{true, true, true, true, true};
     bc7_enc_settings S = *s;
     S.channels = (s->channels == 4) ? 4 : 3;
     auto ranked = [](int t) { return t > 0 && t < 64; };
@@ -1944,7 +2060,7 @@
     const bool bounded = bc7_bounded_order() && on02 && on13 && !r13;
     const bool alpha = bc7_alpha_first(S);
     const bool on7 = S.mode_selection[1] && S.fastSkipTreshold_mode7 > 0;
-    return FusedNeeds{alpha || bounded, bounded, bounded && !alpha && bc7_compact_lists(), bounded && !alpha && !on7};
+    return FusedNeeds{alpha || bounded, bounded, bounded && !alpha && bc7_compact_lists(), bounded && !alpha && !on7, bounded && !alpha && !on7 && S.channels == 3};
 }
 static FusedLayout fused_layout(size_t n, const FusedNeeds& need)
 {
@@ -1970,6 +2086,9 @@
     for (int k = 0; k < 2; k++) { W.band[k].pair_words = o; o += need.pairs ? 4 * W.band[k].cap : 0; }
     for (int k = 0; k < 2; k++) { W.band[k].pair_redo = o; o += need.pairs ? W.band[k].cap : 0; }
     for (int k = 0; k < 2; k++) { W.band[k].pair_cap = W.band[k].cap / 8; W.band[k].pair_buckets = o; o += need.pairs ? 64 * W.band[k].pair_cap : 0; }
+    W.rot_words = o; o = up4(o + (need.rot ? 2 * n : 0));
+    for (int k = 0; k < 2; k++) { W.band[k].rot_lists = o; o += need.rot ? 3 * W.band[k].cap : 0; }
+    for (int k = 0; k < 2; k++) { W.band[k].rot_payload = o; o += need.rot ? 12 * W.band[k].cap : 0; }
     W.words = o;
     return W;
 }
@@ -2173,16 +2292,17 @@
             };
             auto finish = [&](auto phase, const int32_t* in_list, const int32_t* in_count, int32_t* out_list, int32_t* out_count,
                               int32_t* out_list7 = nullptr, int32_t* out_count7 = nullptr, ChunkSel sel = ChunkSel{0, 1, 0, nullptr, 0}, int32_t cnt = -1,
-                              hipStream_t s = nullptr, const uint32_t* wins = nullptr, int32_t rows = 0, const uint4* in_compact = nullptr, uint4* out_compact = nullptr) {
+                              hipStream_t s = nullptr, const uint32_t* wins = nullptr, int32_t rows = 0, const uint4* in_compact = nullptr, uint4* out_compact = nullptr,
+                              RotRegion rot = RotRegion{nullptr, nullptr, nullptr, nullptr, 0}) {
                 constexpr int PH = decltype(phase)::value;
-                if (PH == 3 && out_count != rgb_count + 16 + PAIR_CTR_LIST && out_count != rgb_count + 16 + PAIR_CTR_WORDS + PAIR_CTR_LIST)
+                if ((PH == 3 || PH == 10) && out_count != rgb_count + 16 + PAIR_CTR_LIST && out_count != rgb_count + 16 + PAIR_CTR_WORDS + PAIR_CTR_LIST)
                     fail_msg("bc7_finish_all<3>: the list length must be word %d of a band's counter block", PAIR_CTR_LIST);
                 if (cnt < 0) cnt = nchunks;
                 if (!s) s = st;
                 if (!wins) { wins = wins4; rows = (int32_t)n; }
                 const dim3 grid((unsigned)cnt);
-                if (L.vec) hipLaunchKernelGGL((bc7_finish_all<true, PH>),  grid, blk, 0, s, src, stride, bx, rows, dst, wins, S, alpha_err, in_list, in_count, out_list, out_count, out_list7, out_count7, sel, in_compact, out_compact);
-                else       hipLaunchKernelGGL((bc7_finish_all<false, PH>), grid, blk, 0, s, src, stride, bx, rows, dst, wins, S, alpha_err, in_list, in_count, out_list, out_count, out_list7, out_count7, sel, in_compact, out_compact);
+                if (L.vec) hipLaunchKernelGGL((bc7_finish_all<true, PH>),  grid, blk, 0, s, src, stride, bx, rows, dst, wins, S, alpha_err, in_list, in_count, out_list, out_count, out_list7, out_count7, sel, in_compact, out_compact, rot);
+                else       hipLaunchKernelGGL((bc7_finish_all<false, PH>), grid, blk, 0, s, src, stride, bx, rows, dst, wins, S, alpha_err, in_list, in_count, out_list, out_count, out_list7, out_count7, sel, in_compact, out_compact, rot);
             };
             const bool bounded = bc7_bounded_order() && on02 && on13 && !r13;
             if (bc7_alpha_first(S)) {
@@ -2233,17 +2353,20 @@
             } else if (bounded && !on7) {
                 const bool two = bc7_bands() > 1 && aux && !aux->single && aux->stream && nchunks >= 32;
                 const bool pairs = bc7_pairs_on();
+                const bool rot_tasks = bc7_rot_tasks_on() && S.channels == 3 && S.mode45_channel0 >= 0 && S.mode45_channel0 <= 3;
                 const bool pilot = two && bc7_pilot_threshold() >= 0 && aux->mid;
                 int32_t stripe = nchunks / 16;
                 stripe = stripe < 1 ? 1 : (stripe > 64 ? 64 : stripe);
                 const int32_t stripes = (nchunks + stripe - 1) / stripe;
-                struct Band { ChunkSel sel; int32_t cnt; hipStream_t s; int32_t* list; int32_t* count; uint32_t* wins; int32_t rows; uint4* compact; PairRegion P; int32_t* redo; };
+                struct Band { ChunkSel sel; int32_t cnt; hipStream_t s; int32_t* list; int32_t* count; uint32_t* wins; int32_t rows; uint4* compact; PairRegion P; int32_t* redo; RotRegion R; };
                 auto band = [&](int k, hipStream_t s) {
                     const ListRegion& r = W.band[k];
                     Band B{ChunkSel{two ? 1 : 0, stripe, k, nullptr, 0}, two ? ((stripes + 1 - k) / 2) * stripe : nchunks, s,
                            reinterpret_cast<int32_t*>(wins4 + r.list), nullptr, wins4 + r.wins, 0, compact_on ? reinterpret_cast<uint4*>(wins4 + r.compact) : nullptr,
                            PairRegion{reinterpret_cast<uint64_t*>(wins4 + r.pair_words), reinterpret_cast<int32_t*>(wins4 + r.pair_buckets), reinterpret_cast<int32_t*>(wins4 + r.pair_ctr),
-                                      bc7_pair_cap((int32_t)(two ? r.pair_cap : 2 * r.pair_cap))}, reinterpret_cast<int32_t*>(wins4 + r.pair_redo)};
+                                      bc7_pair_cap((int32_t)(two ? r.pair_cap : 2 * r.pair_cap))}, reinterpret_cast<int32_t*>(wins4 + r.pair_redo),
+                           RotRegion{reinterpret_cast<int32_t*>(wins4 + r.rot_lists), rgb_count + (k ? 11 : 3), reinterpret_cast<unsigned long long*>(wins4 + W.rot_words),
+                                     reinterpret_cast<uint4*>(wins4 + r.rot_payload), (int32_t)(two ? r.cap : 2 * r.cap)}};
                     B.count = B.P.ctr + PAIR_CTR_LIST;
                     B.rows = B.cnt * TPB;
                     if (!two) { B.list = list13; B.wins = wins4; B.rows = (int32_t)n; }
@@ -2252,7 +2375,13 @@
                 auto gated = [&](const Band& B, int32_t want) { ChunkSel g = B.sel; if (pilot) { g.gate = pilot_flag; g.want = want; } return g; };
                 auto head = [&](const Band& B) { scan_rgb(nullptr, nullptr, false, true, 0, B.sel, B.cnt, B.s); };
                 auto tail = [&](const Band& B) {
-                    finish(std::integral_constant<int, 3>{}, nullptr, nullptr, B.list, B.count, nullptr, nullptr, gated(B, 1), B.cnt, B.s, nullptr, 0, nullptr, B.compact);
+                    if (rot_tasks) {
+                        finish(std::integral_constant<int, 9>{}, nullptr, nullptr, nullptr, nullptr, nullptr, nullptr, gated(B, 1), B.cnt, B.s, nullptr, 0, nullptr, nullptr, B.R);
+                        if (L.vec) hipLaunchKernelGGL((bc7_rot_tasks<true>),  dim3((unsigned)B.cnt), blk, 0, B.s, src, stride, bx, S, alpha_err, B.R);
+                        else       hipLaunchKernelGGL((bc7_rot_tasks<false>), dim3((unsigned)B.cnt), blk, 0, B.s, src, stride, bx, S, alpha_err, B.R);
+                        finish(std::integral_constant<int, 10>{}, nullptr, nullptr, B.list, B.count, nullptr, nullptr, gated(B, 1), B.cnt, B.s, nullptr, 0, nullptr, B.compact, B.R);
+                    } else
+                        finish(std::integral_constant<int, 3>{}, nullptr, nullptr, B.list, B.count, nullptr, nullptr, gated(B, 1), B.cnt, B.s, nullptr, 0, nullptr, B.compact);
                     if (pairs) {
                         int32_t* redo_count = B.P.ctr + PAIR_CTR_REDO;
                         hipLaunchKernelGGL(bc7_pair_scan, dim3((unsigned)((B.cnt + 1) / 2)), blk, 0, B.s, src, stride, bx, B.list, B.compact, S, B.P);
@@ -2311,6 +2440,7 @@
                         ITW_CHECK(hipMemcpy(h, rgb_count, sizeof h, hipMemcpyDeviceToHost));
                         std::fprintf(stderr, "bc7 pilot: estimate %d of %d sampled blocks listed -> %s; lists %d + %d of %lld blocks\n", h[8], h[9], h[6] ? "bounded" : "reference order",
                                      h[16 + PAIR_CTR_LIST], h[16 + PAIR_CTR_WORDS + PAIR_CTR_LIST], (long long)n);
+                        if (rot_tasks) std::fprintf(stderr, "bc7 rot tasks: rotation lists %d / %d / %d (band 0) + %d / %d / %d (band 1)\n", h[3], h[4], h[5], h[11], h[12], h[13]);
                         for (int k = 0; k < 2 && pairs; k++) {
                             int32_t c[PAIR_CTR_WORDS];
                             ITW_CHECK(hipMemcpy(c, (k ? Bb : A).P.ctr, sizeof c, hipMemcpyDeviceToHost));
diff --git a/intel-texture-works-plugin_amd/csrc/bc7_exact.hpp b/intel-texture-works-plugin_amd/csrc/bc7_exact.hpp
--- a/intel-texture-works-plugin_amd/csrc/bc7_exact.hpp
+++ b/intel-texture-works-plugin_amd/csrc/bc7_exact.hpp
@@ -182,6 +182,22 @@
     return (e0 * e0 + e1 * e1) * 0.999999f;
 }
 
+#define BOUND_SLACK2_16 2.82842732f
+__device__ __forceinline__ float rotation_bound(int p, const IStats<3>& full)
+{
+    const int32_t c00 = 16 * full.m[0] - full.s[0] * full.s[0], c11 = 16 * full.m[4] - full.s[1] * full.s[1], c22 = 16 * full.m[7] - full.s[2] * full.s[2];
+    const int32_t c01 = 16 * full.m[1] - full.s[0] * full.s[1], c02 = 16 * full.m[2] - full.s[0] * full.s[2], c12 = 16 * full.m[5] - full.s[1] * full.s[2];
+    const int32_t cii = (p == 0) ? c11 : c00, cjj = (p == 2) ? c11 : c22, cij = (p == 0) ? c12 : ((p == 1) ? c02 : c01);
+    const long long det = (long long)cii * (long long)cjj - (long long)cij * (long long)cij;
+    const float t = (float)(cii + cjj);
+    const float dif = (float)(cii - cjj), b = (float)cij;
+    const float lam = 0.5f * (t + __builtin_amdgcn_sqrtf(dif * dif + 4.0f * (b * b)));
+    const float res = ((float)det * __builtin_amdgcn_rcpf(fmaxf(lam, 1.0f))) * 0.99999f;
+    const float dist = __builtin_amdgcn_sqrtf(res * rcp_of_count(16)) * 0.999999f - BOUND_SLACK2_16;
+    const float e = fmaxf(dist, 0.0f);
+    return e * e * 0.999999f;
+}
+
 template <int CH>
 __device__ __forceinline__ void stats_float(Stats<CH>& f, const IStats<CH>& st)
 {
diff --git a/intel-texture-works-plugin_amd/csrc/kernels.hpp b/intel-texture-works-plugin_amd/csrc/kernels.hpp
--- a/intel-texture-works-plugin_amd/csrc/kernels.hpp
+++ b/intel-texture-works-plugin_amd/csrc/kernels.hpp
@@ -27,6 +27,7 @@
 void launch_bc7 (const uint8_t* src, int64_t stride, int width, int height, uint8_t* dst,
                  const bc7_enc_settings& s, float* workspace, hipStream_t st, const Bc7Aux* aux = nullptr);
 void launch_bc7_test_bounds(const uint8_t* src, int64_t stride, int width, int height, float* out, hipStream_t st);
+void launch_bc7_test_rot_bounds(const uint8_t* src, int64_t stride, int width, int height, float* out, hipStream_t st);
 size_t bc6h_workspace_bytes(int width, int height, const bc6h_enc_settings& s);
 void launch_bc6h(const uint8_t* src, int64_t stride, int width, int height, uint8_t* dst,
                  const bc6h_enc_settings& s, hipStream_t st, void* workspace = nullptr);
diff --git a/intel-texture-works-plugin_amd/itw_amd/__init__.py b/intel-texture-works-plugin_amd/itw_amd/__init__.py
--- a/intel-texture-works-plugin_amd/itw_amd/__init__.py
+++ b/intel-texture-works-plugin_amd/itw_amd/__init__.py
@@ -2,7 +2,7 @@
     lib, test_lib, TEST_HOOK_SYMBOLS, lib_path, RgbaSurface, Bc7Settings, Bc6hSettings, EtcSettings, BC7_PROFILES, BC6H_PROFILES,
     bc7_profile, bc6h_profile, etc_profile, compress, compress_numpy, band_for_part, version, device_info,
     BYTES_PER_BLOCK, EXPORTED_SYMBOLS, DXGI_FORMAT, DdsDesc, image_func, compress_image, PROGRESS_FUNC, pad_to_multiple_of_4, dds_file, decode, block_count, KEEPS_PARTIAL_BLOCKS, SIGNED_FORMATS,
-    available, set_error_mode, last_error, ON_ERROR_ABORT, ON_ERROR_RETURN, set_bc7_path, set_bc7_pilot, compress_image_multigpu, multigpu_sub_bands, MultiGpuStats, source_sha256, bc7_two_subset_bounds,
+    available, set_error_mode, last_error, ON_ERROR_ABORT, ON_ERROR_RETURN, set_bc7_path, set_bc7_pilot, compress_image_multigpu, multigpu_sub_bands, MultiGpuStats, source_sha256, bc7_two_subset_bounds, bc7_rotation_bounds,
     chain_bytes, compress_chain, mip_chain, decode_chain, decode_image, load_dds, dds_images,
     KtxDesc, ktx_file, ktx_images, load_ktx,
     ErrorStats, OWN_CHANNELS, measure, measure_async, measure_chain, stats_from_tensor,
diff --git a/intel-texture-works-plugin_amd/itw_amd/abi.py b/intel-texture-works-plugin_amd/itw_amd/abi.py
--- a/intel-texture-works-plugin_amd/itw_amd/abi.py
+++ b/intel-texture-works-plugin_amd/itw_amd/abi.py
@@ -28,7 +28,7 @@
     + ["itwDecodeBlocks", "itwDecodeChain", "itwDecodeImage", "itwMeasureBlocks", "itwMeasureChain", "itwStatsPsnr"]
     + ["itwDdsLevelBytes", "itwDdsHeaderBytes", "itwDdsFileBytes", "itwDdsWriteHeader", "itwDdsReadHeader", "itwDdsWriteFile", "itwDdsImage"]
     + ["itwKtxHeaderBytes", "itwKtxFileBytes", "itwKtxWriteHeader", "itwKtxReadHeader", "itwKtxWriteFile", "itwKtxImage"])
-TEST_HOOK_SYMBOLS = ("itwTestRcp", "itwTestRsqrt", "itwTestF2I", "itwTestBc7TwoSubsetBounds", "itwTestBc45IndexTable", "itwTestBc45ClosestS",
+TEST_HOOK_SYMBOLS = ("itwTestRcp", "itwTestRsqrt", "itwTestF2I", "itwTestBc7TwoSubsetBounds", "itwTestBc7RotationBounds", "itwTestBc45IndexTable", "itwTestBc45ClosestS",
                      "itwMultiGpuTestInjectFailure", "itwTestCombinerHold", "itwTestCombinerCounters")
 
 
@@ -251,6 +251,8 @@
                 getattr(L, n).restype = None
             L.itwTestBc7TwoSubsetBounds.argtypes = [C.POINTER(RgbaSurface), C.c_void_p]
             L.itwTestBc7TwoSubsetBounds.restype = None
+            L.itwTestBc7RotationBounds.argtypes = [C.POINTER(RgbaSurface), C.c_void_p]
+            L.itwTestBc7RotationBounds.restype = None
             L.itwTestBc45IndexTable.argtypes = [C.c_void_p]
             L.itwTestBc45IndexTable.restype = C.c_int
             L.itwTestBc45ClosestS.argtypes = [C.c_void_p]
@@ -527,6 +529,23 @@
     return out
 
 
+def bc7_rotation_bounds(img):
+    import torch
+    assert img.is_cuda and img.dim() == 3 and img.shape[2] == 4 and img.element_size() == 1
+    assert img.stride(2) == 1 and img.stride(1) == 4
+    h, w = img.shape[:2]
+    out = torch.empty(((h // 4) * (w // 4), 3), dtype=torch.float32, device=img.device)
+    L = test_lib()
+    with torch.cuda.device(img.device):
+        L.itwSetStream(torch.cuda.current_stream(img.device).cuda_stream)
+        surf = RgbaSurface(img.data_ptr(), w, h, img.stride(0))
+        L.itwTestBc7RotationBounds(C.byref(surf), out.data_ptr())
+    e = L.itwLastError()
+    if e:
+        raise RuntimeError(e.decode())
+    return out
+
+
 def image_func(fmt, profile=None, L=None):
     name = {"bc1": "CompressImageBC1", "bc3": "CompressImageBC3", "bc4": "CompressImageBC4", "bc5": "CompressImageBC5",
             "bc4_snorm": "CompressImageBC4S", "bc5_snorm": "CompressImageBC5S"}.get(fmt) or \
```

Result: faster. 4023 Mpixels/s (median of 6 runs) (+4.4%).
